# Russoul/cuda-mat

Hardware: AMD Instinct MI355X
Metric: BiCGSTAB iters/sec + SpMV effective HBM GB/s, 10M-row CSR at 1/2/4/8 GPUs (higher is better)
Workload: dtype f64

## Files before the change

### cuda_mat_amd/_lib.py

```python
import ctypes as C
import os
import subprocess

_HERE = os.path.dirname(os.path.abspath(__file__))
LIB_PATH = os.path.join(_HERE, "libcudamat_hip.so")

OK = 0
PRECOND_NONE, PRECOND_ILU0, PRECOND_BLOCK_ILU0 = 0, 1, 2
LOOP_PBICGSTAB, LOOP_PBICGSTAB2, LOOP_PIPELINED = 0, 1, 2
FLAG_DEBUG, FLAG_PROFILE, FLAG_NO_EXIT, FLAG_X0_ONES = 1, 2, 4, 8


class CudamatError(RuntimeError):
    def __init__(self, code, msg):
        super().__init__("cudamat error %d: %s" % (code, msg))
        self.code = code


class Stats(C.Structure):
    _fields_ = [("iters", C.c_int), ("half_exit", C.c_int), ("converged", C.c_int),
                ("breakdown", C.c_int), ("nrm0", C.c_double), ("nrm", C.c_double),
                ("t_analysis", C.c_double), ("t_factor", C.c_double), ("t_solve", C.c_double),
                ("t_total", C.c_double), ("ms_spmv", C.c_double), ("n_spmv", C.c_int),
                ("ms_trsv", C.c_double), ("n_trsv", C.c_int), ("n_levels_l", C.c_int),
                ("n_levels_u", C.c_int), ("trsv_form", C.c_int), ("trsv_fallbacks", C.c_int),
                ("n_gather", C.c_int), ("n_allreduce", C.c_int), ("ms_gather", C.c_double),
                ("ms_gather_exposed", C.c_double), ("ms_allreduce", C.c_double), ("overlapped", C.c_int),
                ("loop_form", C.c_int), ("gather_fraction", C.c_double), ("ms_spmv_alone", C.c_double),
                ("loop_fallbacks", C.c_int), ("restarts", C.c_int), ("t_upload", C.c_double), ("t_setup", C.c_double),
                ("t_tune", C.c_double), ("spmv_mode", C.c_int), ("plan_reused", C.c_int),
                ("trsv_groups_l", C.c_int), ("trsv_groups_u", C.c_int)]

    def as_dict(self):
        return {k: getattr(self, k) for k, _ in self._fields_}


ALLGATHER_FN = C.CFUNCTYPE(C.c_int, C.c_void_p, C.c_void_p, C.c_void_p, C.c_int64)
ALLREDUCE_FN = C.CFUNCTYPE(C.c_int, C.c_void_p, C.c_void_p, C.c_int)


GATHER_PART_FN = C.CFUNCTYPE(C.c_int, C.c_void_p, C.c_void_p, C.c_void_p, C.c_int64, C.c_int64, C.c_int64)
_I64P = C.POINTER(C.c_int64)
GATHER_WINDOW_FN = C.CFUNCTYPE(C.c_int, C.c_void_p, C.c_void_p, C.c_void_p, C.c_int64, _I64P, _I64P, _I64P, _I64P)


class Comm(C.Structure):
    _fields_ = [("rank", C.c_int), ("world", C.c_int), ("user", C.c_void_p),
                ("allgather", ALLGATHER_FN), ("allreduce", ALLREDUCE_FN),
                ("gather_part", GATHER_PART_FN), ("comm_stream", C.c_void_p),
                ("allreduce_side", ALLREDUCE_FN), ("reduce_stream", C.c_void_p),
                ("gather_window", GATHER_WINDOW_FN)]


def build(force=False):
    if force:
        subprocess.run(["make", "-C", _HERE, "clean"], check=True, capture_output=True)
    r = subprocess.run(["make", "-C", _HERE, "-j", "6"], capture_output=True, text=True)
    if r.returncode != 0:
        raise RuntimeError("building libcudamat_hip.so failed:\n" + r.stdout + r.stderr)


_P = C.c_void_p
_SIGS = {
    "cudamat_version": (C.c_int, []),
    "cudamat_last_error": (C.c_char_p, []),
    "cudamat_device_count": (C.c_int, [C.POINTER(C.c_int)]),
    "cudamat_ctx_create": (C.c_int, [C.c_int, _P, C.POINTER(_P)]),
    "cudamat_ctx_destroy": (C.c_int, [_P]),
    "cudamat_ctx_set_option": (C.c_int, [_P, C.c_char_p, C.c_char_p]),
    "cudamat_ctx_reset_options": (C.c_int, [_P]),
    "cudamat_options_help": (C.c_char_p, []),
    "cudamat_option_check": (C.c_int, [C.c_char_p, C.c_char_p]),
    "cudamat_ctx_sync": (C.c_int, [_P]),
    "cudamat_ctx_stream": (C.c_int, [_P, C.POINTER(_P)]),
    "cudamat_malloc": (C.c_int, [_P, C.c_size_t, C.POINTER(_P)]),
    "cudamat_free": (C.c_int, [_P, _P]),
    "cudamat_h2d": (C.c_int, [_P, _P, _P, C.c_size_t]),
    "cudamat_d2h": (C.c_int, [_P, _P, _P, C.c_size_t]),
    "cudamat_d2d": (C.c_int, [_P, _P, _P, C.c_size_t]),
    "cudamat_memset": (C.c_int, [_P, _P, C.c_int, C.c_size_t]),
    "cudamat_timer_create": (C.c_int, [_P, C.POINTER(_P)]),
    "cudamat_timer_start": (C.c_int, [_P, _P]),
    "cudamat_timer_stop": (C.c_int, [_P, _P]),
    "cudamat_timer_elapsed_ms": (C.c_int, [_P, _P, C.POINTER(C.c_double)]),
    "cudamat_timer_destroy": (C.c_int, [_P, _P]),
    "cudamat_spmv": (C.c_int, [_P, C.c_int, _P, _P, _P, C.c_int, C.c_double, _P, _P, C.c_double, _P]),
    "cudamat_dot": (C.c_int, [_P, C.c_int64, _P, _P, _P]),
    "cudamat_nrm2": (C.c_int, [_P, C.c_int64, _P, _P]),
    "cudamat_axpy": (C.c_int, [_P, C.c_int64, C.c_double, _P, _P]),
    "cudamat_scal": (C.c_int, [_P, C.c_int64, C.c_double, _P]),
    "cudamat_solver_create": (C.c_int, [_P, C.c_int, C.c_int64, C.c_int64, _P, _P, _P, C.c_int, C.POINTER(_P)]),
    "cudamat_solver_create_host": (C.c_int, [_P, C.c_int, C.c_int64, C.c_int64, _P, _P, _P, C.c_int, C.POINTER(_P)]),
    "cudamat_solver_destroy": (C.c_int, [_P]),
    "cudamat_solver_set_shift": (C.c_int, [_P, _P]),
    "cudamat_solver_ilu0": (C.c_int, [_P]),
    "cudamat_solver_block_ilu0": (C.c_int, [_P]),
    "cudamat_solver_ilu0_values": (C.c_int, [_P, _P]),
    "cudamat_solver_ilu0_nnz": (C.c_int, [_P, C.POINTER(C.c_int64)]),
    "cudamat_solver_trsv_form": (C.c_int, [_P, C.POINTER(C.c_int)]),
    "cudamat_solver_precond_apply": (C.c_int, [_P, _P, _P]),
    "cudamat_solver_set_comm": (C.c_int, [_P, C.POINTER(Comm)]),
    "cudamat_solve_sharded": (C.c_int, [C.c_int, C.c_int, C.c_int, _P, _P, _P, _P, _P, _P, C.c_int, C.c_int, C.c_int,
                                        C.c_double, C.c_int, _P, C.POINTER(Stats)]),
    "cudamat_comm_dry_create": (C.c_int, [_P, C.c_int, C.c_int, C.POINTER(Comm)]),
    "cudamat_comm_dry_destroy": (C.c_int, [C.POINTER(Comm)]),
    "cudamat_rccl_available": (C.c_int, []),
    "cudamat_rccl_unique_id": (C.c_int, [_P]),
    "cudamat_rccl_comm_create": (C.c_int, [_P, _P, C.c_int, C.c_int, C.POINTER(Comm)]),
    "cudamat_rccl_comm_destroy": (C.c_int, [C.POINTER(Comm)]),
    "cudamat_rccl_comm_abort": (C.c_int, [C.POINTER(Comm)]),
    "cudamat_solver_spmv_mode": (C.c_int, [_P, C.POINTER(C.c_int)]),
    "cudamat_solver_spmv_kernel": (C.c_int, [_P, C.c_char_p, C.c_int]),
    "cudamat_solver_value_dict": (C.c_int, [_P, C.POINTER(C.c_int)]),
    "cudamat_solver_placement": (C.c_int, [_P, C.POINTER(C.c_int), C.POINTER(C.c_int), C.POINTER(C.c_double), C.c_char_p, C.c_int]),
    "cudamat_solver_spmv": (C.c_int, [_P, _P, _P]),
    "cudamat_solver_solve": (C.c_int, [_P, _P, _P, C.c_int, C.c_int, C.c_int, C.c_double, C.c_int,
                                       C.POINTER(Stats)]),
    "cudamat_solver_history": (C.c_int, [_P, _P, C.c_int, C.POINTER(C.c_int)]),
    "cudamat_solver_spmm": (C.c_int, [_P, C.c_int, _P, C.c_int, _P, C.c_int]),
    "cudamat_solver_solve_many": (C.c_int, [_P, C.c_int, _P, C.c_int, _P, C.c_int, C.c_int, C.c_int, C.c_int, C.c_double,
                                            C.c_int, _P, C.POINTER(C.c_int)]),
    "cudamat_solver_precond_apply_many": (C.c_int, [_P, C.c_int, _P, C.c_int, _P, C.c_int]),
    "cudamat_solver_trsm_kernel": (C.c_int, [_P, C.c_int, C.c_char_p, C.c_int]),
    "cudamat_solver_history_col": (C.c_int, [_P, C.c_int, _P, C.c_int, C.POINTER(C.c_int)]),
    "cudamat_solve_many": (C.c_int, [C.c_int, C.c_int, _P, _P, _P, _P, C.c_int, _P, C.c_int, _P, _P, C.c_int, C.c_int,
                                     C.c_int, C.c_int, C.c_double, _P, C.POINTER(C.c_int)]),
    "cudamat_solver_spmm_shifts": (C.c_int, [_P, C.c_int, _P, C.c_int, _P, C.c_int, _P, C.c_int]),
    "cudamat_solver_solve_shifts": (C.c_int, [_P, C.c_int, _P, C.c_int, _P, C.c_int, _P, C.c_int, C.c_int, C.c_int, C.c_int,
                                              C.c_double, C.c_int, _P, C.POINTER(C.c_int)]),
    "cudamat_solve_shifts": (C.c_int, [C.c_int, C.c_int, _P, _P, _P, C.c_int, _P, C.c_int, _P, C.c_int, _P, _P, C.c_int,
                                       C.c_int, C.c_int, C.c_double, _P, C.POINTER(C.c_int)]),
    "cudamat_solve": (C.c_int, [C.c_int, C.c_int, _P, _P, _P, _P, _P, _P, C.c_int, C.c_int, C.c_int,
                                C.c_double, C.c_int, _P, C.POINTER(Stats)]),
    "cudamat_plan_cache_clear": (C.c_int, []),
    "cudamat_pool_trim": (C.c_int, []),
    "cudamat_mem_info": (C.c_int, [C.c_int, C.POINTER(C.c_size_t), C.POINTER(C.c_size_t), C.POINTER(C.c_size_t)]),
    "cudamat_poisson5_nnz": (C.c_int64, [C.c_int, C.c_int]),
    "cudamat_gen_poisson5": (C.c_int, [_P, C.c_int, C.c_int, C.c_int64, C.c_int64, C.c_int, _P, _P, _P]),
    "cudamat_rand_row_nnz": (C.c_int, [C.c_int64, C.c_int]),
    "cudamat_gen_rand_rows": (C.c_int, [_P, C.c_int64, C.c_int, C.c_uint64, C.c_int64, C.c_int64,
                                        C.c_int, _P, _P, _P]),
    "cudamat_gen_xstar": (C.c_int, [_P, C.c_int64, C.c_int64, C.c_uint64, _P]),
    "cudamat_load_mtx": (C.c_int, [C.c_char_p, C.c_int, C.POINTER(C.c_int), C.POINTER(C.c_int),
                                   C.POINTER(C.c_int), C.POINTER(C.POINTER(C.c_double)),
                                   C.POINTER(C.POINTER(C.c_int)), C.POINTER(C.POINTER(C.c_int))]),
    "cudamat_host_free": (None, [_P]),
    "cudamat_to_dense_vector": (None, [C.c_int, C.c_int, _P, _P, _P]),
}

_lib = None


def lib():
    global _lib
    if _lib is None:
        if not os.path.exists(LIB_PATH):
            build()
        L = C.CDLL(LIB_PATH)
        for name, (res, args) in _SIGS.items():
            fn = getattr(L, name)
            fn.restype = res
            fn.argtypes = args
        _lib = L
    return _lib


def check(rc):
    if rc != OK:
        raise CudamatError(rc, lib().cudamat_last_error().decode(errors="replace"))


def device_count():
    n = C.c_int(0)
    rc = lib().cudamat_device_count(C.byref(n))
    return n.value if rc == OK else 0
```

### cuda_mat_amd/api.py

```python
import ctypes as C

import numpy as np

from . import _lib
from ._lib import (FLAG_DEBUG, FLAG_NO_EXIT, FLAG_PROFILE, FLAG_X0_ONES, LOOP_PBICGSTAB,
                   LOOP_PBICGSTAB2, LOOP_PIPELINED, PRECOND_BLOCK_ILU0, PRECOND_ILU0, PRECOND_NONE, Comm, CudamatError, Stats, check)


def _np(a, dtype):
    return np.ascontiguousarray(a, dtype=dtype)


def _vp(a):
    return None if a is None else a.ctypes.data_as(C.c_void_p)


_GPUS = 1


def use_gpus(ngpu):
    global _GPUS
    _GPUS = max(1, int(ngpu))


def _solve(n, nnz, A, iA, jA, d, x0, b, precond, loop, maxit, tol, debug):
    A, iA, jA, b = _np(A, np.float64), _np(iA, np.int32), _np(jA, np.int32), _np(b, np.float64)
    d = None if d is None else _np(d, np.float64)
    x0 = None if x0 is None else _np(x0, np.float64)
    if len(iA) != n + 1 or len(A) < nnz or len(jA) < nnz or len(b) != n:
        raise ValueError("array sizes do not match n / nnz")
    x = np.zeros(n)
    st = Stats()
    if _GPUS > 1:
        if precond == PRECOND_ILU0:
            precond = PRECOND_BLOCK_ILU0
        check(_lib.lib().cudamat_solve_sharded(_GPUS, n, nnz, _vp(A), _vp(iA), _vp(jA), _vp(d), _vp(x0), _vp(b), precond,
                                               loop, maxit, tol, int(bool(debug)), _vp(x), C.byref(st)))
    else:
        check(_lib.lib().cudamat_solve(n, nnz, _vp(A), _vp(iA), _vp(jA), _vp(d), _vp(x0), _vp(b), precond,
                                       loop, maxit, tol, int(bool(debug)), _vp(x), C.byref(st)))
    return x, st


def bicgstab(n, nnz, A, iA, jA, b, maxit, tol, debug=False):
    x, st = _solve(n, nnz, A, iA, jA, None, None, b, PRECOND_NONE, LOOP_PBICGSTAB2, maxit, tol, debug)
    return bool(st.converged), x, st.t_solve, st


def bicgstab_d(n, nnz, A0, iA0, jA0, d, x0, b, maxit, tol, debug=False):
    x, st = _solve(n, nnz, A0, iA0, jA0, d, x0, b, PRECOND_NONE, LOOP_PBICGSTAB2, maxit, tol, debug)
    return bool(st.converged), x, st.t_solve, st


def bicgstab_lu_precond(n, nnz, A, iA, jA, b, maxit, tol, debug=False):
    x, st = _solve(n, nnz, A, iA, jA, None, None, b, PRECOND_ILU0, LOOP_PBICGSTAB, maxit, tol, debug)
    return True, x, st.t_solve, st


def bicgstab_many(n, nnz, A, iA, jA, B, maxit, tol, d=None, x0=None):
    A, iA, jA = _np(A, np.float64), _np(iA, np.int32), _np(jA, np.int32)
    B = np.asarray(B, dtype=np.float64)
    if B.ndim == 1:
        B = B[:, None]
    if len(iA) != n + 1 or len(A) < nnz or len(jA) < nnz or B.shape[0] != n:
        raise ValueError("array sizes do not match n / nnz")
    k = B.shape[1]
    Bf = np.asfortranarray(B)
    d = None if d is None else _np(d, np.float64)
    x0f = None
    if x0 is not None:
        x0f = np.asfortranarray(np.asarray(x0, dtype=np.float64).reshape(n, k))
    X = np.zeros((n, k), order="F")
    st = (Stats * max(k, 1))()
    form = C.c_int(0)
    check(_lib.lib().cudamat_solve_many(n, nnz, _vp(A), _vp(iA), _vp(jA), _vp(d), k, _vp(Bf), n, _vp(x0f), _vp(X), n,
                                        PRECOND_NONE, LOOP_PBICGSTAB2, maxit, tol, st, C.byref(form)))
    stats = [st[j] for j in range(k)]
    return [bool(s.converged) for s in stats], np.ascontiguousarray(X), (stats[0].t_solve if k else 0.0), stats, form.value


def bicgstab_d_many(n, nnz, A0, iA0, jA0, D, x0, B, maxit, tol):
    A0, iA0, jA0 = _np(A0, np.float64), _np(iA0, np.int32), _np(jA0, np.int32)
    B = np.asarray(B, dtype=np.float64)
    if B.ndim == 1:
        B = B[:, None]
    if len(iA0) != n + 1 or len(A0) < nnz or len(jA0) < nnz or B.ndim != 2 or B.shape[0] != n:
        raise ValueError("array sizes do not match n / nnz")
    k = B.shape[1]
    D = np.asarray(D, dtype=np.float64)
    if D.ndim == 1 and D.shape[0] == k:
        D = np.broadcast_to(D[None, :], (n, k))
    if D.shape != (n, k):
        raise ValueError("D must have shape (n, k) = (%d, %d), or hold k scalars; got %s" % (n, k, D.shape))
    Df, Bf = np.asfortranarray(D), np.asfortranarray(B)
    x0f = None
    if x0 is not None:
        x0f = np.asarray(x0, dtype=np.float64)
        if x0f.size != n * k:
            raise ValueError("x0 must have shape (n, k)")
        x0f = np.asfortranarray(x0f.reshape(n, k))
    X = np.zeros((n, k), order="F")
    st = (Stats * max(k, 1))()
    form = C.c_int(0)
    check(_lib.lib().cudamat_solve_shifts(n, nnz, _vp(A0), _vp(iA0), _vp(jA0), k, _vp(Df), n, _vp(Bf), n, _vp(x0f), _vp(X), n,
                                          LOOP_PBICGSTAB2, maxit, tol, st, C.byref(form)))
    stats = [st[j] for j in range(k)]
    return [bool(s.converged) for s in stats], np.ascontiguousarray(X), (stats[0].t_solve if k else 0.0), stats, form.value


def bicgstab_lu_precond_many(n, nnz, A, iA, jA, B, maxit, tol):
    A, iA, jA = _np(A, np.float64), _np(iA, np.int32), _np(jA, np.int32)
    B = np.asarray(B, dtype=np.float64)
    if B.ndim == 1:
        B = B[:, None]
    if len(iA) != n + 1 or len(A) < nnz or len(jA) < nnz or B.ndim != 2 or B.shape[0] != n:
        raise ValueError("array sizes do not match n / nnz")
    k = B.shape[1]
    Bf = np.asfortranarray(B)
    X = np.zeros((n, k), order="F")
    st = (Stats * max(k, 1))()
    form = C.c_int(0)
    check(_lib.lib().cudamat_solve_many(n, nnz, _vp(A), _vp(iA), _vp(jA), None, k, _vp(Bf), n, None, _vp(X), n,
                                        PRECOND_ILU0, LOOP_PBICGSTAB, maxit, tol, st, C.byref(form)))
    stats = [st[j] for j in range(k)]
    return [True] * k, np.ascontiguousarray(X), (stats[0].t_solve if k else 0.0), stats, form.value


def loadMMSparseMatrix(filename, elem_type="d", csrFormat=True):
    if elem_type != "d":
        raise ValueError("only elem_type 'd' is supported on this path")
    m, n, nnz = C.c_int(), C.c_int(), C.c_int()
    v, r, c = C.POINTER(C.c_double)(), C.POINTER(C.c_int)(), C.POINTER(C.c_int)()
    L = _lib.lib()
    err = L.cudamat_load_mtx(str(filename).encode(), int(bool(csrFormat)), C.byref(m), C.byref(n),
                             C.byref(nnz), C.byref(v), C.byref(r), C.byref(c))
    if err:
        return 1, 0, 0, 0, None, None, None
    nr = m.value + 1 if csrFormat else nnz.value
    nc = nnz.value if csrFormat else n.value + 1
    row = np.ctypeslib.as_array(r, shape=(nr,)).astype(np.int32, copy=True)
    col = np.ctypeslib.as_array(c, shape=(nc,)).astype(np.int32, copy=True) if nc else np.zeros(0, np.int32)
    val = (np.ctypeslib.as_array(v, shape=(nnz.value,)).astype(np.float64, copy=True)
           if nnz.value else np.zeros(0))
    for p in (v, r, c):
        L.cudamat_host_free(p)
    return 0, m.value, n.value, nnz.value, val, row, col


def toDenseVector(n, nnz, A, IA):
    A, IA = _np(A, np.float64), _np(IA, np.int32)
    out = np.empty(n)
    _lib.lib().cudamat_to_dense_vector(n, nnz, _vp(A), _vp(IA), _vp(out))
    return out


class DeviceArray:

    def __init__(self, ctx, n, dtype):
        self.ctx, self.n, self.dtype = ctx, int(n), np.dtype(dtype)
        p = C.c_void_p()
        check(_lib.lib().cudamat_malloc(ctx.h, self.n * self.dtype.itemsize, C.byref(p)))
        self.ptr = p.value

    @property
    def nbytes(self):
        return self.n * self.dtype.itemsize

    def upload(self, a):
        a = _np(a, self.dtype)
        assert a.size == self.n
        check(_lib.lib().cudamat_h2d(self.ctx.h, self.ptr, _vp(a), self.nbytes))
        return self

    def download(self):
        out = np.empty(self.n, self.dtype)
        check(_lib.lib().cudamat_d2h(self.ctx.h, _vp(out), self.ptr, self.nbytes))
        return out

    def zero(self):
        check(_lib.lib().cudamat_memset(self.ctx.h, self.ptr, 0, self.nbytes))
        return self

    def free(self):
        if self.ptr:
            _lib.lib().cudamat_free(self.ctx.h, self.ptr)
            self.ptr = None


def _ptr(a):
    if a is None:
        return None
    if isinstance(a, DeviceArray):
        return a.ptr
    if hasattr(a, "data_ptr"):
        return a.data_ptr()
    return int(a)


class Context:

    def __init__(self, device=0, stream=None):
        h = C.c_void_p()
        check(_lib.lib().cudamat_ctx_create(device, stream, C.byref(h)))
        self.h = h
        self.device = device

    def close(self):
        if self.h:
            _lib.lib().cudamat_ctx_destroy(self.h)
            self.h = None

    def sync(self):
        check(_lib.lib().cudamat_ctx_sync(self.h))

    def set_option(self, name, value):
        check(_lib.lib().cudamat_ctx_set_option(self.h, str(name).encode(), str(value).encode()))
        return self

    def reset_options(self):
        check(_lib.lib().cudamat_ctx_reset_options(self.h))
        return self

    def empty(self, n, dtype=np.float64):
        return DeviceArray(self, n, dtype)

    def array(self, a, dtype=None):
        a = np.asarray(a)
        dtype = a.dtype if dtype is None else dtype
        return DeviceArray(self, a.size, dtype).upload(a)

    def spmv(self, n, rowptr, colidx, val, base, x, y, alpha=1.0, beta=0.0, d=None):
        check(_lib.lib().cudamat_spmv(self.h, n, _ptr(rowptr), _ptr(colidx), _ptr(val), base, alpha,
                                      _ptr(x), _ptr(d), beta, _ptr(y)))

    def dot(self, n, x, y):
        out = self.empty(1)
        check(_lib.lib().cudamat_dot(self.h, n, _ptr(x), _ptr(y), out.ptr))
        v = out.download()[0]
        out.free()
        return v

    def nrm2(self, n, x):
        out = self.empty(1)
        check(_lib.lib().cudamat_nrm2(self.h, n, _ptr(x), out.ptr))
        v = out.download()[0]
        out.free()
        return v

    def axpy(self, n, alpha, x, y):
        check(_lib.lib().cudamat_axpy(self.h, n, alpha, _ptr(x), _ptr(y)))

    def scal(self, n, alpha, x):
        check(_lib.lib().cudamat_scal(self.h, n, alpha, _ptr(x)))

    def gen_rand_rows(self, n, per_row, seed, row0, row1, base, rowptr, colidx, val):
        check(_lib.lib().cudamat_gen_rand_rows(self.h, n, per_row, seed, row0, row1, base, _ptr(rowptr),
                                               _ptr(colidx), _ptr(val)))

    def gen_poisson5(self, nx, ny, row0, row1, base, rowptr, colidx, val):
        check(_lib.lib().cudamat_gen_poisson5(self.h, nx, ny, row0, row1, base, _ptr(rowptr),
                                              _ptr(colidx), _ptr(val)))

    def gen_xstar(self, i0, i1, seed, x):
        check(_lib.lib().cudamat_gen_xstar(self.h, i0, i1, seed, _ptr(x)))

    def timer(self):
        return Timer(self)


class Timer:

    def __init__(self, ctx):
        self.ctx = ctx
        h = C.c_void_p()
        check(_lib.lib().cudamat_timer_create(ctx.h, C.byref(h)))
        self.h = h

    def start(self):
        check(_lib.lib().cudamat_timer_start(self.ctx.h, self.h))

    def stop(self):
        check(_lib.lib().cudamat_timer_stop(self.ctx.h, self.h))

    def elapsed_ms(self):
        ms = C.c_double()
        check(_lib.lib().cudamat_timer_elapsed_ms(self.ctx.h, self.h, C.byref(ms)))
        return ms.value

    def close(self):
        if self.h:
            _lib.lib().cudamat_timer_destroy(self.ctx.h, self.h)
            self.h = None


class Solver:

    def __init__(self, ctx, n_local, n_cols, nnz, rowptr, colidx, val, base):
        self.ctx = ctx
        self.n, self.n_cols, self.nnz = int(n_local), int(n_cols), int(nnz)
        h = C.c_void_p()
        check(_lib.lib().cudamat_solver_create(ctx.h, self.n, self.n_cols, self.nnz, _ptr(rowptr),
                                               _ptr(colidx), _ptr(val), base, C.byref(h)))
        self.h = h
        self._keep = []

    @classmethod
    def from_host_csr(cls, ctx, rowptr, colidx, val, n_cols=None):
        rowptr, colidx, val = _np(rowptr, np.int32), _np(colidx, np.int32), _np(val, np.float64)
        n = len(rowptr) - 1
        base = int(rowptr[0])
        nnz = int(rowptr[-1]) - base
        if nnz == 0:
            colidx, val = np.zeros(1, np.int32), np.zeros(1)
        s = cls.__new__(cls)
        s.ctx = ctx
        s.n, s.n_cols, s.nnz = n, int(n if n_cols is None else n_cols), nnz
        h = C.c_void_p()
        check(_lib.lib().cudamat_solver_create_host(ctx.h, s.n, s.n_cols, s.nnz, _vp(rowptr), _vp(colidx), _vp(val), base, C.byref(h)))
        s.h = h
        s._keep = []
        return s

    def close(self):
        if self.h:
            _lib.lib().cudamat_solver_destroy(self.h)
            self.h = None

    def set_shift(self, d):
        self._keep.append(d)
        check(_lib.lib().cudamat_solver_set_shift(self.h, _ptr(d)))

    def set_comm(self, comm):
        self._keep.append(comm)
        check(_lib.lib().cudamat_solver_set_comm(self.h, None if comm is None else C.byref(comm)))

    def ilu0(self):
        check(_lib.lib().cudamat_solver_ilu0(self.h))

    def trsv_form(self):
        f = C.c_int()
        check(_lib.lib().cudamat_solver_trsv_form(self.h, C.byref(f)))
        return f.value

    def block_ilu0(self):
        check(_lib.lib().cudamat_solver_block_ilu0(self.h))

    def ilu0_values(self):
        cnt = C.c_int64()
        check(_lib.lib().cudamat_solver_ilu0_nnz(self.h, C.byref(cnt)))
        out = self.ctx.empty(max(cnt.value, 1))
        check(_lib.lib().cudamat_solver_ilu0_values(self.h, out.ptr))
        v = out.download()[:cnt.value]
        out.free()
        return v

    def precond_apply(self, vin, vout):
        check(_lib.lib().cudamat_solver_precond_apply(self.h, _ptr(vin), _ptr(vout)))

    def precond_apply_many(self, nrhs, In, ldin, Out, ldout):
        check(_lib.lib().cudamat_solver_precond_apply_many(self.h, int(nrhs), _ptr(In), int(ldin), _ptr(Out), int(ldout)))

    def trsm_kernel(self, nrhs):
        buf = C.create_string_buffer(160)
        check(_lib.lib().cudamat_solver_trsm_kernel(self.h, int(nrhs), buf, 160))
        return buf.value.decode()

    def spmv(self, x, y):
        check(_lib.lib().cudamat_solver_spmv(self.h, _ptr(x), _ptr(y)))

    def spmv_mode(self):
        m = C.c_int()
        check(_lib.lib().cudamat_solver_spmv_mode(self.h, C.byref(m)))
        return m.value

    def spmv_kernel(self):
        buf = C.create_string_buffer(96)
        check(_lib.lib().cudamat_solver_spmv_kernel(self.h, buf, 96))
        return buf.value.decode()

    def placement(self):
        placed, slabs, sec = C.c_int(), C.c_int(), C.c_double()
        buf = C.create_string_buffer(256)
        check(_lib.lib().cudamat_solver_placement(self.h, C.byref(placed), C.byref(slabs), C.byref(sec), buf, 256))
        return {"placed": placed.value, "slabs": slabs.value, "seconds": sec.value, "blocks_by_class": buf.value.decode().strip()}

    def value_dict(self):
        m = C.c_int()
        check(_lib.lib().cudamat_solver_value_dict(self.h, C.byref(m)))
        return m.value

    def solve(self, b, x, precond=PRECOND_NONE, loop=LOOP_PBICGSTAB, maxit=2000, tol=1e-8, flags=0):
        st = Stats()
        check(_lib.lib().cudamat_solver_solve(self.h, _ptr(b), _ptr(x), precond, loop, maxit, tol, flags,
                                              C.byref(st)))
        return st

    def history(self, cap=1 << 16, col=None):
        if col is not None:
            return self.history_col(col, cap)
        buf = np.empty(cap)
        cnt = C.c_int()
        check(_lib.lib().cudamat_solver_history(self.h, _vp(buf), cap, C.byref(cnt)))
        return buf[:cnt.value].copy()

    def history_col(self, col, cap=1 << 16):
        buf = np.empty(cap)
        cnt = C.c_int()
        check(_lib.lib().cudamat_solver_history_col(self.h, int(col), _vp(buf), cap, C.byref(cnt)))
        return buf[:cnt.value].copy()

    def spmm(self, nrhs, X, ldx, Y, ldy):
        check(_lib.lib().cudamat_solver_spmm(self.h, int(nrhs), _ptr(X), int(ldx), _ptr(Y), int(ldy)))

    def solve_many(self, nrhs, B, ldb, X, ldx, precond=PRECOND_NONE, loop=LOOP_PBICGSTAB, maxit=2000, tol=1e-8, flags=0):
        st = (Stats * max(int(nrhs), 1))()
        form = C.c_int(0)
        check(_lib.lib().cudamat_solver_solve_many(self.h, int(nrhs), _ptr(B), int(ldb), _ptr(X), int(ldx), precond, loop,
                                                   maxit, tol, flags, st, C.byref(form)))
        return [st[j] for j in range(int(nrhs))], form.value

    def spmm_shifts(self, nrhs, X, ldx, D, ldd, Y, ldy):
        check(_lib.lib().cudamat_solver_spmm_shifts(self.h, int(nrhs), _ptr(X), int(ldx), _ptr(D), int(ldd), _ptr(Y), int(ldy)))

    def solve_shifts(self, nrhs, D, ldd, B, ldb, X, ldx, precond=PRECOND_NONE, loop=LOOP_PBICGSTAB, maxit=2000, tol=1e-8,
                     flags=0):
        st = (Stats * max(int(nrhs), 1))()
        form = C.c_int(0)
        check(_lib.lib().cudamat_solver_solve_shifts(self.h, int(nrhs), _ptr(D), int(ldd), _ptr(B), int(ldb), _ptr(X), int(ldx),
                                                     precond, loop, maxit, tol, flags, st, C.byref(form)))
        return [st[j] for j in range(int(nrhs))], form.value
```

### cuda_mat_amd/csrc/config.cpp

```cpp
#include "config.h"

#include <stdio.h>
#include <stdlib.h>
#include <string.h>

#include <unistd.h>

#include <mutex>
#include <set>
#include <string>

extern char **environ;

#include "common.h"

namespace cm {

namespace {

enum Kind { K_FLAG, K_INT, K_LLONG, K_ENUM, K_FAIL };

struct Option {
    const char *name;
    Kind kind;
    int Config::*field;
    long long Config::*wide;
    long long lo, hi;
    const char *words;
    const char *help;
};

#define OPT_FLAG(NAME, FIELD, HELP) {NAME, K_FLAG, &Config::FIELD, nullptr, 0, 1, nullptr, HELP}
#define OPT_INT(NAME, FIELD, LO, HI, HELP) {NAME, K_INT, &Config::FIELD, nullptr, LO, HI, nullptr, HELP}
#define OPT_ENUM(NAME, FIELD, WORDS, HELP) {NAME, K_ENUM, &Config::FIELD, nullptr, 0, 0, WORDS, HELP}

const Option kOptions[] = {
    OPT_INT("VERBOSE", verbose, 0, 2, "1: set-up breakdowns and auto-tune timings on stderr; 2: also the memory classes of a large blocked copy's arrays (timed probe, diagnosis)"),
    OPT_FLAG("ROCTX", roctx, "roctx ranges around solver creation, SpMV-form choice, ILU(0) set-up, the loop, SpMVs and all-reduces"),
    OPT_ENUM("SPMV_MODE", spmv_mode, "csr=0,pb=1,sell=2,pat=3", "force the CSR forms / the blocked two-phase form / SELL-C-sigma / the row-pattern dictionary"),
    OPT_FLAG("SPMV_SELL", spmv_sell, "0: keep SELL-C-sigma out of the candidates"),
    OPT_ENUM("SPMV_FORM", spmv_form, "lanes=1,tiles=2", "inside the CSR forms: lanes per row / nnz-balanced tiles"),
    OPT_INT("SPMV_LANES", spmv_lanes, 2, 64, "lanes per row, a power of two (and no stream tiles)"),
    OPT_FLAG("SPMV_COMPRESS", spmv_compress, "0: stream kernel on the plain 32-bit indices"),
    OPT_FLAG("SPMV_ALIGN", spmv_align, "0: compressed stream kernel without line-aligned copies of its value / offset streams"),
    OPT_ENUM("SPMV_TUNE", spmv_tune_full, "full=1", "time every SpMV candidate even when the column span already decides"),
    OPT_FLAG("VALUE_DICT", value_dict, "0: keep fp64 values even when the matrix has <= 256 distinct ones"),
    OPT_INT("PB_MIN_WAVES", pb_min_waves, 256, 1 << 20, "blocked form: fewest phase-2 waves"),
    OPT_INT("PB_DEPTH", pb_depth, 4, 16, "blocked form: segment loads in flight per phase-2 wave (4, 8 or 16)"),
    OPT_FLAG("POOL", pool, "0: device memory straight from hipMalloc / hipFree instead of the library's recycling pool (read once per process)"),
    OPT_FLAG("SKIP_ORIG_COPY", skip_orig_copy, "0: cudamat_solve with ILU(0) builds the blocked copy in the original index space even when its loop will run in the level-major spaces"),
    OPT_FLAG("EARLY_ANALYSIS", early_analysis, "0: cudamat_solve analyses the ILU(0) levels after the upload of the values instead of beside it"),
    OPT_INT("PB_FILL_OCC", pb_fill_occ, 0, 64, "resident waves per CU of the two-pass fill's first pass (0: 8; probing)"),
    OPT_FLAG("PB_FILL2", pb_fill2, "0: fill the blocked copy with the single-pass scatter kernel (rounds 1-4) instead of the two-pass partition"),
    OPT_INT("PB_PLACE", pb_place, 0, 2, "blocked copy of a large matrix: 1 (default): a resident solver's product stream is placed in a memory class of its own, values and indices in another (timed probe of the device's memory classes, 10-35 ms per copy: spmv_pb.hip); 2: the drop-in calls place theirs as well; 0: arrays wherever the allocator puts them"),
    OPT_INT("PB_PLACE_MAX_MS", pb_place_max_ms, 0, 60000, "PB_PLACE: what the search for an arrangement may take before the arrays are allocated as ever (ms; the slabs it allocates included -- 0.3 ms per 16 GB on most boxes, 2 s on some)"),
    OPT_FLAG("PB_PROBE_FAIL", pb_probe_fail, "1 (tests): treat the run-time LDS-order probe as failed, i.e. select the architected-order phase 2"),
    OPT_FLAG("PB_STRICT", pb_strict, "1: phase 2 adds a row's products of one wave instruction rank by rank (architected order, +10 %)"),
    {"FUSED", K_LLONG, nullptr, &Config::fused, 0, 1LL << 40, nullptr,
     "0: never fold the vector updates into the SpMVs (three launches per iteration); N: do it for every supported plan up to N rows"},
    OPT_FLAG("RESIDENT", resident, "0: never run the whole loop of a very small system in one launch"),
    OPT_INT("RESIDENT_SPIN_LIMIT", resident_spin_limit, 0, 1 << 30, "polls a grid-barrier wait of the single-launch loop may take"),
    OPT_INT("PIPE_RR", pipe_rr, 0, 1 << 20, "residual replacement period of the pipelined loop (0: never)"),
    OPT_FLAG("TRSV_SYNCFREE", trsv_syncfree, "0: one launch per level; 1: dependency-driven launches also for narrow levels"),
    OPT_FLAG("TRSV_LDS", trsv_lds, "0: no single-workgroup LDS-resident triangular solve for small systems"),
    OPT_FLAG("TRSV_HYBRID", trsv_hybrid, "0 | 1: never / always split big factors into far (blocked SpMV) and near (dependency-driven) parts"),
    OPT_INT("TRSV_GROUPS", trsv_groups, 2, 128, "groups of levels of a hybrid factor"),
    OPT_INT("TRSV_LANES", trsv_lanes, 2, 64, "lanes per row of the triangular-solve kernels, a power of two"),
    OPT_INT("TRSV_SPIN_LIMIT", trsv_spin_limit, 1, 1 << 30, "polls of one dependency before a row gives up"),
    OPT_FLAG("TRSV_PERM", trsv_perm, "0: permute around every M^-1 application instead of running the loop in the level-major spaces"),
    OPT_FLAG("LEVELS_SWEEP", levels_sweep, "1: level analysis by relaxation sweeps"),
    OPT_FLAG("ILU0_SIMPLE", ilu0_simple, "1: numeric ILU(0) without LDS staging / prefetch"),
    OPT_FLAG("FORCE_SHARDED", force_sharded, "1: keep the collective path at world size 1"),
    OPT_FLAG("OVERLAP", overlap, "0: plain all-gather instead of pieces behind phase 1 of the blocked SpMV"),
    OPT_INT("OVERLAP_CHUNKS", overlap_chunks, 1, 16, "pieces per slice of an overlapped gather"),
    OPT_FLAG("WINDOWED", windowed, "0: never exchange windows (halo) only"),
    OPT_FLAG("SHARDED_ONE_DEVICE", sharded_one_device,
             "1: cudamat_solve_sharded with every rank on device 0 and host-synchronised copies in place of RCCL (debugging aid)"),
    OPT_FLAG("PLAN_CACHE", plan_cache, "0: cudamat_solve does not keep the solver of its last call"),
    OPT_ENUM("MANY_FORM", many_form, "auto=0,batched=1,columns=2",
             "several right-hand sides: batched (one SpMM per step for up to 8 columns) / columns (one solve per column); auto: the faster as timed at the first solve"),
    OPT_ENUM("MANY_PRECOND", many_precond, "columns=0,auto=1,batched=2",
             "several right-hand sides with ILU(0): columns (one preconditioned solve per column, default) / batched (multi-column triangular solves and one SpMM per step for up to 8 columns, where the factors are covered) / auto: the faster as timed at the first such solve; MANY_FORM = columns overrides"),
    {"TEST_COMM_FAIL", K_FAIL, nullptr, nullptr, 0, 0, nullptr, "rank:k -- fault injection: that rank's k-th all-reduce reports an error (tests)"},
};

bool power_of_two(long long v) { return v > 0 && (v & (v - 1)) == 0; }

bool apply(Config &cfg, const Option &o, const char *value)
{
    switch (o.kind) {
    case K_FLAG:
        if (!strcmp(value, "0") || !strcmp(value, "1")) { cfg.*(o.field) = value[0] - '0'; return true; }
        return false;
    case K_INT: {
        char *end = nullptr;
        const long long v = strtoll(value, &end, 10);
        if (end == value || *end || v < o.lo || v > o.hi) return false;
        if ((!strcmp(o.name, "SPMV_LANES") || !strcmp(o.name, "TRSV_LANES")) && !power_of_two(v)) return false;
        if (!strcmp(o.name, "PB_DEPTH") && v != 4 && v != 8 && v != 16) return false;
        cfg.*(o.field) = (int)v;
        return true;
    }
    case K_LLONG: {
        char *end = nullptr;
        const long long v = strtoll(value, &end, 10);
        if (end == value || *end || v < o.lo || v > o.hi) return false;
        cfg.*(o.wide) = v;
        return true;
    }
    case K_ENUM: {
        const size_t len = strlen(value);
        for (const char *w = o.words; w && *w;) {
            const char *eq = strchr(w, '=');
            if ((size_t)(eq - w) == len && !strncmp(w, value, len)) { cfg.*(o.field) = atoi(eq + 1); return true; }
            const char *comma = strchr(eq, ',');
            w = comma ? comma + 1 : nullptr;
        }
        return false;
    }
    case K_FAIL: {
        int r = -1, k = -1;
        if (sscanf(value, "%d:%d", &r, &k) != 2 || r < 0 || k < 1) return false;
        cfg.fail_rank = r;
        cfg.fail_call = k;
        return true;
    }
    }
    return false;
}

}

bool Config::operator==(const Config &o) const
{
    for (const Option &q : kOptions) {
        if (q.field && this->*(q.field) != o.*(q.field)) return false;
        if (q.wide && this->*(q.wide) != o.*(q.wide)) return false;
    }
    return fail_rank == o.fail_rank && fail_call == o.fail_call;
}

bool config_set(Config &cfg, const char *name, const char *value)
{
    if (!name || !value) { set_error("option name / value is NULL"); return false; }
    if (!strncmp(name, "CUDAMAT_", 8)) name += 8;
    for (const Option &o : kOptions) {
        if (strcmp(o.name, name)) continue;
        if (apply(cfg, o, value)) return true;
        set_error("option %s: value \"%s\" is not accepted (%s)", name, value, o.help);
        return false;
    }
    set_error("unknown option \"%s\" (cudamat_options_help lists them)", name);
    return false;
}

static void warn_once(const std::string &text)
{
    static std::mutex mu;
    static std::set<std::string> seen;
    std::lock_guard<std::mutex> lock(mu);
    if (seen.insert(text).second) fprintf(stderr, "cudamat: %s\n", text.c_str());
}

Config config_from_env()
{
    Config cfg;
    for (const Option &o : kOptions) {
        const std::string var = std::string("CUDAMAT_") + o.name;
        const char *v = getenv(var.c_str());
        if (!v || !*v) continue;
        if (!apply(cfg, o, v))
            warn_once(var + "=\"" + v + "\" is not an accepted value and was IGNORED (" + o.help + ")");
    }
    for (char **e = environ; e && *e; e++) {
        if (strncmp(*e, "CUDAMAT_", 8) || !strncmp(*e, "CUDAMAT_BENCH_", 14)) continue;
        const char *eq = strchr(*e, '=');
        if (!eq || !eq[1]) continue;
        const std::string name(*e + 8, (size_t)(eq - (*e + 8)));
        bool known = false;
        for (const Option &o : kOptions) known = known || name == o.name;
        if (!known) warn_once("CUDAMAT_" + name + " names no switch of this library and was IGNORED (cudamat_options_help lists them)");
    }
    return cfg;
}

const char *config_help()
{
    static const std::string text = [] {
        std::string t;
        for (const Option &o : kOptions) {
            t += "CUDAMAT_";
            t += o.name;
            t += o.kind == K_FLAG ? " = 0 | 1" : o.kind == K_ENUM ? " = " : o.kind == K_FAIL ? " = rank:k" : " = N";
            if (o.kind == K_ENUM) {
                for (const char *w = o.words; w && *w;) {
                    const char *eq = strchr(w, '=');
                    if (w != o.words) t += " | ";
                    t.append(w, (size_t)(eq - w));
                    const char *comma = strchr(eq, ',');
                    w = comma ? comma + 1 : nullptr;
                }
            }
            if (o.kind == K_INT || o.kind == K_LLONG) t += " in [" + std::to_string(o.lo) + ", " + std::to_string(o.hi) + "]";
            t += "   ";
            t += o.help;
            t += "\n";
        }
        return t;
    }();
    return text.c_str();
}

}
```

### cuda_mat_amd/csrc/config.h

```cpp
#pragma once

namespace cm {

struct Config {
    int verbose = 0;
    int roctx = 0;
    int spmv_mode = -1;
    int spmv_sell = 1;
    int spmv_form = 0;
    int spmv_lanes = 0;
    int spmv_compress = 1;
    int spmv_align = 1;
    int spmv_tune_full = 0;
    int value_dict = 1;
    int pb_min_waves = 0;
    int pb_depth = 0;
    int pool = 1;
    int skip_orig_copy = 1;
    int early_analysis = 1;
    int pb_fill_occ = 0;
    int pb_fill2 = 1;
    int pb_place = 1;
    int pb_place_max_ms = 300;
    int pb_probe_fail = 0;
    int pb_strict = 0;
    long long fused = -1;
    int resident = 1;
    int resident_spin_limit = -1;
    int pipe_rr = -1;
    int trsv_syncfree = -1;
    int trsv_lds = 1;
    int trsv_hybrid = -1;
    int trsv_groups = 0;
    int trsv_lanes = 0;
    int trsv_spin_limit = 0;
    int trsv_perm = 1;
    int levels_sweep = 0;
    int ilu0_simple = 0;
    int force_sharded = 0;
    int overlap = 1;
    int overlap_chunks = 0;
    int windowed = 1;
    int sharded_one_device = 0;
    int plan_cache = 1;
    int many_form = 0;
    int many_precond = 0;
    int fail_rank = -1, fail_call = -1;

    bool operator==(const Config &o) const;
    bool operator!=(const Config &o) const { return !(*this == o); }
};

Config config_from_env();
bool config_set(Config &cfg, const char *name, const char *value);
const char *config_help();

}
```

### cuda_mat_amd/csrc/solver.hip

```cpp
#include <mutex>
#include <utility>
#include <math.h>
#include <stdlib.h>
#include <string.h>

#include "solver.h"

using namespace cm;

namespace cm {

int dev_alloc(void **p, size_t bytes)
{
    *p = nullptr;
    hipError_t e = hipMalloc(p, bytes ? bytes : 16);
    if (e != hipSuccess) {
        set_error("hipMalloc(%zu bytes) failed: %s", bytes, hipGetErrorString(e));
        return e == hipErrorOutOfMemory ? CUDAMAT_ERR_NOMEM : CUDAMAT_ERR_HIP;
    }
    return CUDAMAT_OK;
}

static void free_work(cudamat_solver *s)
{
    double **vs[] = {&s->r, &s->rw, &s->p, &s->pw, &s->s, &s->t, &s->v, &s->gather, &s->x0_save, &s->v2,
                     &s->pz, &s->pww, &s->pq, &s->py, &s->pxh, &s->pipeA, &s->pipeB, &s->red_pipe,
                     &s->prh, &s->pwh, &s->psh, &s->pzh, &s->pqh, &s->ptmp};
    for (double **q : vs) {
        if (*q) CM_DROP(hipFree(*q));
        *q = nullptr;
    }
}

int ensure_work(cudamat_solver *s)
{
    if (s->r) return CUDAMAT_OK;
    hipStream_t st = s->ctx->stream;
    const size_t nb = sizeof(double) * (size_t)(s->n_pad > 0 ? s->n_pad : 1);
    double **vs[] = {&s->r, &s->rw, &s->p, &s->pw, &s->s, &s->t, &s->v};
    for (double **q : vs) {
        CM_TRY(dev_alloc((void **)q, nb));
        CM_HIP(hipMemsetAsync(*q, 0, nb, st));
    }
    if (s->ctx->cfg.verbose)
        fprintf(stderr, "[cudamat] work vectors: r %p rw %p p %p pw %p s %p t %p v %p (%zu bytes each)\n", (void *)s->r, (void *)s->rw, (void *)s->p,
                (void *)s->pw, (void *)s->s, (void *)s->t, (void *)s->v, nb);
    if (s->sharded) {
        CM_TRY(dev_alloc((void **)&s->gather, nb * (size_t)s->comm.world));
        CM_HIP(hipMemsetAsync(s->gather, 0, nb * (size_t)s->comm.world, st));
    }
    return CUDAMAT_OK;
}

}

__global__ __launch_bounds__(kBlock) void k_check_rowptr(int n, long long nnz, const int *rp, int *flags)
{
    const long long i = (long long)blockIdx.x * kBlock + threadIdx.x;
    if (i > n) return;
    bool bad = false;
    if (i == 0 && rp[0] != 0) bad = true;
    if (i == n && rp[n] != nnz) bad = true;
    if (i < n && rp[i] > rp[i + 1]) bad = true;
    if (rp[i] < 0 || rp[i] > nnz) bad = true;
    if (bad) flags[0] = 1;
}

__global__ __launch_bounds__(kBlock) void k_check_columns(int n, long long n_cols, const int *rp, const int *ci, int *flags)
{
    constexpr int L = 8;
    const long long row = ((long long)blockIdx.x * kBlock + threadIdx.x) / L;
    if (row >= n) return;
    const int lane = threadIdx.x & (L - 1);
    const int s = rp[row], e = rp[row + 1];
    bool range = false, order = false;
    for (int k = s + lane; k < e; k += L) {
        const int c = ci[k];
        if (c < 0 || c >= n_cols) range = true;
        if (k > s && ci[k - 1] >= c) order = true;
    }
    if (range) flags[1] = 1;
    if (order) flags[2] = 1;
}

static int validate_csr(cudamat_solver *s)
{
    hipStream_t st = s->ctx->stream;
    int *d = (int *)s->ctx->scratch, h[3] = {0, 0, 0};
    hipError_t e = hipMemsetAsync(d, 0, sizeof(h), st);
    hipLaunchKernelGGL(k_check_rowptr, dim3((unsigned)(((long long)s->n + 1 + kBlock - 1) / kBlock)), dim3(kBlock), 0, st, s->n,
                       (long long)s->nnz, s->rp, d);
    if (e == hipSuccess) e = hipGetLastError();
    if (e == hipSuccess) e = hipMemcpyAsync(h, d, sizeof(h), hipMemcpyDeviceToHost, st);
    if (e == hipSuccess) e = hipStreamSynchronize(st);
    if (e == hipSuccess && !h[0] && s->n > 0 && s->nnz > 0) {
        hipLaunchKernelGGL(k_check_columns, dim3((unsigned)(((long long)s->n * 8 + kBlock - 1) / kBlock)), dim3(kBlock), 0, st,
                           s->n, (long long)s->n_cols, s->rp, s->ci, d);
        e = hipGetLastError();
        if (e == hipSuccess) e = hipMemcpyAsync(h, d, sizeof(h), hipMemcpyDeviceToHost, st);
        if (e == hipSuccess) e = hipStreamSynchronize(st);
    }
    if (e != hipSuccess) return fail_hip(e, "CSR validation", __FILE__, __LINE__);
    if (h[0]) { set_error("row pointers must start at the index base, never decrease and end at nnz"); return CUDAMAT_ERR_ARG; }
    if (h[1]) { set_error("a column index lies outside [base, base + n_cols)"); return CUDAMAT_ERR_ARG; }
    s->cols_sorted = h[2] == 0;
    return CUDAMAT_OK;
}

namespace cm {

int solver_alloc(cudamat_ctx *ctx, int n_local, int64_t n_cols, int64_t nnz, cudamat_solver **out)
{
    *out = nullptr;
    CM_ARG(n_local >= 0 && n_cols >= n_local && nnz >= 0, "sizes");
    CM_ARG(nnz < (1LL << 31) && n_cols < (1LL << 31), "local nnz and dimension must fit int32");
    CM_HIP(hipSetDevice(ctx->device));
    cudamat_solver *s = new cudamat_solver();
    s->ctx = ctx;
    s->n = n_local;
    s->n_pad = n_local;
    s->n_cols = n_cols;
    s->nnz = nnz;
    s->t_create0 = now_s();
    hipStream_t st = ctx->stream;
    int rc = CUDAMAT_OK;
    do {
        if ((rc = dev_alloc((void **)&s->rp, sizeof(int) * ((size_t)n_local + 1)))) break;
        if ((rc = dev_alloc((void **)&s->ci, sizeof(int) * (size_t)nnz))) break;
        if ((rc = dev_alloc((void **)&s->val, sizeof(double) * (size_t)nnz))) break;
        if ((rc = dev_alloc((void **)&s->parts_full, sizeof(double) * 2 * kMaxParts))) break;
        if ((rc = dev_alloc((void **)&s->parts_rv, sizeof(double) * 2 * kMaxParts))) break;
        if ((rc = dev_alloc((void **)&s->parts_half, sizeof(double) * 2 * kMaxParts))) break;
        if ((rc = dev_alloc((void **)&s->parts_tt, sizeof(double) * 2 * kMaxParts))) break;
        if ((rc = dev_alloc((void **)&s->red, sizeof(double) * 16))) break;
        if ((rc = dev_alloc((void **)&s->st, sizeof(LoopState)))) break;
        if (hipHostMalloc((void **)&s->st_ring, sizeof(LoopState) * kRing, hipHostMallocDefault) != hipSuccess) {
            rc = CUDAMAT_ERR_HIP; set_error("hipHostMalloc failed"); break;
        }
        if (hipHostMalloc((void **)&s->snap_host, sizeof(unsigned long long) * kRing, hipHostMallocDefault) != hipSuccess ||
            hipHostGetDevicePointer((void **)&s->snap_dev, s->snap_host, 0) != hipSuccess) {
            rc = CUDAMAT_ERR_HIP; set_error("pinned progress words unavailable"); break;
        }
        if (hipMemsetAsync(s->st, 0, sizeof(LoopState), st) != hipSuccess) { rc = CUDAMAT_ERR_HIP; break; }
    } while (0);
    if (rc) {
        cudamat_solver_destroy(s);
        return rc;
    }
    *out = s;
    return CUDAMAT_OK;
}

int solver_setup_pattern(cudamat_solver *s)
{
    cudamat_ctx *ctx = s->ctx;
    hipStream_t st = ctx->stream;
    const bool verbose = ctx->cfg.verbose != 0;
    double t_mark = now_s();
    auto stamp = [&](const char *what) {
        if (!verbose) return;
        const double t = now_s();
        fprintf(stderr, "[cudamat] create %-34s %8.3f ms\n", what, (t - t_mark) * 1e3);
        t_mark = t;
    };
    if (verbose) fprintf(stderr, "[cudamat] create %-34s %8.3f ms\n", "allocations + copies", (t_mark - s->t_create0) * 1e3);
    CM_TRY(validate_csr(s));
    stamp("validation");
    s->plan = plan_spmv(ctx->cfg, s->n, s->nnz);
    CM_TRY(plan_spmv_refine(st, ctx->cfg, s->n, s->nnz, s->rp, 0, &s->plan, ctx->scratch));
    stamp("CSR launch plan (refine)");
    CM_TRY(plan_spmv_compress(st, ctx->cfg, s->n, s->nnz, s->rp, s->ci, &s->plan));
    stamp("compressed-index attempt");
    return CUDAMAT_OK;
}

int solver_setup_values(cudamat_solver *s)
{
    cudamat_ctx *ctx = s->ctx;
    hipStream_t st = ctx->stream;
    if (s->plan.c_off16) {
        CM_TRY(ensure_valdict(s));
        if (s->vd.n > 0) CM_TRY(plan_spmv_dict(st, s->n, s->nnz, s->rp, s->vd.idx, s->vd.dict, &s->plan));
        if (!s->plan.d_pbase)
            CM_TRY(plan_spmv_align(st, ctx->cfg, s->n, s->nnz, s->rp, s->val, &s->plan));
    }
    s->t_create = now_s() - s->t_create0;
    return CUDAMAT_OK;
}

}

extern "C" int cudamat_solver_create(cudamat_ctx *ctx, int n_local, int64_t n_cols, int64_t nnz,
                                     const int *rowptr, const int *colidx, const double *val,
                                     int base, cudamat_solver **out)
{
    CM_ARG(ctx && out, "null pointer");
    *out = nullptr;
    CM_ARG(base == 0 || base == 1, "base in {0,1}");
    CM_ARG(rowptr && (nnz == 0 || (colidx && val)), "null CSR array");
    Range range_create("cudamat: solver create (copies, validation, CSR plan)");
    cudamat_solver *s = nullptr;
    CM_TRY(solver_alloc(ctx, n_local, n_cols, nnz, &s));
    hipStream_t st = ctx->stream;
    int rc = launch_rebase(st, (int64_t)n_local + 1, rowptr, -base, s->rp);
    if (!rc && nnz) {
        rc = launch_rebase(st, nnz, colidx, -base, s->ci);
        if (!rc && hipMemcpyAsync(s->val, val, sizeof(double) * (size_t)nnz, hipMemcpyDeviceToDevice, st) != hipSuccess) {
            rc = CUDAMAT_ERR_HIP; set_error("val copy failed");
        }
    }
    if (!rc && hipStreamSynchronize(st) != hipSuccess) { rc = CUDAMAT_ERR_HIP; set_error("sync after upload failed"); }
    if (!rc) rc = solver_setup_pattern(s);
    if (!rc) rc = solver_setup_values(s);
    if (rc) {
        cudamat_solver_destroy(s);
        return rc;
    }
    *out = s;
    return CUDAMAT_OK;
}

extern "C" int cudamat_solver_destroy(cudamat_solver *s)
{
    if (!s) return CUDAMAT_OK;
    CM_DROP(hipSetDevice(s->ctx->device));
    CM_DROP(hipStreamSynchronize(s->ctx->stream));
    ilu0_release(s);
    pb_free(&s->pb);
    sell_free(&s->sell);
    pat_free(&s->pat);
    free_work(s);
    many_release(s);
    plan_spmv_free(&s->plan);
    void *ptrs[] = {s->rp, s->ci, s->val, s->parts_full, s->parts_rv, s->parts_half, s->parts_tt,
                    s->red, s->st, s->hist};
    for (void *p : ptrs)
        if (p) CM_DROP(hipFree(p));
    if (s->st_ring) CM_DROP(hipHostFree(s->st_ring));
    if (s->snap_host) CM_DROP(hipHostFree(s->snap_host));
    for (int i = 0; i < kRing; i++)
        if (s->ev[i]) CM_DROP(hipEventDestroy(s->ev[i]));
    for (hipEvent_t e : s->prof_ev) CM_DROP(hipEventDestroy(e));
    for (hipEvent_t e : s->comm_ev) CM_DROP(hipEventDestroy(e));
    if (s->need_dev) CM_DROP(hipFree(s->need_dev));
    if (s->bar) CM_DROP(hipFree(s->bar));
    valdict_free(&s->vd);
    for (int e = 0; e < 2; e++) {
        if (s->ev_red[e]) CM_DROP(hipEventDestroy(s->ev_red[e]));
        if (s->ev_red_done[e]) CM_DROP(hipEventDestroy(s->ev_red_done[e]));
    }
    if (s->ev_x) CM_DROP(hipEventDestroy(s->ev_x));
    for (hipEvent_t e : s->ev_part)
        if (e) CM_DROP(hipEventDestroy(e));
    for (hipEvent_t e : s->ev_p1)
        if (e) CM_DROP(hipEventDestroy(e));
    for (hipStream_t q : s->part_stream)
        if (q) { CM_DROP(hipStreamSynchronize(q)); CM_DROP(hipStreamDestroy(q)); }
    delete s;
    return CUDAMAT_OK;
}

extern "C" int cudamat_solver_set_shift(cudamat_solver *s, const double *d)
{
    CM_ARG(s, "solver is NULL");
    s->d = d;
    return CUDAMAT_OK;
}

extern "C" int cudamat_solver_set_comm(cudamat_solver *s, const cudamat_comm *comm)
{
    CM_ARG(s, "solver is NULL");
    CM_HIP(hipStreamSynchronize(s->ctx->stream));
    free_work(s);
    pb_free(&s->pb);
    sell_free(&s->sell);
    pat_free(&s->pat);
    ilu0_release(s);
    s->spmv_mode = -1;
    s->overlap = false;
    s->agreed = false;
    s->windowed = false;
    s->windows_known = false;
    if (s->need_dev) { CM_DROP(hipFree(s->need_dev)); s->need_dev = nullptr; }
    const bool forced = comm && comm->world == 1 && s->ctx->cfg.force_sharded;
    if (!comm || (comm->world <= 1 && !forced)) {
        s->sharded = false;
        s->n_pad = s->n;
        return CUDAMAT_OK;
    }
    CM_ARG(comm->allgather && comm->allreduce, "collectives missing");
    CM_ARG(comm->rank >= 0 && comm->rank < comm->world, "rank");
    const int64_t per = (s->n_cols + comm->world - 1) / comm->world;
    int64_t mine = s->n_cols - per * comm->rank;
    if (mine > per) mine = per;
    if (mine < 0) mine = 0;
    if (mine != s->n) {
        set_error("row block mismatch: rank %d of %d must own %lld rows of %lld (uniform blocks of %lld), has %d",
                  comm->rank, comm->world, (long long)mine, (long long)s->n_cols, (long long)per, s->n);
        return CUDAMAT_ERR_ARG;
    }
    s->comm = *comm;
    s->sharded = true;
    s->n_pad = (int)per;
    if (comm->gather_window && comm->world > 1 && comm->world <= 4096)
        CM_TRY(dev_alloc((void **)&s->need_dev, sizeof(double) * ((size_t)2 * comm->world + (size_t)2 * comm->world * comm->world)));
    if (comm->gather_part && comm->comm_stream && !s->ev_x) {
        CM_HIP(hipEventCreateWithFlags(&s->ev_x, hipEventDisableTiming));
        for (int c = 0; c < kPbMaxChunks; c++) {
            CM_HIP(hipEventCreateWithFlags(&s->ev_part[c], hipEventDisableTiming));
            CM_HIP(hipEventCreateWithFlags(&s->ev_p1[c], hipEventDisableTiming));
            CM_HIP(hipStreamCreateWithFlags(&s->part_stream[c], hipStreamNonBlocking));
        }
    }
    if (s->ctx->cfg.overlap_chunks >= 1 && s->ctx->cfg.overlap_chunks <= kPbMaxChunks) s->overlap_chunks = s->ctx->cfg.overlap_chunks;
    return CUDAMAT_OK;
}

namespace cm {

static hipEvent_t comm_event(cudamat_solver *s)
{
    if (s->comm_used == s->comm_ev.size()) {
        hipEvent_t e = nullptr;
        if (hipEventCreate(&e) != hipSuccess) s->prof_failed = true;
        s->comm_ev.push_back(e);
    }
    return s->comm_ev[s->comm_used++];
}
void comm_mark_begin(cudamat_solver *s, int kind, hipStream_t st)
{
    if (!s->profiling) return;
    s->comm_kind.push_back(kind);
    if (hipEventRecord(comm_event(s), st) != hipSuccess) s->prof_failed = true;
}
void comm_mark_end(cudamat_solver *s, hipStream_t st)
{
    if (s->profiling && hipEventRecord(comm_event(s), st) != hipSuccess) s->prof_failed = true;
}

int spmv_local(cudamat_solver *s, const double *x_local, double *y, int dot, const double *w,
               double *parts, LoopArgs la, int check, ScalarSrc half)
{
    Range range_spmv(s->sharded ? "cudamat: SpMV + exchange of its input" : "cudamat: SpMV");
    const double *xfull = x_local;
    const bool windowed = s->sharded && s->windowed;
    const bool overlapped = s->sharded && !windowed && s->overlap && s->spmv_mode == 1;
    if (windowed) {
        hipStream_t st = s->ctx->stream;
        CM_HIP(hipMemcpyAsync(s->gather + (size_t)s->comm.rank * (size_t)s->n_pad, x_local, sizeof(double) * (size_t)s->n_pad,
                              hipMemcpyDeviceToDevice, st));
        comm_mark_begin(s, 2, st);
        if (s->comm.gather_window(s->comm.user, x_local, s->gather, (int64_t)s->n_pad, s->w_send_off.data(), s->w_send_cnt.data(),
                                  s->w_recv_off.data(), s->w_recv_cnt.data()) != 0) {
            set_error("gather_window callback failed");
            return CUDAMAT_ERR_COMM;
        }
        comm_mark_end(s, st);
    } else if (s->sharded && !overlapped) {
        comm_mark_begin(s, 2, s->ctx->stream);
        if (s->comm.allgather(s->comm.user, x_local, s->gather, (int64_t)s->n_pad) != 0) {
            set_error("allgather callback failed");
            return CUDAMAT_ERR_COMM;
        }
        comm_mark_end(s, s->ctx->stream);
    }
    if (s->sharded) xfull = s->gather;
    SpmvArgs a{};
    a.n = s->n;
    a.rp = s->rp;
    a.ci = s->ci;
    a.val = s->val;
    a.x = xfull;
    a.d = s->d;
    a.xd = x_local;
    a.alpha = 1.0;
    a.beta = 0.0;
    a.y = y;
    a.dot = dot;
    a.w = w;
    a.parts = parts;
    a.loop = la;
    a.check = check;
    a.half = half;
    a.pb_strict = 0;
    if (s->spmv_mode == 1 || s->perm_active) CM_TRY(pb_strict_for(s->ctx, &a.pb_strict));
    if (overlapped) {
        hipStream_t st = s->ctx->stream, cst = (hipStream_t)s->comm.comm_stream;
        const PbPlan &p = s->pb;
        CM_HIP(hipEventRecord(s->ev_x, st));
        CM_HIP(hipStreamWaitEvent(cst, s->ev_x, 0));
        comm_mark_begin(s, 0, cst);
        for (int c = 0; c < p.chunks; c++) {
            const int64_t off = (int64_t)c * p.chunk_len;
            int64_t cnt = (int64_t)s->n_pad - off;
            if (cnt > p.chunk_len) cnt = p.chunk_len;
            if (cnt > 0 && s->comm.gather_part(s->comm.user, x_local, s->gather, (int64_t)s->n_pad, off, cnt) != 0) {
                set_error("gather_part callback failed");
                return CUDAMAT_ERR_COMM;
            }
            CM_HIP(hipEventRecord(s->ev_part[c], cst));
        }
        comm_mark_end(s, cst);
        CM_HIP(hipMemcpyAsync(s->gather + (size_t)s->comm.rank * (size_t)s->n_pad, x_local, sizeof(double) * (size_t)s->n_pad,
                              hipMemcpyDeviceToDevice, st));
        CM_TRY(launch_pb_check(st, a));
        CM_TRY(launch_pb_phase1(st, p, a, 0));
        for (int c = 0; c < p.chunks; c++) {
            hipStream_t ps = s->part_stream[c];
            CM_HIP(hipStreamWaitEvent(ps, s->ev_x, 0));
            CM_HIP(hipStreamWaitEvent(ps, s->ev_part[c], 0));
            CM_TRY(launch_pb_phase1(ps, p, a, 1 + c));
            CM_HIP(hipEventRecord(s->ev_p1[c], ps));
        }
        for (int c = 0; c < p.chunks; c++) CM_HIP(hipStreamWaitEvent(st, s->ev_p1[c], 0));
        return launch_pb_phase2(st, p, a);
    }
    if (s->perm_active) return launch_spmv_pb(s->ctx->stream, s->pb_perm, a);
    if (s->spmv_mode == 1) return launch_spmv_pb(s->ctx->stream, s->pb, a);
    if (s->spmv_mode == 2) return launch_spmv_sell(s->ctx->stream, s->sell, a);
    if (s->spmv_mode == 3) return launch_spmv_pat(s->ctx->stream, s->pat, a);
    return launch_spmv(s->ctx->stream, s->plan, a);
}

int ensure_valdict(cudamat_solver *s)
{
    if (s->vd_tried) return CUDAMAT_OK;
    s->vd_tried = true;
    if (s->nnz < (1 << 20)) return CUDAMAT_OK;
    return valdict_build(s->ctx->stream, s->ctx->cfg, s->nnz, s->val, &s->vd);
}

int spmv_parts(const cudamat_solver *s)
{
    if (s->perm_active) return s->pb_perm.NRB;
    return s->spmv_mode == 1 ? s->pb.NRB : s->spmv_mode == 2 ? s->sell.grid : s->spmv_mode == 3 ? s->pat.grid : plan_spmv_parts(s->plan);
}

__global__ __launch_bounds__(kBlock) void k_col_span(int n, const int *rp, const int *ci, int samples, unsigned long long *sum, int *cnt)
{
    const int q = blockIdx.x * kBlock + threadIdx.x;
    if (q >= samples) return;
    const int row = (int)((long long)q * n / samples);
    const int s = rp[row], e = rp[row + 1];
    if (e - s < 2) return;
    atomicAdd(sum, (unsigned long long)(ci[e - 1] - ci[s]));
    atomicAdd(cnt, 1);
}

static int col_span_bytes(cudamat_solver *s, double *out)
{
    *out = 0.0;
    hipStream_t st = s->ctx->stream;
    unsigned long long *d = (unsigned long long *)s->ctx->scratch, h[2] = {0ULL, 0ULL};
    CM_HIP(hipMemsetAsync(d, 0, sizeof(h), st));
    const int samples = s->n < 4096 ? s->n : 4096;
    hipLaunchKernelGGL(k_col_span, dim3((samples + kBlock - 1) / kBlock), dim3(kBlock), 0, st, s->n, s->rp, s->ci, samples, d, (int *)(d + 1));
    hipError_t e = hipMemcpyAsync(h, d, sizeof(h), hipMemcpyDeviceToHost, st);
    if (e == hipSuccess) e = hipStreamSynchronize(st);
    CM_HIP(e);
    const int cnt = (int)(h[1] & 0xffffffffULL);
    *out = cnt > 0 ? 8.0 * (double)h[0] / cnt : 0.0;
    return CUDAMAT_OK;
}

static int ensure_spmv_mode_inner(cudamat_solver *s);

int spmv_mode_is_blocked_early(cudamat_solver *s, bool *blocked)
{
    *blocked = false;
    const Config &cfg = s->ctx->cfg;
    if (s->sharded || s->n == 0 || s->nnz == 0 || !s->cols_sorted) return CUDAMAT_OK;
    if (cfg.spmv_mode == 0 || cfg.spmv_mode == 2) return CUDAMAT_OK;
    if (cfg.spmv_mode == 1) { *blocked = true; return CUDAMAT_OK; }
    if (!pb_candidate(s->ctx->stream, s->n, s->n_cols, s->nnz, s->rp, s->ci)) return CUDAMAT_OK;
    if (cfg.spmv_tune_full || s->nnz < 8 * (int64_t)s->n) return CUDAMAT_OK;
    if (s->col_span_bytes < 0.0) CM_TRY(col_span_bytes(s, &s->col_span_bytes));
    *blocked = s->col_span_bytes >= 16.0 * 1024 * 1024;
    return CUDAMAT_OK;
}

void spmv_mode_adopt_blocked(cudamat_solver *s, const PbPlan &pb, double seconds)
{
    s->pb = pb;
    s->spmv_mode = 1;
    s->t_spmv_setup = seconds;
    if (s->ctx->cfg.verbose)
        fprintf(stderr, "[cudamat] SpMV form 1 (blocked) built beside the upload in %.3f ms (a row's columns span %.1f MB of x)\n",
                seconds * 1e3, s->col_span_bytes / 1048576.0);
}

int ensure_spmv_mode(cudamat_solver *s)
{
    if (s->spmv_mode >= 0) return CUDAMAT_OK;
    Range range_mode("cudamat: SpMV form (matrix copies, tuning)");
    const double t0 = now_s();
    int rc = ensure_spmv_mode_inner(s);
    const int rc_sync = CM_RC(hipStreamSynchronize(s->ctx->stream));
    if (!rc) rc = rc_sync;
    s->t_spmv_setup = now_s() - t0;
    if (s->ctx->cfg.verbose)
        fprintf(stderr, "[cudamat] SpMV form %d chosen in %.3f ms (blocked copy %.3f ms, timing %.3f ms)\n", s->spmv_mode,
                s->t_spmv_setup * 1e3, s->pb.build_seconds * 1e3, s->t_spmv_timing * 1e3);
    return rc;
}

static int ensure_spmv_mode_inner(cudamat_solver *s)
{
    hipStream_t st = s->ctx->stream;
    const Config &cfg = s->ctx->cfg;
    const bool force_csr = cfg.spmv_mode == 0;
    const bool force_pb = cfg.spmv_mode == 1;
    const bool force_sell = cfg.spmv_mode == 2;
    const bool force_pat = cfg.spmv_mode == 3;
    s->spmv_mode = 0;
    if (force_csr || s->n == 0 || s->nnz == 0) return CUDAMAT_OK;
    bool have[4] = {true, false, false, false};
    if (!force_sell && !force_pat) {
        if (!s->cols_sorted) {
            if (force_pb) { set_error("the blocked SpMV needs rows with increasing column indices"); return CUDAMAT_ERR_ARG; }
        } else if (force_pb || pb_candidate(st, s->n, s->n_cols, s->nnz, s->rp, s->ci)) {
            PbCols cols;
            const bool can_overlap = s->sharded && s->comm.world > 1 && s->comm.gather_part && s->comm.comm_stream;
            if (s->sharded && s->comm.world > 1) {
                cols.per = s->n_pad;
                cols.rank = s->comm.rank;
                cols.chunks = can_overlap ? s->overlap_chunks : 1;
            }
            CM_TRY(ensure_valdict(s));
            const int rc = pb_build(st, cfg, s->n, s->n_cols, s->nnz, s->rp, s->ci, s->val, &s->pb, &cols, &s->vd);
            if (rc != CUDAMAT_OK && force_pb) return rc;
            have[1] = rc == CUDAMAT_OK;
        }
        if (force_pb && !s->sharded) { s->spmv_mode = 1; return CUDAMAT_OK; }
        if (force_pb) { have[0] = false; }
    }
    bool scattered = false;
    {
        if (have[1] && !force_pb && !force_sell && !force_pat && !cfg.spmv_tune_full && s->nnz >= 8 * (int64_t)s->n) {
            if (s->col_span_bytes < 0.0) CM_TRY(col_span_bytes(s, &s->col_span_bytes));
            scattered = s->col_span_bytes >= 16.0 * 1024 * 1024;
        }
        if (scattered) {
            have[0] = false;
            if (!s->sharded) {
                s->spmv_mode = 1;
                if (cfg.verbose)
                    fprintf(stderr, "cudamat: SpMV: a row's columns span %.1f MB of x on average -> blocked, nothing timed\n", s->col_span_bytes / 1048576.0);
                return CUDAMAT_OK;
            }
        }
    }
    const bool sell_off = !cfg.spmv_sell;
    if (force_sell || (!force_pb && !force_pat && !scattered && !sell_off && s->n >= 4096 && s->nnz >= (1 << 16) && s->plan.stream_rows == 0 && s->nnz >= 8 * (int64_t)s->n)) {
        const int rc = sell_build(st, s->n, s->nnz, s->rp, s->ci, s->val, &s->sell, force_sell ? 0.0 : 1.5);
        if (rc != CUDAMAT_OK && force_sell) return rc;
        have[2] = rc == CUDAMAT_OK;
        if (force_sell) { s->spmv_mode = 2; return CUDAMAT_OK; }
    }
    if (force_pat || (!force_pb && !scattered && s->plan.stream_rows > 0 && s->n > 300000 && s->nnz >= (1 << 20))) {
        CM_TRY(ensure_valdict(s));
        const int rc = pat_build(st, s->n, s->nnz, s->rp, s->ci, s->val, &s->pat, force_pat ? 0.0 : 1.25, &s->vd);
        if (rc != CUDAMAT_OK && (force_pat || rc != CUDAMAT_ERR_ARG) && rc != CUDAMAT_ERR_NOMEM) return rc;
        if (rc != CUDAMAT_OK && force_pat) return rc;
        have[3] = rc == CUDAMAT_OK;
        if (force_pat) { s->spmv_mode = 3; return CUDAMAT_OK; }
    }
    if (!have[1] && !have[2] && !have[3]) return CUDAMAT_OK;
    if (force_pb && !have[1]) { set_error("the blocked copy could not be built"); return CUDAMAT_ERR_NOMEM; }
    if (force_pb) have[2] = have[3] = false;
    const LoopArgs la_none{nullptr, nullptr, 0, 0, 0};
    const ScalarSrc nosrc{nullptr, 0, 1};
    const double *xin = s->sharded ? s->gather : s->p;
    hipEvent_t e0 = nullptr, e1 = nullptr;
    CM_HIP(hipEventCreate(&e0));
    if (hipEventCreate(&e1) != hipSuccess) { CM_DROP(hipEventDestroy(e0)); return fail_hip(hipGetLastError(), "hipEventCreate", __FILE__, __LINE__); }
    float ms[4] = {0.f, 0.f, 0.f, 0.f};
    int rc = CUDAMAT_OK;
    const double t_timing0 = now_s();
    for (int mode = 0; mode < 4 && rc == CUDAMAT_OK; mode++) {
        if (!have[mode]) continue;
        SpmvArgs a{};
        a.n = s->n; a.rp = s->rp; a.ci = s->ci; a.val = s->val; a.x = xin; a.d = nullptr; a.xd = s->p;
        a.alpha = 1.0; a.beta = 0.0; a.y = s->v; a.dot = 0; a.loop = la_none; a.check = CHECK_NONE; a.half = nosrc;
        a.pb_strict = 0;
        if (mode == 1) CM_TRY(pb_strict_for(s->ctx, &a.pb_strict));
        for (int rep = 0; rep < 3 && rc == CUDAMAT_OK; rep++) {
            if (rep == 1) rc = CM_RC(hipEventRecord(e0, st));
            if (rc) break;
            rc = mode == 1 ? launch_spmv_pb(st, s->pb, a) : mode == 2 ? launch_spmv_sell(st, s->sell, a) :
                 mode == 3 ? launch_spmv_pat(st, s->pat, a) : launch_spmv(st, s->plan, a);
        }
        if (!rc) rc = CM_RC(hipEventRecord(e1, st));
        if (!rc) rc = CM_RC(hipEventSynchronize(e1));
        if (!rc) rc = CM_RC(hipEventElapsedTime(&ms[mode], e0, e1));
    }
    CM_DROP(hipEventDestroy(e0));
    CM_DROP(hipEventDestroy(e1));
    CM_TRY(rc);
    s->t_spmv_timing = now_s() - t_timing0;
    CM_HIP(hipMemsetAsync(s->v, 0, sizeof(double) * (size_t)(s->n_pad > 0 ? s->n_pad : 1), st));
    s->ms_csr = ms[0] / 2;
    s->ms_pb = ms[1] / 2;
    s->ms_sell = ms[2] / 2;
    s->ms_pat = ms[3] / 2;
    int best = have[0] ? 0 : 1;
    if (rc == CUDAMAT_OK)
        for (int mode = 1; mode < 4; mode++)
            if (have[mode] && (!have[best] || ms[mode] < ms[best])) best = mode;
    s->spmv_mode = best;
    s->ms_spmv_alone = ms[best] / 2;
    const double sell_fill = s->sell.fill;
    if (best != 1) pb_free(&s->pb);
    if (best != 2) sell_free(&s->sell);
    const int npat = s->pat.npat;
    if (best != 3) pat_free(&s->pat);
    if (cfg.verbose)
        fprintf(stderr, "cudamat: SpMV auto-tune csr %.3f ms, blocked %s%.3f ms, sell %s%.3f ms (fill %.2f), row patterns %s%.3f ms (%d patterns) -> %s\n",
                s->ms_csr, have[1] ? "" : "(n/a) ", s->ms_pb, have[2] ? "" : "(n/a) ", s->ms_sell, sell_fill, have[3] ? "" : "(n/a) ", s->ms_pat,
                npat, best == 1 ? "blocked" : best == 2 ? "sell" : best == 3 ? "row patterns" : "csr");
    return CUDAMAT_OK;
}

int allreduce(cudamat_solver *s, double *buf, int count)
{
    Range range_ar("cudamat: all-reduce");
    if (s->ctx->cfg.fail_rank >= 0 && s->ctx->cfg.fail_rank == s->comm.rank && ++s->test_allreduces == s->ctx->cfg.fail_call) {
        set_error("injected all-reduce failure (TEST_COMM_FAIL=%d:%d)", s->ctx->cfg.fail_rank, s->ctx->cfg.fail_call);
        return CUDAMAT_ERR_COMM;
    }
    comm_mark_begin(s, 3, s->ctx->stream);
    if (s->comm.allreduce(s->comm.user, buf, count) != 0) {
        set_error("allreduce callback failed");
        return CUDAMAT_ERR_COMM;
    }
    comm_mark_end(s, s->ctx->stream);
    return CUDAMAT_OK;
}

__global__ __launch_bounds__(kBlock) void k_col_windows(long long nnz, const int *ci, int per, int world, int *lo, int *hi)
{
    extern __shared__ int tab[];
    int *lo_s = tab, *hi_s = tab + world;
    for (int q = threadIdx.x; q < world; q += kBlock) { lo_s[q] = per; hi_s[q] = 0; }
    __syncthreads();
    const long long per_thread = (nnz + (long long)gridDim.x * kBlock - 1) / ((long long)gridDim.x * kBlock);
    const long long k0 = ((long long)blockIdx.x * kBlock + threadIdx.x) * per_thread;
    const long long k1 = k0 + per_thread < nnz ? k0 + per_thread : nnz;
    int cq = -1, clo = 0, chi = 0;
    for (long long k = k0; k < k1; k++) {
        const int c = ci[k], q = c / per, w = c - q * per;
        if (q == cq && w >= clo && w < chi) continue;
        if (q != cq) { cq = q; clo = w; chi = w + 1; }
        else { clo = w < clo ? w : clo; chi = w + 1 > chi ? w + 1 : chi; }
        atomicMin(&lo_s[q], w);
        atomicMax(&hi_s[q], w + 1);
    }
    __syncthreads();
    for (int q = threadIdx.x; q < world; q += kBlock) {
        if (hi_s[q] > 0) { atomicMin(&lo[q], lo_s[q]); atomicMax(&hi[q], hi_s[q]); }
    }
}

static int compute_windows(cudamat_solver *s)
{
    s->windows_known = true;
    s->windowed = false;
    s->gather_fraction = 1.0;
    const int W = s->comm.world, me = s->comm.rank;
    if (!s->comm.gather_window || W <= 1 || W > 4096) return CUDAMAT_OK;
    hipStream_t st = s->ctx->stream;
    const int per = s->n_pad;
    std::vector<int> h((size_t)2 * W);
    std::vector<double> mine((size_t)2 * W, 0.0), all((size_t)2 * W * W, 0.0);
    char saved[512] = "";
    auto local = [&]() -> int {
        int *d_lohi = nullptr;
        CM_HIP(hipMalloc((void **)&d_lohi, sizeof(int) * 2 * (size_t)W));
        for (int q = 0; q < W; q++) { h[(size_t)q] = per; h[(size_t)W + q] = 0; }
        hipError_t e = hipMemcpyAsync(d_lohi, h.data(), sizeof(int) * h.size(), hipMemcpyHostToDevice, st);
        if (e == hipSuccess && s->nnz > 0) {
            hipLaunchKernelGGL(k_col_windows, dim3(row_grid(s->nnz, 4096LL * kBlock)), dim3(kBlock), sizeof(int) * 2 * (size_t)W, st, (long long)s->nnz, s->ci, per, W,
                               d_lohi, d_lohi + W);
        }
        if (e == hipSuccess) e = hipMemcpyAsync(h.data(), d_lohi, sizeof(int) * h.size(), hipMemcpyDeviceToHost, st);
        if (e == hipSuccess) e = hipStreamSynchronize(st);
        CM_DROP(hipFree(d_lohi));
        CM_HIP(e);
        for (int q = 0; q < W; q++)
            if (q != me && h[(size_t)W + q] > h[(size_t)q]) { mine[(size_t)2 * q] = h[(size_t)q]; mine[(size_t)2 * q + 1] = h[(size_t)W + q]; }
        return CUDAMAT_OK;
    };
    const int rc_local = local();
    if (rc_local != CUDAMAT_OK) {
        snprintf(saved, sizeof(saved), "%s", cudamat_last_error());
        mine.assign((size_t)2 * W, -1.0);
    }
    CM_HIP(hipMemcpyAsync(s->need_dev, mine.data(), sizeof(double) * mine.size(), hipMemcpyHostToDevice, st));
    CM_HIP(hipStreamSynchronize(st));
    if (s->comm.allgather(s->comm.user, s->need_dev, s->need_dev + 2 * W, (int64_t)2 * W) != 0) {
        set_error("allgather callback failed");
        return CUDAMAT_ERR_COMM;
    }
    CM_HIP(hipMemcpyAsync(all.data(), s->need_dev + 2 * W, sizeof(double) * all.size(), hipMemcpyDeviceToHost, st));
    CM_HIP(hipStreamSynchronize(st));
    if (rc_local != CUDAMAT_OK) { set_error("%s", saved); return rc_local; }
    for (double v : all)
        if (v < 0.0) { set_error("another rank failed while it looked for its column windows"); return CUDAMAT_ERR_COMM; }
    s->w_send_off.assign((size_t)W, 0); s->w_send_cnt.assign((size_t)W, 0);
    s->w_recv_off.assign((size_t)W, 0); s->w_recv_cnt.assign((size_t)W, 0);
    double worst = 0.0;
    for (int p = 0; p < W; p++) {
        double tot = 0.0;
        for (int q = 0; q < W; q++) {
            const double lo = all[((size_t)p * W + q) * 2], hi = all[((size_t)p * W + q) * 2 + 1];
            if (q == p || hi <= lo) continue;
            tot += hi - lo;
            if (p == me) { s->w_recv_off[(size_t)q] = (int64_t)lo; s->w_recv_cnt[(size_t)q] = (int64_t)(hi - lo); }
            if (q == me) { s->w_send_off[(size_t)p] = (int64_t)lo; s->w_send_cnt[(size_t)p] = (int64_t)(hi - lo); }
        }
        const double frac = tot / ((double)(W - 1) * (double)per);
        if (p == me) s->gather_fraction = frac;
        worst = frac > worst ? frac : worst;
    }
    s->windowed = worst <= 0.5 && s->ctx->cfg.windowed;
    if (!s->windowed) s->gather_fraction = 1.0;
    if (s->ctx->cfg.verbose)
        fprintf(stderr, "cudamat: rank %d references %.4f of the other slices (worst rank %.4f) -> %s\n", me,
                s->windowed ? s->gather_fraction : worst, worst, s->windowed ? "windowed gather" : "whole gather");
    return CUDAMAT_OK;
}

int setup_agree(cudamat_solver *s, int rc_local)
{
    if (!s->sharded) return rc_local;
    char saved[512];
    snprintf(saved, sizeof(saved), "%s", cudamat_last_error());
    hipStream_t st = s->ctx->stream;
    double h[2] = {rc_local != CUDAMAT_OK ? 1.0 : 0.0, s->spmv_mode == 1 ? 1.0 : 0.0};
    CM_HIP(hipMemcpyAsync(s->red + 10, h, sizeof(h), hipMemcpyHostToDevice, st));
    CM_HIP(hipStreamSynchronize(st));
    CM_TRY(allreduce(s, s->red + 10, 2));
    CM_HIP(hipMemcpyAsync(h, s->red + 10, sizeof(h), hipMemcpyDeviceToHost, st));
    CM_HIP(hipStreamSynchronize(st));
    s->overlap = s->comm.world > 1 && s->comm.gather_part && s->comm.comm_stream && s->ev_x && s->pb.chunks >= 1 &&
                 h[1] == (double)s->comm.world && s->ctx->cfg.overlap;
    s->agreed = true;
    if (h[0] == 0.0 && !s->windows_known) CM_TRY(compute_windows(s));
    if (h[0] != 0.0) {
        if (rc_local != CUDAMAT_OK) { set_error("%s", saved); return rc_local; }
        set_error("%d rank(s) of the sharded solver failed during setup", (int)h[0]);
        return CUDAMAT_ERR_COMM;
    }
    return CUDAMAT_OK;
}

}

extern "C" int cudamat_solver_spmv_mode(cudamat_solver *s, int *mode)
{
    CM_ARG(s && mode, "null pointer");
    CM_HIP(hipSetDevice(s->ctx->device));
    CM_TRY(ensure_work(s));
    CM_TRY(ensure_spmv_mode(s));
    *mode = s->spmv_mode;
    return CUDAMAT_OK;
}

extern "C" int cudamat_solver_value_dict(cudamat_solver *s, int *distinct)
{
    CM_ARG(s && distinct, "null pointer");
    CM_HIP(hipSetDevice(s->ctx->device));
    CM_TRY(ensure_work(s));
    CM_TRY(ensure_spmv_mode(s));
    *distinct = 0;
    if (s->spmv_mode == 1 && s->pb.pvi) *distinct = s->pb.ndict;
    else if (s->spmv_mode == 0 && s->plan.d_pbase) *distinct = s->vd.n;
    else if (s->spmv_mode == 3 && s->pat.vidx) *distinct = s->pat.ndict;
    return CUDAMAT_OK;
}

extern "C" int cudamat_solver_placement(cudamat_solver *s, int *placed, int *slabs, double *seconds, char *classes, int cap)
{
    CM_ARG(s, "null pointer");
    CM_HIP(hipSetDevice(s->ctx->device));
    CM_TRY(ensure_work(s));
    CM_TRY(ensure_spmv_mode(s));
    const PbPlan *q = s->pb_perm.P ? &s->pb_perm : s->spmv_mode == 1 && s->pb.P ? &s->pb : nullptr;
    if (placed) *placed = q ? q->placed : -1;
    if (slabs) *slabs = q ? q->place_slabs : 0;
    if (seconds) *seconds = q ? q->place_seconds : 0.0;
    if (classes && cap > 0) snprintf(classes, (size_t)cap, "%s", q ? q->place_classes : "");
    return CUDAMAT_OK;
}

extern "C" int cudamat_solver_spmv_kernel(cudamat_solver *s, char *name, int cap)
{
    CM_ARG(s && name && cap > 0, "null pointer");
    CM_HIP(hipSetDevice(s->ctx->device));
    CM_TRY(ensure_work(s));
    CM_TRY(ensure_spmv_mode(s));
    const SpmvPlan &p = s->plan;
    if (s->spmv_mode == 1) {
        int strict = 0;
        CM_TRY(pb_strict_for(s->ctx, &strict));
        snprintf(name, (size_t)cap, "%s + k_pb_phase2%s", s->pb.pvi ? "k_pb_phase1_dict" : "k_pb_phase1", strict ? " (architected order)" : "");
    }
    else if (s->spmv_mode == 2) snprintf(name, (size_t)cap, "k_spmv_sell");
    else if (s->spmv_mode == 3 && s->pat.vidx) snprintf(name, (size_t)cap, "k_spmv_pat_d<%d>", s->pat.vword / 8);
    else if (s->spmv_mode == 3) snprintf(name, (size_t)cap, "k_spmv_pat<%d>", s->pat.W <= 8 ? 8 : 16);
    else if (p.tiles > 0) snprintf(name, (size_t)cap, "k_spmv_tiles");
    else if (p.stream_rows && p.c_off16) snprintf(name, (size_t)cap, "%s<%d>", p.d_pbase ? "k_spmv_stream_d" : "k_spmv_stream_c", p.stream_rows);
    else if (p.stream_rows) snprintf(name, (size_t)cap, "k_spmv_stream<%d>", p.stream_rows);
    else snprintf(name, (size_t)cap, "k_spmv<%d>", p.lanes);
    return CUDAMAT_OK;
}

extern "C" int cudamat_solver_spmv(cudamat_solver *s, const double *x_local, double *y_local)
{
    CM_ARG(s && x_local && y_local, "null pointer");
    CM_HIP(hipSetDevice(s->ctx->device));
    {
        int rc_setup = ensure_work(s);
        if (rc_setup == CUDAMAT_OK) rc_setup = ensure_spmv_mode(s);
        if (s->sharded && !s->agreed) rc_setup = setup_agree(s, rc_setup);
        CM_TRY(rc_setup);
    }
    const double *xin = x_local;
    if (s->sharded) {
        CM_HIP(hipMemcpyAsync(s->pw, x_local, sizeof(double) * (size_t)s->n, hipMemcpyDeviceToDevice,
                              s->ctx->stream));
        xin = s->pw;
    }
    return spmv_local(s, xin, y_local, 0, nullptr, nullptr, LoopArgs{nullptr, nullptr, 0, 0, 0},
                      CHECK_NONE, ScalarSrc{nullptr, 0, 1});
}

namespace cm {

hipEvent_t prof_event(cudamat_solver *s, size_t i)
{
    while (s->prof_ev.size() <= i) {
        hipEvent_t e = nullptr;
        if (hipEventCreate(&e) != hipSuccess) s->prof_failed = true;
        s->prof_ev.push_back(e);
    }
    return s->prof_ev[i];
}

int precond_apply(cudamat_solver *s, const double *in, double *tmp, double *out, bool native)
{
    if (s->L.lm && !native) return precond_apply_original(s, in, tmp, out);
    CM_TRY(trsv_apply(s, s->L, false, in, tmp));
    CM_TRY(trsv_apply(s, s->U, true, tmp, out));
    return CUDAMAT_OK;
}

}

extern "C" int cudamat_solver_precond_apply(cudamat_solver *s, const double *in, double *out)
{
    CM_ARG(s && in && out, "null pointer");
    CM_ARG(s->has_ilu, "call cudamat_solver_ilu0 / cudamat_solver_block_ilu0 first");
    CM_HIP(hipSetDevice(s->ctx->device));
    CM_TRY(ensure_work(s));
    return precond_apply(s, in, s->t, out);
}
```

### cuda_mat_amd/csrc/spmv_pb.h

```cpp
#pragma once
#include "kernels.h"
#include "valdict.h"

namespace cm {

constexpr int kPbMaxChunks = 16;

struct PbCols {
    int64_t per = 0;
    int chunks = 1;
    int rank = 0;
};

struct PbPlan {
    int n = 0;
    int64_t n_cols = 0;
    int64_t nnz = 0;
    int CB = 0, NCB = 0;
    int64_t per = 0;
    int chunks = 1;
    int64_t chunk_len = 0;
    int bpc = 0;
    int RB = 0, NRB = 0;
    int NW = 0;
    int SR = 0;
    int LPS = 64;
    int depth = 4;
    int NSUB = 0;
    double *pv = nullptr;
    unsigned char *pvi = nullptr;
    const double *dict = nullptr;
    int ndict = 0;
    unsigned short *pc = nullptr;
    unsigned short *pr = nullptr;
    double *P = nullptr;
    int *cstart = nullptr;
    int *col0 = nullptr;
    int *sstart = nullptr;
    int *slen = nullptr;
    int *order = nullptr;
    int part_off[kPbMaxChunks + 2] = {0};
    int placed = -1;
    int place_slabs = 0;
    double place_seconds = 0.0;
    float place_check_ms = 0.f, place_fast_ms = 0.f, place_slow_ms = 0.f;
    char place_classes[192] = {0};
    bool pc_zeroed = false;
    double build_seconds = 0.0;
};

struct PbCut {
    int per, chunks, chunk_len, bpc, CB;
};
struct PbBuild {
    PbPlan p;
    int *bins = nullptr;
    PbCut cut{};
    size_t cap = 0;
    double t0 = 0.0;
    bool verbose = false;
    bool two_pass = false;
    int place = 0;
    bool report_classes = false;
    double place_max_seconds = 0.3;
    int fill_occ = 0;
    int GB = 1, NG = 1;
    unsigned long long *smeta = nullptr;
    int *gstart = nullptr;
};
int pb_build_begin(hipStream_t st, const Config &cfg, int n, int64_t n_cols, int64_t nnz, const int *rp, const int *ci,
                   const PbCols *cols, PbBuild *b);
int pb_build_alloc(hipStream_t st, const Config &cfg, int n, int64_t n_cols, int64_t nnz, const PbCols *cols, PbBuild *b);
int pb_build_count(hipStream_t st, const Config &cfg, const int *rp, const int *ci, PbBuild *b);
int pb_build_values(hipStream_t st, PbBuild *b, const ValDict *vd);
int pb_build_fill(hipStream_t st, PbBuild *b, const int *rp, const int *ci, const double *val, const ValDict *vd, int sub0, int sub1);
int pb_build_end(hipStream_t st, PbBuild *b, PbPlan *out);
void pb_build_abort(PbBuild *b);

bool pb_candidate(hipStream_t st, int n, int64_t n_cols, int64_t nnz, const int *rp, const int *ci);
int pb_build(hipStream_t st, const Config &cfg, int n, int64_t n_cols, int64_t nnz, const int *rp, const int *ci,
             const double *val, PbPlan *out, const PbCols *cols = nullptr, const ValDict *vd = nullptr);
void pb_free(PbPlan *p);
int pb_strict_for(cudamat_ctx *ctx, int *strict);
int launch_spmv_pb(hipStream_t st, const PbPlan &plan, const SpmvArgs &a);
int launch_pb_check(hipStream_t st, const SpmvArgs &a);
int launch_pb_phase1(hipStream_t st, const PbPlan &plan, const SpmvArgs &a, int part);
int launch_pb_phase2(hipStream_t st, const PbPlan &plan, const SpmvArgs &a);

}
```

### cuda_mat_amd/csrc/spmv_pb.hip

```cpp
#include <algorithm>
#include <map>
#include <mutex>
#include <string>
#include <vector>

#include "spmv_pb.h"

namespace cm {

typedef unsigned short u16;
constexpr int kPbBuildWaves = 4;
constexpr int kP1Threads = 1024;
constexpr int kP1Unroll = 8;
constexpr int kTileMax = 13312;
constexpr int kPbAlign = 64;

template <typename T>
static int dalloc(T **p, size_t count)
{
    *p = nullptr;
    hipError_t e = hipMalloc((void **)p, sizeof(T) * (count ? count : 1));
    if (e != hipSuccess) {
        set_error("hipMalloc(%zu bytes) failed: %s", sizeof(T) * count, hipGetErrorString(e));
        return e == hipErrorOutOfMemory ? CUDAMAT_ERR_NOMEM : CUDAMAT_ERR_HIP;
    }
    return CUDAMAT_OK;
}

void pb_free(PbPlan *p)
{
    void *ptrs[] = {p->pv, p->pvi, p->pc, p->pr, p->P, p->cstart, p->col0, p->sstart, p->slen, p->order};
    for (void *q : ptrs)
        if (q) CM_DROP(hipFree(q));
    *p = PbPlan();
}

bool pb_candidate(hipStream_t st, int n, int64_t n_cols, int64_t nnz, const int *rp, const int *ci)
{
    (void)st; (void)rp; (void)ci;
    if (n < 65536 || nnz < (1 << 20) || n_cols * 8 < (1 << 20)) return false;
    if ((double)nnz / n < 4.0) return false;
    if ((int64_t)n > (int64_t)kMaxParts * kTileMax) return false;
    return true;
}

__device__ __forceinline__ int col_to_cb(const PbCut &c, int col)
{
    const int q = col / c.per, w = col - q * c.per;
    const int ch = w / c.chunk_len, off = w - ch * c.chunk_len;
    return (q * c.chunks + ch) * c.bpc + off / c.CB;
}

__device__ __forceinline__ int col_to_cb_fast(const PbCut &c, double inv_cb, int col)
{
    if (c.chunks == 1 && col < c.per) {
        int cb = (int)((double)col * inv_cb);
        cb -= (long long)cb * c.CB > (long long)col ? 1 : 0;
        cb += (long long)(cb + 1) * c.CB <= (long long)col ? 1 : 0;
        return cb;
    }
    return col_to_cb(c, col);
}

__device__ __forceinline__ int wave_match_rank(unsigned long long *tab, int key, bool active, int lane, int nkeys, int *count_of_key_lane)
{
    if (lane < nkeys) tab[lane] = 0ULL;
    __builtin_amdgcn_fence(__ATOMIC_RELEASE, "wavefront");
    __builtin_amdgcn_wave_barrier();
    if (active) atomicOr(&tab[key], 1ULL << lane);
    __builtin_amdgcn_fence(__ATOMIC_RELEASE, "wavefront");
    __builtin_amdgcn_wave_barrier();
    const unsigned long long mine = active ? tab[key] : 0ULL;
    *count_of_key_lane = lane < nkeys ? __popcll(tab[lane]) : 0;
    __builtin_amdgcn_fence(__ATOMIC_RELEASE, "wavefront");
    __builtin_amdgcn_wave_barrier();
    return __popcll(mine & ((1ULL << lane) - 1ULL));
}

template <bool FILL>
__global__ __launch_bounds__(64 * kPbBuildWaves) void k_pb_rows(int n, const int *rp, const int *ci,
                                                               const double *val, PbCut cut, const int *col0, int NCB,
                                                               int SR, int NSUB, int *bins, double *pv, u16 *pc, u16 *pr,
                                                               const unsigned char *vidx, unsigned char *pvi, int sub0, int sub1)
{
    extern __shared__ int lds_i[];
    const int wave = threadIdx.x >> 6, lane = threadIdx.x & 63;
    const int sub = sub0 + blockIdx.x * kPbBuildWaves + wave;
    if (sub >= sub1) return;
    int *cur = lds_i + (size_t)wave * NCB;
    for (int c = lane; c < NCB; c += 64) cur[c] = FILL ? bins[(size_t)c * NSUB + sub] : 0;
    __builtin_amdgcn_fence(__ATOMIC_RELEASE, "wavefront");
    __builtin_amdgcn_wave_barrier();
    const long long row0 = (long long)sub * SR;
    const int row1 = (int)(row0 + SR < n ? row0 + SR : n);
    for (int row = (int)row0; row < row1; row++) {
        const int rs = rp[row], re = rp[row + 1];
        for (int k0 = rs; k0 < re; k0 += 64) {
            const int k = k0 + lane;
            const bool active = k < re;
            const int col = active ? ci[k] : -1;
            const int cb = active ? col_to_cb(cut, col) : -1;
            const int prev = __shfl_up(cb, 1, 64);
            const bool head = lane == 0 || cb != prev;
            int hs = head ? lane : 0;
#pragma unroll
            for (int o = 1; o < 64; o <<= 1) {
                const int t = __shfl_up(hs, o, 64);
                if (lane >= o) hs = t > hs ? t : hs;
            }
            const int next = __shfl_down(cb, 1, 64);
            const bool tail = lane == 63 || next != cb;
            if (active) {
                const int base = cur[cb];
                const int rank = lane - hs;
                if (FILL) {
                    const int dest = base + rank;
                    if (pvi) pvi[dest] = vidx[k];
                    else pv[dest] = val[k];
                    pc[dest] = (u16)(col - col0[cb]);
                    pr[dest] = (u16)(row - (int)row0);
                }
                if (tail) cur[cb] = base + rank + 1;
            }
            __builtin_amdgcn_fence(__ATOMIC_RELEASE, "wavefront");
            __builtin_amdgcn_wave_barrier();
        }
    }
    if (!FILL)
        for (int c = lane; c < NCB; c += 64) bins[(size_t)c * NSUB + sub] = cur[c];
}

constexpr int kPbGroups = 32;
static_assert(kPbGroups <= 64, "one lane per group");
constexpr int kPbRpMax = 2047;
constexpr int kPbBucketMax = 2048;

__device__ __forceinline__ unsigned long long pb_pack(int cb, int pc, int pr)
{
    return ((unsigned long long)(unsigned)cb << 32) | ((unsigned long long)(unsigned)(pc & 0xffff) << 16) | (unsigned long long)(unsigned)(pr & 0xffff);
}

__global__ __launch_bounds__(64 * kPbBuildWaves) void k_pb_count(int n, const int *rp, const int *ci, PbCut cut, int NCB, int SR, int NSUB,
                                                                int *bins, int sub0, int sub1)
{
    extern __shared__ int lds_i[];
    const int wave = threadIdx.x >> 6, lane = threadIdx.x & 63;
    const int sub = sub0 + blockIdx.x * kPbBuildWaves + wave;
    if (sub >= sub1) return;
    int *cur = lds_i + (size_t)wave * NCB;
    for (int c = lane; c < NCB; c += 64) cur[c] = 0;
    __builtin_amdgcn_fence(__ATOMIC_RELEASE, "wavefront");
    __builtin_amdgcn_wave_barrier();
    const long long row0 = (long long)sub * SR;
    const int row1 = (int)(row0 + SR < n ? row0 + SR : n);
    const int e0 = row0 < n ? rp[row0] : rp[n], e1 = rp[row1];
    const double inv_cb = 1.0 / (double)cut.CB;
    for (int k0 = e0; k0 < e1; k0 += 256) {
        int col[4];
#pragma unroll
        for (int u = 0; u < 4; u++) col[u] = k0 + 64 * u + lane < e1 ? ci[k0 + 64 * u + lane] : -1;
#pragma unroll
        for (int u = 0; u < 4; u++)
            if (col[u] >= 0) atomicAdd(&cur[col_to_cb_fast(cut, inv_cb, col[u])], 1);
    }
    __builtin_amdgcn_fence(__ATOMIC_RELEASE, "wavefront");
    __builtin_amdgcn_wave_barrier();
    for (int c = lane; c < NCB; c += 64) bins[(size_t)c * NSUB + sub] = cur[c];
}

__global__ __launch_bounds__(64 * kPbBuildWaves) void k_pb_group(int n, const int *rp, const int *ci, const double *val,
                                                                const unsigned char *vidx, PbCut cut, const int *col0, int NCB,
                                                                int SR, const int *slen, int GB, int NG, int *gstart,
                                                                double *sval, unsigned char *sval8, unsigned long long *smeta,
                                                                int sub0, int sub1)
{
    __shared__ unsigned long long tab_all[kPbBuildWaves][kPbGroups];
    __shared__ int lrp_all[kPbBuildWaves][kPbRpMax + 1];
    const int wave = threadIdx.x >> 6, lane = threadIdx.x & 63;
    const int sub = sub0 + blockIdx.x * kPbBuildWaves + wave;
    if (sub >= sub1) return;
    unsigned long long *tab = tab_all[wave];
    int *lrp = lrp_all[wave];
    const int gshift = 31 - __builtin_clz(GB);
    const double inv_cb = 1.0 / (double)cut.CB;
    const long long row0 = (long long)sub * SR;
    const int row1 = (int)(row0 + SR < n ? row0 + SR : n);
    int cnt = 0;
    if (lane < NG) {
        const int *sl = slen + (size_t)sub * NCB;
        for (int c = lane * GB; c < (lane + 1) * GB && c < NCB; c++) cnt += sl[c];
    }
    int inc = cnt;
#pragma unroll
    for (int o = 1; o < 64; o <<= 1) {
        const int t = __shfl_up(inc, o, 64);
        if (lane >= o) inc += t;
    }
    const int e0 = row0 < n ? rp[row0] : rp[n], e1 = rp[row1];
    const int base = e0 - rp[0];
    const int total = __builtin_amdgcn_readlane(inc, 63);
    int run = base + inc - cnt;
    if (lane < NG) gstart[(size_t)sub * (NG + 1) + lane] = run;
    if (lane == 0) gstart[(size_t)sub * (NG + 1) + NG] = base + total;
    const int nrows = row1 - (int)row0;
    const bool rp_lds = nrows <= kPbRpMax;
    if (rp_lds)
        for (int i = lane; i <= nrows; i += 64) lrp[i] = rp[row0 + i];
    __builtin_amdgcn_fence(__ATOMIC_RELEASE, "wavefront");
    __builtin_amdgcn_wave_barrier();
    const bool one_piece = cut.chunks == 1 && cut.bpc >= NCB;
    int rbase = 0;
    int col_n = e0 + lane < e1 ? ci[e0 + lane] : -1;
    double val_n = 0.0;
    unsigned char vidx_n = 0;
    if (e0 + lane < e1) { if (sval8) vidx_n = vidx[e0 + lane]; else val_n = val[e0 + lane]; }
    for (int k0 = e0; k0 < e1; k0 += 64) {
        const int k = k0 + lane;
        const bool active = k < e1;
        const int col = col_n;
        const double v = val_n;
        const unsigned char vi = vidx_n;
        col_n = k + 64 < e1 ? ci[k + 64] : -1;
        if (k + 64 < e1) { if (sval8) vidx_n = vidx[k + 64]; else val_n = val[k + 64]; }
        int r = rbase;
        if (active) {
            if (rp_lds) { while (k >= lrp[r + 1]) r++; }
            else { while (k >= rp[row0 + r + 1]) r++; }
        }
        const int cb = active ? col_to_cb_fast(cut, inv_cb, col) : 0;
        const int g = cb >> gshift;
        int added;
        const int rank = wave_match_rank(tab, g, active, lane, NG, &added);
        const int dest = __shfl(run, g, 64) + rank;
        run += added;
        if (active) {
            if (sval8) sval8[dest] = vi;
            else sval[dest] = v;
            smeta[dest] = pb_pack(cb, col - (one_piece ? cb * cut.CB : col0[cb]), r);
        }
        const unsigned long long am = __ballot(active);
        rbase = __builtin_amdgcn_readlane(r, 63 - __builtin_clzll(am));
    }
}

constexpr int kPbScatterWaves = 4;
__global__ __launch_bounds__(64 * kPbScatterWaves) void k_pb_scatter(int NCB, int NSUB, const int *slen, const int *bins, int GB, int NG,
                                                                    const int *gstart, const double *sval, const unsigned char *sval8,
                                                                    const unsigned long long *smeta, double *pv, unsigned char *pvi,
                                                                    u16 *pc, u16 *pr, int sub0, int sub1)
{
    __shared__ unsigned raw_all[kPbScatterWaves][kPbBucketMax];
    __shared__ unsigned char cbl_all[kPbScatterWaves][kPbBucketMax];
    __shared__ u16 inv_all[kPbScatterWaves][kPbBucketMax];
    __shared__ unsigned long long tab_all[kPbScatterWaves][64];
    const int wave = threadIdx.x >> 6, lane = threadIdx.x & 63;
    const long long bucket = (long long)blockIdx.x * kPbScatterWaves + wave;
    const int sub = sub0 + (int)(bucket / NG), g = (int)(bucket % NG);
    if (sub >= sub1) return;
    u16 *inv = inv_all[wave];
    unsigned *raw = raw_all[wave];
    unsigned char *cbs = cbl_all[wave];
    const int start = gstart[(size_t)sub * (NG + 1) + g], len = gstart[(size_t)sub * (NG + 1) + g + 1] - start;
    if (len <= 0) return;
    const int cbid = g * GB + lane;
    const bool owner = lane < GB && cbid < NCB;
    const int cnt = owner ? slen[(size_t)sub * NCB + cbid] : 0;
    int inc = cnt;
#pragma unroll
    for (int o = 1; o < 64; o <<= 1) {
        const int t = __shfl_up(inc, o, 64);
        if (lane >= o) inc += t;
    }
    const int lbase = inc - cnt;
    const int gdst = owner ? bins[(size_t)cbid * NSUB + sub] : 0;
    const bool staged = len <= kPbBucketMax;
    int run = staged ? lbase : gdst;
    unsigned long long m_next = lane < len ? smeta[start + lane] : 0ULL;
    for (int k0 = 0; k0 < len; k0 += 64) {
        const int k = k0 + lane;
        const bool active = k < len;
        const unsigned long long m = m_next;
        m_next = k + 64 < len ? smeta[start + k + 64] : 0ULL;
        const int cbl = active ? (int)(m >> 32) - g * GB : 0;
        int added;
        const int rank = wave_match_rank(tab_all[wave], cbl, active, lane, GB, &added);
        const int r = __shfl(run, cbl, 64) + rank;
        run += added;
        if (active) {
            if (staged) { inv[r] = (u16)k; raw[k] = (unsigned)(m & 0xffffffffULL); cbs[k] = (unsigned char)cbl; }
            else {
                if (pvi) pvi[r] = sval8[start + k];
                else pv[r] = sval[start + k];
                pc[r] = (u16)((m >> 16) & 0xffff);
                pr[r] = (u16)(m & 0xffff);
            }
        }
    }
    if (!staged) return;
    __builtin_amdgcn_fence(__ATOMIC_RELEASE, "wavefront");
    __builtin_amdgcn_wave_barrier();
    for (int t0 = 0; t0 < len; t0 += 256) {
        unsigned m[4];
        double v[4];
        unsigned char vi[4];
        int dest[4];
#pragma unroll
        for (int u = 0; u < 4; u++) {
            const int t = t0 + 64 * u + lane;
            const bool active = t < len;
            const int loc = active ? (int)inv[t] : 0;
            m[u] = raw[loc];
            v[u] = 0.0;
            vi[u] = 0;
            if (active) { if (pvi) vi[u] = sval8[start + loc]; else v[u] = sval[start + loc]; }
            const int cbl = active ? (int)cbs[loc] : 0;
            dest[u] = __shfl(gdst, cbl, 64) + (t - __shfl(lbase, cbl, 64));
        }
#pragma unroll
        for (int u = 0; u < 4; u++) {
            if (t0 + 64 * u + lane < len) {
                if (pvi) pvi[dest[u]] = vi[u];
                else pv[dest[u]] = v[u];
                pc[dest[u]] = (u16)((m[u] >> 16) & 0xffff);
                pr[dest[u]] = (u16)(m[u] & 0xffff);
            }
        }
    }
}

__global__ __launch_bounds__(kBlock) void k_pb_colsum(int NSUB, const int *bins, int *colsum)
{
    __shared__ int red[kBlock / 64];
    const int *b = bins + (size_t)blockIdx.x * NSUB;
    int acc = 0;
    for (int i = threadIdx.x; i < NSUB; i += kBlock) acc += b[i];
#pragma unroll
    for (int o = 32; o > 0; o >>= 1) acc += __shfl_xor(acc, o, 64);
    if ((threadIdx.x & 63) == 0) red[threadIdx.x >> 6] = acc;
    __syncthreads();
    if (threadIdx.x == 0) {
        int t = 0;
        for (int w = 0; w < kBlock / 64; w++) t += red[w];
        colsum[blockIdx.x] = t;
    }
}

__device__ __forceinline__ int block_exclusive_scan(int v, int *lds_waves, int *total)
{
    const int lane = threadIdx.x & 63, wave = threadIdx.x >> 6;
    int inc = v;
#pragma unroll
    for (int o = 1; o < 64; o <<= 1) {
        const int t = __shfl_up(inc, o, 64);
        if (lane >= o) inc += t;
    }
    __syncthreads();
    if (lane == 63) lds_waves[wave] = inc;
    __syncthreads();
    int before = 0, all = 0;
    for (int w = 0; w < kBlock / 64; w++) {
        const int t = lds_waves[w];
        if (w < wave) before += t;
        all += t;
    }
    *total = all;
    return before + inc - v;
}

__global__ __launch_bounds__(kBlock) void k_pb_colscan(int NCB, const int *colsum, int *cstart, int align)
{
    __shared__ int lds_waves[kBlock / 64];
    int run = 0;
    for (int c0 = 0; c0 < NCB; c0 += kBlock) {
        const int c = c0 + threadIdx.x;
        const int v = c < NCB ? (colsum[c] + align - 1) / align * align : 0;
        int total;
        const int ex = block_exclusive_scan(v, lds_waves, &total);
        if (c < NCB) cstart[c] = run + ex;
        run += total;
    }
    if (threadIdx.x == 0) cstart[NCB] = run;
}

__global__ __launch_bounds__(kBlock) void k_pb_segscan(int NCB, int NSUB, const int *cstart, int *bins, int *sstart,
                                                       int *slen)
{
    __shared__ int lds_waves[kBlock / 64];
    const int c = blockIdx.x;
    int *b = bins + (size_t)c * NSUB;
    int run = cstart[c];
    for (int s0 = 0; s0 < NSUB; s0 += kBlock) {
        const int sidx = s0 + threadIdx.x;
        const int cnt = sidx < NSUB ? b[sidx] : 0;
        int total;
        const int ex = block_exclusive_scan(cnt, lds_waves, &total);
        if (sidx < NSUB) {
            const int start = run + ex;
            b[sidx] = start;
            sstart[(size_t)sidx * NCB + c] = start;
            slen[(size_t)sidx * NCB + c] = cnt;
        }
        run += total;
    }
}

static int round_blocks(int64_t n, int tile_max)
{
    int64_t m = (n + (int64_t)256 * tile_max - 1) / ((int64_t)256 * tile_max);
    if (m < 1) m = 1;
    return (int)(256 * m);
}

static void pb_scratch_free(PbBuild *b)
{
    if (b->smeta) CM_DROP(hipFree(b->smeta));
    if (b->gstart) CM_DROP(hipFree(b->gstart));
    b->smeta = nullptr;
    b->gstart = nullptr;
}

void pb_build_abort(PbBuild *b)
{
    pb_scratch_free(b);
    if (b->bins) CM_DROP(hipFree(b->bins));
    b->bins = nullptr;
    pb_free(&b->p);
}

int pb_build_begin(hipStream_t st, const Config &cfg, int n, int64_t n_cols, int64_t nnz, const int *rp, const int *ci,
                   const PbCols *cols, PbBuild *b)
{
    CM_TRY(pb_build_alloc(st, cfg, n, n_cols, nnz, cols, b));
    return pb_build_count(st, cfg, rp, ci, b);
}

int pb_build_alloc(hipStream_t st, const Config &cfg, int n, int64_t n_cols, int64_t nnz, const PbCols *cols, PbBuild *b)
{
    b->t0 = now_s();
    PbPlan &p = b->p;
    p = PbPlan();
    p.n = n;
    p.n_cols = n_cols;
    p.nnz = nnz;
    int local_slice = 0;
    if (cols && cols->per > 0 && cols->per < n_cols) {
        p.per = cols->per;
        p.chunks = cols->chunks < 1 ? 1 : cols->chunks > kPbMaxChunks ? kPbMaxChunks : cols->chunks;
        p.chunk_len = (p.per + p.chunks - 1) / p.chunks;
        p.bpc = (int)((p.chunk_len + kTileMax - 1) / kTileMax);
        p.CB = (int)((p.chunk_len + p.bpc - 1) / p.bpc);
        const int64_t slices = (n_cols + p.per - 1) / p.per;
        p.NCB = (int)(slices * p.chunks * p.bpc);
        local_slice = cols->rank;
    } else {
        p.per = n_cols;
        p.chunks = 1;
        p.chunk_len = n_cols;
        p.NCB = round_blocks(n_cols, kTileMax);
        p.CB = (int)((n_cols + p.NCB - 1) / p.NCB);
        p.NCB = (int)((n_cols + p.CB - 1) / p.CB);
        p.bpc = p.NCB;
    }
    const double seg_target = 48.0;
    double nsub_t = (double)nnz / ((double)p.NCB * seg_target);
    const bool few = nsub_t < 2560.0 && (double)n / 2048.0 * 8.0 * 8.0 <= 144.0 * 1024.0;
    double min_waves = few ? 2048.0 : 4096.0;
    if (cfg.pb_min_waves) min_waves = (double)cfg.pb_min_waves;
    if (nsub_t < min_waves) nsub_t = min_waves;
    if (nsub_t > (double)n / 16.0) nsub_t = (double)n / 16.0;
    if (nsub_t < 4.0) nsub_t = 4.0;
    p.NW = nsub_t >= 4096.0 ? 16 : nsub_t >= 2048.0 ? 8 : 4;
    int nrb = (int)(nsub_t / p.NW / 256.0 + 0.5) * 256;
    if (nrb < 256) nrb = 256;
    const int nrb_min = (int)(((int64_t)n + kTileMax - 1) / kTileMax);
    while (nrb < nrb_min) nrb += 256;
    if (nrb > kMaxParts) nrb = kMaxParts;
    p.NRB = nrb;
    p.RB = (int)(((int64_t)n + p.NRB - 1) / p.NRB);
    p.SR = (p.RB + p.NW - 1) / p.NW;
    if (p.SR < 1) p.SR = 1;
    p.RB = p.SR * p.NW;
    p.NRB = (int)(((int64_t)n + p.RB - 1) / p.RB);
    p.NSUB = p.NRB * p.NW;
    const double seg = (double)nnz / ((double)p.NCB * p.NSUB);
    p.LPS = seg <= 6.0 ? 16 : seg <= 22.0 ? 32 : 64;
    p.depth = few ? 16 : 4;
    if (cfg.pb_depth) p.depth = cfg.pb_depth;
    if (p.NRB > kMaxParts || p.CB > 65536 || p.SR > 65536 || (size_t)p.RB * 8 > 150 * 1024 ||
        sizeof(int) * (size_t)kPbBuildWaves * p.NCB > 150 * 1024) {
        set_error("pb_build: matrix shape outside the blocked kernel's limits");
        return CUDAMAT_ERR_ARG;
    }
    const size_t nbins = (size_t)p.NCB * p.NSUB;
    int *&bins = b->bins;
    bins = nullptr;
    int rc = CUDAMAT_OK;
    do {
        if ((rc = dalloc(&bins, nbins))) break;
        constexpr int align = kPbAlign;
        const size_t cap = (size_t)nnz + (size_t)(align - 1) * (size_t)p.NCB + 16;
        b->cap = cap;
        if ((rc = dalloc(&p.cstart, (size_t)p.NCB + 1))) break;
        if ((rc = dalloc(&p.col0, (size_t)p.NCB + 1))) break;
        if ((rc = dalloc(&p.order, (size_t)p.NCB))) break;
        {
            std::vector<int> h0((size_t)p.NCB + 1), ord;
            const int per_slice = p.chunks * p.bpc;
            for (int cb = 0; cb <= p.NCB; cb++) {
                const int64_t q = cb / per_slice, ch = (cb % per_slice) / p.bpc, k = cb % p.bpc;
                int64_t in_piece = k * (int64_t)p.CB;
                if (in_piece > p.chunk_len) in_piece = p.chunk_len;
                int64_t in_slice = ch * p.chunk_len + in_piece;
                if (in_slice > p.per) in_slice = p.per;
                int64_t c0 = q * p.per + in_slice;
                if (c0 > n_cols) c0 = n_cols;
                h0[(size_t)cb] = (int)c0;
            }
            ord.reserve((size_t)p.NCB);
            const int slices = p.NCB / per_slice;
            if (slices > 1) {
                for (int k = 0; k < per_slice; k++) ord.push_back(local_slice * per_slice + k);
                p.part_off[0] = 0;
                p.part_off[1] = (int)ord.size();
                for (int ch = 0; ch < p.chunks; ch++) {
                    for (int q = 0; q < slices; q++)
                        if (q != local_slice)
                            for (int k = 0; k < p.bpc; k++) ord.push_back((q * p.chunks + ch) * p.bpc + k);
                    p.part_off[ch + 2] = (int)ord.size();
                }
            } else {
                for (int cb = 0; cb < p.NCB; cb++) ord.push_back(cb);
                p.part_off[0] = 0;
                for (int ch = 0; ch <= p.chunks; ch++) p.part_off[ch + 1] = p.NCB;
            }
            if (hipMemcpyAsync(p.col0, h0.data(), sizeof(int) * h0.size(), hipMemcpyHostToDevice, st) != hipSuccess ||
                hipMemcpyAsync(p.order, ord.data(), sizeof(int) * ord.size(), hipMemcpyHostToDevice, st) != hipSuccess ||
                hipStreamSynchronize(st) != hipSuccess) { rc = CUDAMAT_ERR_HIP; set_error("pb column cut upload failed"); break; }
        }
        b->cut = PbCut{(int)p.per, p.chunks, (int)p.chunk_len, p.bpc, p.CB};
        if ((rc = dalloc(&p.sstart, nbins))) break;
        if ((rc = dalloc(&p.slen, nbins))) break;
        if ((rc = set_max_lds((const void *)k_pb_count))) break;
        if ((rc = set_max_lds((const void *)k_pb_rows<true>))) break;
        b->GB = 1;
        while (b->GB * kPbGroups < p.NCB) b->GB *= 2;
        b->NG = (p.NCB + b->GB - 1) / b->GB;
        b->fill_occ = cfg.pb_fill_occ;
        b->place = cfg.pb_place;
        b->place_max_seconds = 1e-3 * cfg.pb_place_max_ms;
        b->verbose = cfg.verbose != 0;
        b->report_classes = cfg.verbose >= 2;
        b->two_pass = cfg.pb_fill2 != 0 && nnz > 0 && nnz < 0x7fffffffLL && p.SR <= 65536 && b->GB <= 64;
        if (b->two_pass) {
            if (dalloc(&b->smeta, (size_t)nnz) != CUDAMAT_OK || dalloc(&b->gstart, (size_t)p.NSUB * (size_t)(b->NG + 1)) != CUDAMAT_OK) {
                if (b->smeta) CM_DROP(hipFree(b->smeta));
                b->smeta = nullptr;
                b->two_pass = false;
            }
        }
    } while (0);
    if (rc) pb_build_abort(b);
    return rc;
}

int pb_build_count(hipStream_t st, const Config &cfg, const int *rp, const int *ci, PbBuild *b)
{
    PbPlan &p = b->p;
    const int n = p.n;
    const int64_t nnz = p.nnz;
    int *bins = b->bins;
    constexpr int align = kPbAlign;
    int rc = CUDAMAT_OK;
    do {
        const PbCut cut = b->cut;
        const unsigned grid = (unsigned)((p.NSUB + kPbBuildWaves - 1) / kPbBuildWaves);
        const size_t lds = sizeof(int) * (size_t)kPbBuildWaves * p.NCB;
        hipLaunchKernelGGL(k_pb_count, dim3(grid), dim3(64 * kPbBuildWaves), lds, st, n, rp, ci, cut, p.NCB, p.SR, p.NSUB, bins, 0, p.NSUB);
        if (hipGetLastError() != hipSuccess) { rc = CUDAMAT_ERR_HIP; set_error("pb count launch failed"); break; }
        hipLaunchKernelGGL(k_pb_colsum, dim3(p.NCB), dim3(kBlock), 0, st, p.NSUB, bins, p.cstart);
        hipLaunchKernelGGL(k_pb_colscan, dim3(1), dim3(kBlock), 0, st, p.NCB, p.cstart, p.cstart, align);
        hipLaunchKernelGGL(k_pb_segscan, dim3(p.NCB), dim3(kBlock), 0, st, p.NCB, p.NSUB, p.cstart, bins, p.sstart, p.slen);
        int counted = -1;
        if (hipGetLastError() != hipSuccess ||
            hipMemcpyAsync(&counted, p.cstart + p.NCB, sizeof(int), hipMemcpyDeviceToHost, st) != hipSuccess ||
            hipStreamSynchronize(st) != hipSuccess) { rc = CUDAMAT_ERR_HIP; set_error("pb scan failed"); break; }
        if ((int64_t)counted < nnz || (int64_t)counted > nnz + (int64_t)(align - 1) * p.NCB) {
            rc = CUDAMAT_ERR_ARG; set_error("pb_build: counted %d entries, expected %lld", counted, (long long)nnz); break;
        }
        b->verbose = cfg.verbose != 0;
        b->report_classes = cfg.verbose >= 2;
    } while (0);
    if (rc) pb_build_abort(b);
    return rc;
}

__global__ __launch_bounds__(1024) void k_place_probe(const double2 *rd, double2 *wr, long n2)
{
    const long per = (n2 + gridDim.x - 1) / gridDim.x;
    const long lo = blockIdx.x * per, hi = lo + per < n2 ? lo + per : n2;
    for (long i = lo + threadIdx.x; i < hi; i += 1024) {
        const double2 v = rd[i];
        double2 o;
        o.x = v.x * 1.5;
        o.y = v.y + 1.0;
        wr[i] = o;
    }
}

struct PlaceTimer {
    hipStream_t st;
    hipEvent_t e0 = nullptr, e1 = nullptr;
    bool ok = false;
    int launches = 0;
    explicit PlaceTimer(hipStream_t s) : st(s) { ok = hipEventCreate(&e0) == hipSuccess && hipEventCreate(&e1) == hipSuccess; }
    ~PlaceTimer()
    {
        if (e0) CM_DROP(hipEventDestroy(e0));
        if (e1) CM_DROP(hipEventDestroy(e1));
    }
    float ms(const void *rd, void *wr, size_t bytes)
    {
        float t[12];
        int n = 0;
        while (ok && n < 12) {
            if (hipEventRecord(e0, st) != hipSuccess) { ok = false; break; }
            hipLaunchKernelGGL(k_place_probe, dim3(256), dim3(1024), 0, st, (const double2 *)rd, (double2 *)wr, (long)(bytes / 16));
            float x = 0.f;
            if (hipGetLastError() != hipSuccess || hipEventRecord(e1, st) != hipSuccess || hipEventSynchronize(e1) != hipSuccess ||
                hipEventElapsedTime(&x, e0, e1) != hipSuccess) { ok = false; break; }
            launches++;
            t[n++] = x;
            if (n >= 3) {
                const float lo = fminf(t[n - 1], fminf(t[n - 2], t[n - 3])), hi = fmaxf(t[n - 1], fmaxf(t[n - 2], t[n - 3]));
                if (hi <= 1.015f * lo) return lo;
            }
        }
        if (!ok || n < 3) return -1.f;
        return fminf(t[n - 1], fminf(t[n - 2], t[n - 3]));
    }
};

constexpr size_t kPlaceBlock = (size_t)2 << 30;
constexpr size_t kPlaceSample = (size_t)896 << 20;
constexpr size_t kPlaceSlab = (size_t)16 << 30;
constexpr size_t kPlaceMinBytes = (size_t)2 << 30;
constexpr size_t kPlaceMaxHeld = (size_t)96 << 30;
constexpr float kPlaceGap = 1.035f;

struct PlaceMemo {
    unsigned gen = ~0u;
    std::map<char *, int> cls;
    std::vector<char *> ref;
    float t_own = 0.f;
    float t_lo = 0.f, t_hi = 0.f;
    std::vector<std::pair<char *, float>> provisional;
    bool relabel = false;
    void reset() { cls.clear(); ref.clear(); provisional.clear(); t_own = t_lo = t_hi = 0.f; relabel = false; }
};
static std::mutex g_place_mu;
static std::map<int, PlaceMemo> g_place;

struct PlaceRun { size_t slab; size_t first, count; int cls; };

struct PlaceSlab {
    char *base = nullptr;
    size_t bytes = 0;
    char *b0 = nullptr;
    std::vector<int> cls;
    std::vector<char> taken;
};

static int place_class_of(PlaceTimer &tm, PlaceMemo &m, char *blk)
{
    auto it = m.cls.find(blk);
    if (it != m.cls.end()) return it->second;
    if (m.ref.empty()) {
        m.t_own = tm.ms(blk, blk + kPlaceBlock - kPlaceSample, kPlaceSample);
        if (m.t_own <= 0.f) return -1;
        m.ref.push_back(blk);
        m.cls[blk] = 0;
        return 0;
    }
    float t[3] = {0.f, 0.f, 0.f};
    const bool was_separated = m.t_hi >= kPlaceGap * m.t_lo && m.t_lo > 0.f;
    for (size_t k = 0; k < m.ref.size() && k < 3; k++) {
        t[k] = tm.ms(m.ref[k], blk + kPlaceBlock - kPlaceSample, kPlaceSample);
        if (t[k] <= 0.f) return -1;
        if (m.t_lo <= 0.f || t[k] < m.t_lo) m.t_lo = t[k];
        if (t[k] > m.t_hi) m.t_hi = t[k];
    }
    const bool separated = m.t_hi >= kPlaceGap * m.t_lo;
    int c = 0;
    if (separated) {
        const float mid = sqrtf(m.t_lo * m.t_hi);
        if (!was_separated) {
            for (auto p = m.provisional.begin(); p != m.provisional.end(); ++p)
                if (p->second <= mid) { m.cls.erase(p->first); m.relabel = true; }
            m.provisional.clear();
        }
        int slow = 0, arg = 0;
        for (size_t k = 0; k < m.ref.size() && k < 3; k++) {
            if (t[k] > mid) slow++;
            if (t[k] > t[arg]) arg = (int)k;
        }
        if (slow == 0 && m.ref.size() < 3) {
            c = (int)m.ref.size();
            m.ref.push_back(blk);
        } else {
            c = arg;
        }
    } else {
        m.provisional.push_back({blk, t[0]});
    }
    m.cls[blk] = c;
    return c;
}

static bool place_find(std::vector<PlaceSlab> &slabs, size_t need, int want, int avoid, PlaceRun *out)
{
    for (size_t si = 0; si < slabs.size(); si++) {
        PlaceSlab &sl = slabs[si];
        for (size_t i = 0; i + need <= sl.cls.size(); i++) {
            const int c = sl.cls[i];
            if (c < 0 || (want >= 0 && c != want) || c == avoid) continue;
            bool ok = true;
            for (size_t j = i; j < i + need && ok; j++) ok = !sl.taken[j] && sl.cls[j] == c;
            if (!ok) continue;
            for (size_t j = i; j < i + need; j++) sl.taken[j] = 1;
            *out = PlaceRun{si, i, need, c};
            return true;
        }
    }
    return false;
}

static int place_copy(hipStream_t st, bool verbose, double max_seconds, size_t b_vals, size_t b_idx, size_t b_prod, void **vals, void **pc, void **pr, void **prod, bool *placed,
                      PbPlan *report)
{
    *placed = false;
    if (!pool_enabled()) return CUDAMAT_OK;
    const double t0 = now_s();
    PlaceTimer tm(st);
    if (!tm.ok) return CUDAMAT_OK;
    int dev = 0;
    if (hipGetDevice(&dev) != hipSuccess) return CUDAMAT_OK;
    std::lock_guard<std::mutex> lock(g_place_mu);
    PlaceMemo &m = g_place[dev];
    if (m.gen != pool_generation()) {
        m.gen = pool_generation();
        m.reset();
    }
    const size_t gran = (size_t)2 << 20;
    auto up = [&](size_t x) { return (x + gran - 1) / gran * gran; };
    const size_t a_vals = up(b_vals), a_idx = up(b_idx), a_prod = up(b_prod);
    const size_t n_prod = (a_prod + kPlaceBlock - 1) / kPlaceBlock;
    const size_t n_vals = (a_vals + 2 * a_idx + kPlaceBlock - 1) / kPlaceBlock;
    const size_t slab_bytes = std::max(kPlaceSlab, (n_prod + n_vals + 1) * kPlaceBlock);
    std::vector<PlaceSlab> slabs;
    PlaceRun r_prod{}, r_vals{};
    float check_ms = 0.f;
    bool found = false, verified = false;
    size_t held = 0;
    while (!found) {
        if (held + slab_bytes > kPlaceMaxHeld || now_s() - t0 > max_seconds) break;
        PlaceSlab sl;
        if (hipMalloc(&sl.base, slab_bytes) != hipSuccess) { CM_DROP(hipGetLastError()); break; }
        sl.bytes = slab_bytes;
        held += slab_bytes;
        char *seg = nullptr;
        size_t blk_bytes = 0;
        if (!pool_segment_of(sl.base, &seg, &blk_bytes)) { slabs.push_back(sl); break; }
        sl.bytes = blk_bytes;
        sl.b0 = seg + ((size_t)(sl.base - seg) + kPlaceBlock - 1) / kPlaceBlock * kPlaceBlock;
        const size_t whole = sl.b0 + kPlaceBlock <= sl.base + sl.bytes ? (size_t)(sl.base + sl.bytes - sl.b0) / kPlaceBlock : 0;
        bool verdicts = true;
        for (size_t i = 0; i < whole && verdicts; i++) {
            const int c = place_class_of(tm, m, sl.b0 + i * kPlaceBlock);
            verdicts = c >= 0;
            sl.cls.push_back(c);
        }
        sl.taken.assign(sl.cls.size(), 0);
        slabs.push_back(sl);
        if (verdicts && m.relabel) {
            m.relabel = false;
            for (auto &q : slabs)
                for (size_t i = 0; i < q.cls.size() && verdicts; i++) {
                    q.cls[i] = place_class_of(tm, m, q.b0 + i * kPlaceBlock);
                    verdicts = q.cls[i] >= 0;
                }
        }
        if (!verdicts) break;
        for (size_t a = 0; a < m.ref.size() && !found; a++) {
            for (auto &q : slabs) std::fill(q.taken.begin(), q.taken.end(), 0);
            found = place_find(slabs, n_prod, (int)a, -1, &r_prod) && place_find(slabs, n_vals, -1, (int)a, &r_vals);
        }
    }
    if (found) {
        struct Keep { size_t slab; char *p; size_t bytes; void **out; };
        char *p_vals = slabs[r_vals.slab].b0 + r_vals.first * kPlaceBlock, *p_prod = slabs[r_prod.slab].b0 + r_prod.first * kPlaceBlock;
        char *p_idx = p_vals + a_vals;
        const size_t s_idx = r_vals.slab;
        const Keep keeps[4] = {{r_vals.slab, p_vals, a_vals, vals}, {s_idx, p_idx, a_idx, pc}, {s_idx, p_idx + a_idx, a_idx, pr}, {r_prod.slab, p_prod, a_prod, prod}};
        for (size_t si = 0; si < slabs.size(); si++) {
            PlaceSlab &sl = slabs[si];
            std::vector<std::pair<char *, bool>> marks, cuts;
            bool base_kept = false;
            for (const Keep &k : keeps) {
                if (k.slab != si) continue;
                marks.push_back({k.p, true});
                marks.push_back({k.p + k.bytes, false});
                base_kept = base_kept || k.p == sl.base;
            }
            std::sort(marks.begin(), marks.end());
            for (size_t k = 0; k < marks.size(); k++) {
                if (k + 1 < marks.size() && marks[k + 1].first == marks[k].first) { marks[k + 1].second = marks[k].second || marks[k + 1].second; continue; }
                if (marks[k].first > sl.base && marks[k].first < sl.base + sl.bytes) cuts.push_back(marks[k]);
            }
            bool ok = true;
            for (size_t k = cuts.size(); k-- > 0 && ok;) ok = pool_split(sl.base, (size_t)(cuts[k].first - sl.base));
            if (!ok) { found = false; break; }
            if (!base_kept) CM_DROP(hipFree(sl.base));
            for (auto &c : cuts)
                if (!c.second) CM_DROP(hipFree(c.first));
            sl.base = nullptr;
        }
        if (found) {
            for (const Keep &k : keeps) *k.out = k.p;
            const float t_check = tm.ms(p_vals, p_prod + kPlaceBlock - kPlaceSample, kPlaceSample);
            *placed = true;
            verified = t_check > 0.f && m.t_hi >= kPlaceGap * m.t_lo && t_check < sqrtf(m.t_lo * m.t_hi);
            check_ms = t_check;
        }
    }
    for (auto &sl : slabs)
        if (sl.base) CM_DROP(hipFree(sl.base));
    std::string seen;
    for (auto &sl : slabs) {
        for (int c : sl.cls) seen += c < 0 ? '?' : (char)('0' + c % 10);
        seen += ' ';
    }
    report->placed = *placed && verified ? 1 : 0;
    report->place_check_ms = check_ms;
    report->place_fast_ms = m.t_lo;
    report->place_slow_ms = m.t_hi;
    report->place_slabs = (int)slabs.size();
    report->place_seconds = now_s() - t0;
    snprintf(report->place_classes, sizeof(report->place_classes), "%s| check %.3f ms, groups %.3f / %.3f ms", seen.c_str(), check_ms, m.t_lo, m.t_hi);
    if (verbose) {
        fprintf(stderr, "[cudamat] pb placement: %s; %zu slab(s) of %.0f GB, blocks by class: %s, %d timed launches, %.1f ms (one block read + written: %.3f ms)\n",
                *placed && verified ? "product stream in a memory class of its own, values and indices in another" : *placed ? "an arrangement was cut, but its own check timed slow (classes misjudged?)" : "no arrangement found: arrays allocated one after the other",
                slabs.size(), (double)slab_bytes / (double)((size_t)1 << 30), seen.c_str(), tm.launches, (now_s() - t0) * 1e3, m.t_own);
    }
    return CUDAMAT_OK;
}

int pb_build_values(hipStream_t st, PbBuild *b, const ValDict *vd)
{
    PbPlan &p = b->p;
    const size_t cap = b->cap;
    const bool dict = vd && vd->n > 0;
    int rc = CUDAMAT_OK;
    do {
        if (!p.P && b->place > 0 && sizeof(double) * cap >= kPlaceMinBytes) {
            void *v = nullptr, *c = nullptr, *r = nullptr, *pp = nullptr;
            bool placed = false;
            if ((rc = place_copy(st, b->verbose, b->place_max_seconds, dict ? cap : sizeof(double) * cap, sizeof(u16) * cap, sizeof(double) * cap, &v, &c, &r, &pp, &placed, &p))) break;
            if (placed) {
                if (dict) p.pvi = (unsigned char *)v; else p.pv = (double *)v;
                p.pc = (u16 *)c;
                p.pr = (u16 *)r;
                p.P = (double *)pp;
            }
        }
        if (dict) {
            if (!p.pvi && (rc = dalloc(&p.pvi, cap))) break;
            if (hipMemsetAsync(p.pvi, 0, cap, st) != hipSuccess) { rc = CUDAMAT_ERR_HIP; break; }
            p.dict = vd->dict;
            p.ndict = vd->n;
        } else {
            if (!p.pv && (rc = dalloc(&p.pv, cap))) break;
            if (hipMemsetAsync(p.pv, 0, sizeof(double) * cap, st) != hipSuccess) { rc = CUDAMAT_ERR_HIP; break; }
        }
        if (p.P && p.pc && p.pr && p.pc_zeroed) break;
        if (!p.pc && (rc = dalloc(&p.pc, cap))) break;
        if (!p.pr && (rc = dalloc(&p.pr, cap))) break;
        if (!p.P && (rc = dalloc(&p.P, cap))) break;
        if (kPbAlign > 1 && hipMemsetAsync(p.pc, 0, sizeof(u16) * cap, st) != hipSuccess) { rc = CUDAMAT_ERR_HIP; break; }
        p.pc_zeroed = true;
    } while (0);
    if (rc) pb_build_abort(b);
    return rc;
}

int pb_build_fill(hipStream_t st, PbBuild *b, const int *rp, const int *ci, const double *val, const ValDict *vd, int sub0, int sub1)
{
    PbPlan &p = b->p;
    if (sub1 > p.NSUB) sub1 = p.NSUB;
    if (sub1 <= sub0) return CUDAMAT_OK;
    const unsigned grid = (unsigned)((sub1 - sub0 + kPbBuildWaves - 1) / kPbBuildWaves);
    const unsigned char *vidx = p.pvi ? vd->idx : (const unsigned char *)nullptr;
    const int cfg_fill_occ = b->fill_occ;
    if (b->two_pass) {
        size_t pad = 0;
        if (cfg_fill_occ > 0) {
            const size_t per_wg = (size_t)(160 * 1024) / (size_t)((cfg_fill_occ + kPbBuildWaves - 1) / kPbBuildWaves);
            pad = per_wg > 40 * 1024 ? per_wg - 40 * 1024 : 0;
            if (pad > 64 * 1024) pad = 64 * 1024;
        }
        hipLaunchKernelGGL(k_pb_group, dim3(grid), dim3(64 * kPbBuildWaves), pad, st, p.n, rp, ci, val, vidx, b->cut, p.col0, p.NCB, p.SR,
                           p.slen, b->GB, b->NG, b->gstart, p.P, p.pvi ? (unsigned char *)p.P : (unsigned char *)nullptr, b->smeta, sub0, sub1);
        const long long buckets = (long long)(sub1 - sub0) * b->NG;
        hipLaunchKernelGGL(k_pb_scatter, dim3((unsigned)((buckets + kPbScatterWaves - 1) / kPbScatterWaves)), dim3(64 * kPbScatterWaves), 0, st,
                           p.NCB, p.NSUB, p.slen, b->bins, b->GB, b->NG, b->gstart, p.P, p.pvi ? (const unsigned char *)p.P : (const unsigned char *)nullptr,
                           b->smeta, p.pv, p.pvi, p.pc, p.pr, sub0, sub1);
    } else {
        const size_t lds = sizeof(int) * (size_t)kPbBuildWaves * p.NCB;
        hipLaunchKernelGGL(k_pb_rows<true>, dim3(grid), dim3(64 * kPbBuildWaves), lds, st, p.n, rp, ci, val, b->cut, p.col0,
                           p.NCB, p.SR, p.NSUB, b->bins, p.pv, p.pc, p.pr, vidx, p.pvi, sub0, sub1);
    }
    if (hipGetLastError() != hipSuccess) { set_error("pb fill launch failed"); pb_build_abort(b); return CUDAMAT_ERR_HIP; }
    return CUDAMAT_OK;
}

static void pb_print_plan(const PbPlan &p)
{
    const size_t nbins = (size_t)p.NCB * p.NSUB;
    std::vector<int> hl(nbins);
    if (hipMemcpy(hl.data(), p.slen, sizeof(int) * nbins, hipMemcpyDeviceToHost) != hipSuccess) return;
    long long hist[7] = {0, 0, 0, 0, 0, 0, 0}, in_long = 0;
    for (int v : hl) {
        hist[v == 0 ? 0 : v <= 8 ? 1 : v <= 24 ? 2 : v <= 48 ? 3 : v <= 64 ? 4 : v <= 128 ? 5 : 6]++;
        if (v > 64) in_long += v;
    }
    fprintf(stderr, "[cudamat] pb arrays: pv %p pvi %p pc %p pr %p P %p sstart %p slen %p cstart %p\n", (void *)p.pv, (void *)p.pvi, (void *)p.pc,
            (void *)p.pr, (void *)p.P, (void *)p.sstart, (void *)p.slen, (void *)p.cstart);
    fprintf(stderr, "[cudamat] pb plan: %d x %lld, nnz %lld, NCB %d (CB %d), NSUB %d (NW %d, SR %d), LPS %d, depth %d; segments: "
                    "empty %lld, 1-8 %lld, 9-24 %lld, 25-48 %lld, 49-64 %lld, 65-128 %lld, >128 %lld; %.1f %% of the entries in "
                    "segments longer than a wave\n",
            p.n, (long long)p.n_cols, (long long)p.nnz, p.NCB, p.CB, p.NSUB, p.NW, p.SR, p.LPS, p.depth, hist[0], hist[1], hist[2], hist[3],
            hist[4], hist[5], hist[6], 100.0 * (double)in_long / (double)(p.nnz > 0 ? p.nnz : 1));
}

static void place_report_classes(hipStream_t st, const PbPlan &p, size_t cap)
{
    if (!pool_enabled()) return;
    PlaceTimer tm(st);
    if (!tm.ok) return;
    int dev = 0;
    if (hipGetDevice(&dev) != hipSuccess) return;
    std::lock_guard<std::mutex> lock(g_place_mu);
    PlaceMemo &m = g_place[dev];
    if (m.gen != pool_generation()) { m.gen = pool_generation(); m.reset(); }
    std::vector<char *> slabs;
    std::vector<char *> scratch(3, nullptr);
    for (int k = 0; k < 4 && !(scratch[0] && scratch[1] && scratch[2]); k++) {
        char *base = nullptr;
        if (hipMalloc(&base, kPlaceSlab) != hipSuccess) { CM_DROP(hipGetLastError()); break; }
        slabs.push_back(base);
        char *seg = nullptr;
        size_t bytes = 0;
        if (!pool_segment_of(base, &seg, &bytes)) break;
        char *b0 = seg + ((size_t)(base - seg) + kPlaceBlock - 1) / kPlaceBlock * kPlaceBlock;
        for (char *q = b0; q + kPlaceBlock <= base + bytes; q += kPlaceBlock) {
            const int c = place_class_of(tm, m, q);
            if (c >= 0 && c < 3 && !scratch[c]) scratch[c] = q;
        }
    }
    struct Arr { const char *name; const char *ptr; size_t bytes; };
    const Arr arrs[4] = {{"values", p.pv ? (const char *)p.pv : (const char *)p.pvi, p.pv ? sizeof(double) * cap : cap},
                         {"col idx", (const char *)p.pc, sizeof(u16) * cap}, {"row idx", (const char *)p.pr, sizeof(u16) * cap}, {"products", (const char *)p.P, sizeof(double) * cap}};
    for (const Arr &a : arrs) {
        std::string line;
        for (size_t off = 0; off + kPlaceSample <= a.bytes; off += kPlaceSample) {
            int cls = -1;
            float worst = 0.f;
            for (int k = 0; k < 3; k++) {
                if (!scratch[k]) continue;
                const float t = tm.ms(a.ptr + off, scratch[k] + kPlaceBlock - kPlaceSample, kPlaceSample);
                if (t > worst) { worst = t; cls = k; }
            }
            line += cls < 0 || !(m.t_hi >= kPlaceGap * m.t_lo) || worst <= sqrtf(m.t_lo * m.t_hi) ? '?' : (char)('0' + cls);
        }
        fprintf(stderr, "[cudamat] pb classes: %-8s at %p, per %zu MB: %s\n", a.name, (const void *)a.ptr, kPlaceSample >> 20, line.c_str());
    }
    for (char *q : slabs) CM_DROP(hipFree(q));
}

int pb_build_end(hipStream_t st, PbBuild *b, PbPlan *out)
{
    if (hipStreamSynchronize(st) != hipSuccess) { set_error("pb fill failed"); pb_build_abort(b); return CUDAMAT_ERR_HIP; }
    if (b->verbose) pb_print_plan(b->p);
    if (b->report_classes && sizeof(double) * b->cap >= kPlaceMinBytes) place_report_classes(st, b->p, b->cap);
    pb_scratch_free(b);
    CM_DROP(hipFree(b->bins));
    b->bins = nullptr;
    b->p.build_seconds = now_s() - b->t0;
    *out = b->p;
    b->p = PbPlan();
    return CUDAMAT_OK;
}

int pb_build(hipStream_t st, const Config &cfg, int n, int64_t n_cols, int64_t nnz, const int *rp, const int *ci,
             const double *val, PbPlan *out, const PbCols *cols, const ValDict *vd)
{
    PbBuild b;
    CM_TRY(pb_build_begin(st, cfg, n, n_cols, nnz, rp, ci, cols, &b));
    CM_TRY(pb_build_values(st, &b, vd));
    CM_TRY(pb_build_fill(st, &b, rp, ci, val, vd, 0, b.p.NSUB));
    return pb_build_end(st, &b, out);
}


__global__ __launch_bounds__(kP1Threads) void k_pb_phase1(const double *x, const int *col0, const int *list,
                                                          const int *cstart, const double *pv, const u16 *pc,
                                                          double *P, const LoopState *st, int cb0)
{
    extern __shared__ __attribute__((aligned(16))) double xs[];
    if (st && st->state != 0) return;
    const int cb = list ? list[blockIdx.x] : (int)blockIdx.x + cb0;
    const int s = cstart[cb], e = cstart[cb + 1];
    if (s >= e) return;
    const int c0 = col0[cb], cn = col0[cb + 1] - c0;
    for (int i = threadIdx.x; i < cn; i += kP1Threads) xs[i] = x[c0 + i];
    __syncthreads();
    constexpr int STEP = 2 * kP1Threads;
    const int k0 = (s & ~1) + 2 * (int)threadIdx.x;
    for (int k = k0; k < e; k += 4 * STEP) {
        double2 v[4];
        ushort2 c[4];
        bool full[4];
#pragma unroll
        for (int u = 0; u < 4; u++) {
            const int kk = k + u * STEP;
            full[u] = kk >= s && kk + 1 < e;
            if (full[u]) {
                v[u] = *(const double2 *)(pv + kk);
                c[u] = *(const ushort2 *)(pc + kk);
            }
        }
#pragma unroll
        for (int u = 0; u < 4; u++) {
            const int kk = k + u * STEP;
            if (full[u]) {
                double2 o;
                o.x = v[u].x * xs[c[u].x];
                o.y = v[u].y * xs[c[u].y];
                *(double2 *)(P + kk) = o;
            } else {
                if (kk >= s && kk < e) P[kk] = pv[kk] * xs[pc[kk]];
                if (kk + 1 >= s && kk + 1 < e) P[kk + 1] = pv[kk + 1] * xs[pc[kk + 1]];
            }
        }
    }
}

__global__ __launch_bounds__(kP1Threads) void k_pb_phase1_dict(const double *x, const int *col0, const int *list,
                                                               const int *cstart, const unsigned char *pvi, const u16 *pc,
                                                               const double *dict, int cb_doubles, double *P,
                                                               const LoopState *st, int cb0)
{
    extern __shared__ __attribute__((aligned(16))) double xs[];
    if (st && st->state != 0) return;
    const int cb = list ? list[blockIdx.x] : (int)blockIdx.x + cb0;
    const int s = cstart[cb], e = cstart[cb + 1];
    if (s == e) return;
    double *dv = xs + cb_doubles;
    const int c0 = col0[cb], cn = col0[cb + 1] - c0;
    for (int i = threadIdx.x; i < cn; i += kP1Threads) xs[i] = x[c0 + i];
    if (threadIdx.x < kDictMax) dv[threadIdx.x] = dict[threadIdx.x];
    __syncthreads();
    constexpr int U = kP1Unroll, STEP = 2 * kP1Threads, CH = U * STEP;
    const int a0 = (s + 1) & ~1;
    if (threadIdx.x == 0 && s < a0) P[s] = dv[pvi[s]] * xs[pc[s]];
    int kb = a0;
    const int t2 = 2 * (int)threadIdx.x;
    for (; kb + CH <= e; kb += CH) {
        const int k = kb + t2;
        u16 iv[U];
        unsigned cv[U];
#pragma unroll
        for (int u = 0; u < U; u++) {
            iv[u] = *(const u16 *)(pvi + k + u * STEP);
            cv[u] = *(const unsigned *)(pc + k + u * STEP);
        }
#pragma unroll
        for (int u = 0; u < U; u++) {
            double2 o;
            o.x = dv[iv[u] & 0xffu] * xs[cv[u] & 0xffffu];
            o.y = dv[iv[u] >> 8] * xs[cv[u] >> 16];
            *(double2 *)(P + k + u * STEP) = o;
        }
    }
    {
        const int m = e > kb ? (e - kb) / STEP : 0;
        const int k = kb + t2;
        u16 iv[U - 1];
        unsigned cv[U - 1];
#pragma unroll
        for (int u = 0; u < U - 1; u++) {
            if (u < m) {
                iv[u] = *(const u16 *)(pvi + k + u * STEP);
                cv[u] = *(const unsigned *)(pc + k + u * STEP);
            }
        }
#pragma unroll
        for (int u = 0; u < U - 1; u++) {
            if (u < m) {
                double2 o;
                o.x = dv[iv[u] & 0xffu] * xs[cv[u] & 0xffffu];
                o.y = dv[iv[u] >> 8] * xs[cv[u] >> 16];
                *(double2 *)(P + k + u * STEP) = o;
            }
        }
        const int kr = k + m * STEP;
        if (kr + 1 < e) {
            const u16 iw = *(const u16 *)(pvi + kr);
            const unsigned cw = *(const unsigned *)(pc + kr);
            double2 o;
            o.x = dv[iw & 0xffu] * xs[cw & 0xffffu];
            o.y = dv[iw >> 8] * xs[cw >> 16];
            *(double2 *)(P + kr) = o;
        } else if (kr < e) {
            P[kr] = dv[pvi[kr]] * xs[pc[kr]];
        }
    }
}

struct Pb2Args {
    int n, NCB, SR;
    const int *sstart, *slen;
    const double *P;
    const u16 *pr;
    const double *d, *xd;
    double alpha, beta;
    double *y;
    int dot;
    const double *w;
    double *parts;
    const LoopState *st;
    int strict;
};

__device__ __forceinline__ void pb_seg_add(double *my, int r, double p, bool on, int lane, int group_first, bool strict)
{
    if (!strict) {
        if (on) unsafeAtomicAdd(&my[r], p);
        return;
    }
    const int r_prev = __shfl_up(r, 1, 64);
    const int on_prev = __shfl_up((int)on, 1, 64);
    const bool d1 = on && lane > group_first && on_prev && r_prev == r;
    if (on && !d1) unsafeAtomicAdd(&my[r], p);
    if (__ballot(d1) == 0) return;
    const bool d2 = d1 && __shfl_up((int)d1, 1, 64) != 0;
    if (d1 && !d2) unsafeAtomicAdd(&my[r], p);
    if (__ballot(d2) == 0) return;
    int head = d1 ? 0 : lane;
#pragma unroll
    for (int o = 1; o < 64; o <<= 1) {
        const int t = __shfl_up(head, o, 64);
        if (lane >= o) head = t > head ? t : head;
    }
    const int rank = on ? lane - head : 0;
    for (int q = 2; __ballot(on && rank >= q); q++)
        if (on && rank == q) unsafeAtomicAdd(&my[r], p);
}

__global__ __launch_bounds__(64) void k_lds_order_probe(int *mismatch)
{
    __shared__ double acc[64], val[64], start[64];
    const int lane = threadIdx.x;
    unsigned long long z = 0x9E3779B97F4A7C15ULL * (unsigned long long)(lane + 1);
    int bad = 0;
    for (int pat = 0; pat < 4; pat++) {
        const int addr = pat == 0 ? 0 : pat == 1 ? lane >> 3 : pat == 2 ? (lane & 31) : (lane & 3);
        const int naddr = pat == 0 ? 1 : pat == 1 ? 8 : pat == 2 ? 32 : 4;
        for (int rep = 0; rep < 4; rep++) {
            z ^= z >> 30; z *= 0xBF58476D1CE4E5B9ULL; z ^= z >> 27; z *= 0x94D049BB133111EBULL; z ^= z >> 31;
            const double v = 0.5 + (double)(z >> 11) * 0x1.0p-53;
            const double c = 3.0 + (double)((z * 0x9E3779B97F4A7C15ULL) >> 11) * 0x1.0p-53;
            val[lane] = v;
            start[lane] = c;
            acc[lane] = c;
            __syncthreads();
            unsafeAtomicAdd(&acc[addr], v);
            __syncthreads();
            if (lane < naddr) {
#pragma clang fp contract(off)
                double e = start[lane];
                for (int l = 0; l < 64; l++) {
                    const int al = pat == 0 ? 0 : pat == 1 ? l >> 3 : pat == 2 ? (l & 31) : (l & 3);
                    if (al == lane) e = e + val[l];
                }
                if (__double_as_longlong(e) != __double_as_longlong(acc[lane])) bad = 1;
            }
            __syncthreads();
        }
    }
    if (bad) atomicOr(mismatch, 1);
}

int pb_strict_for(cudamat_ctx *ctx, int *strict)
{
    *strict = 1;
    if (ctx->cfg.pb_strict) return CUDAMAT_OK;
    if (ctx->lds_lane_order < 0) {
        int *flag = (int *)ctx->scratch, h = 1;
        CM_HIP(hipMemsetAsync(flag, 0, sizeof(int), ctx->stream));
        hipLaunchKernelGGL(k_lds_order_probe, dim3(1), dim3(64), 0, ctx->stream, flag);
        CM_HIP(hipGetLastError());
        CM_HIP(hipMemcpyAsync(&h, flag, sizeof(int), hipMemcpyDeviceToHost, ctx->stream));
        CM_HIP(hipStreamSynchronize(ctx->stream));
        if (ctx->cfg.pb_probe_fail) h = 1;
        ctx->lds_lane_order = h ? 0 : 1;
        if (h || ctx->cfg.verbose)
            fprintf(stderr, "[cudamat] LDS order probe: equal addresses of one ds_add_f64 are %s -> blocked SpMV phase 2 in its %s form\n",
                    h ? (ctx->cfg.pb_probe_fail ? "reported NOT in lane order (PB_PROBE_FAIL)" : "NOT served in lane order")
                      : "served in lane order", h ? "architected-order (PB_STRICT)" : "default");
    }
    *strict = ctx->lds_lane_order ? 0 : 1;
    return CUDAMAT_OK;
}

template <int NW, int LPS, int DEPTH>
__global__ __launch_bounds__(64 * NW) void k_pb_phase2(Pb2Args a)
{
    extern __shared__ __attribute__((aligned(16))) double yt[];
    if (a.st && a.st->state != 0) return;
    const int wave = threadIdx.x >> 6, lane = threadIdx.x & 63;
    const int sub = blockIdx.x * NW + wave;
    double *my = yt + (size_t)wave * a.SR;
    for (int i = lane; i < a.SR; i += 64) my[i] = 0.0;
    __builtin_amdgcn_fence(__ATOMIC_RELEASE, "wavefront");
    __builtin_amdgcn_wave_barrier();
    const int *ss = a.sstart + (size_t)sub * a.NCB;
    const int *sl = a.slen + (size_t)sub * a.NCB;
    for (int cb0 = 0; cb0 < a.NCB; cb0 += 64) {
        const int c = cb0 + lane;
        const int mys = c < a.NCB ? ss[c] : 0;
        const int myl = c < a.NCB ? sl[c] : 0;
        const int lim = a.NCB - cb0 < 64 ? a.NCB - cb0 : 64;
        const bool grouped = LPS < 64 && !__any(myl > LPS);
        if (!grouped) {
            for (int j = 0; j < lim; j += DEPTH) {
                int s[DEPTH], l[DEPTH];
                double pv4[DEPTH];
                int r4[DEPTH];
#pragma unroll
                for (int u = 0; u < DEPTH; u++) {
                    s[u] = __builtin_amdgcn_readlane(mys, (j + u) & 63);
                    l[u] = __builtin_amdgcn_readlane(myl, (j + u) & 63);
                }
#pragma unroll
                for (int u = 0; u < DEPTH; u++) {
                    const bool on = lane < l[u];
                    pv4[u] = on ? a.P[s[u] + lane] : 0.0;
                    r4[u] = on ? (int)a.pr[s[u] + lane] : 0;
                }
#pragma unroll
                for (int u = 0; u < DEPTH; u++) {
                    pb_seg_add(my, r4[u], pv4[u], lane < l[u], lane, 0, a.strict != 0);
                    for (int off0 = 64; off0 < l[u]; off0 += 64) {
                        const int off = off0 + lane;
                        const bool on = off < l[u];
                        pb_seg_add(my, on ? (int)a.pr[s[u] + off] : 0, on ? a.P[s[u] + off] : 0.0, on, lane, 0, a.strict != 0);
                    }
                }
            }
        } else {
            constexpr int G = 64 / LPS;
            const int g = lane / LPS, li = lane % LPS;
            for (int j = 0; j < lim; j += DEPTH * G) {
                int s[DEPTH], l[DEPTH];
                double pv4[DEPTH];
                int r4[DEPTH];
#pragma unroll
                for (int u = 0; u < DEPTH; u++) {
                    const int cbi = j + u * G + g;
                    s[u] = __shfl(mys, cbi & 63, 64);
                    l[u] = cbi < 64 ? __shfl(myl, cbi & 63, 64) : 0;
                }
#pragma unroll
                for (int u = 0; u < DEPTH; u++) {
                    const bool on = li < l[u];
                    pv4[u] = on ? a.P[s[u] + li] : 0.0;
                    r4[u] = on ? (int)a.pr[s[u] + li] : 0;
                }
#pragma unroll
                for (int u = 0; u < DEPTH; u++) {
                    if (!a.strict) {
                        if (li < l[u]) unsafeAtomicAdd(&my[r4[u]], pv4[u]);
                    } else {
#pragma unroll
                        for (int gg = 0; gg < G; gg++)
                            pb_seg_add(my, r4[u], pv4[u], g == gg && li < l[u], lane, gg * LPS, true);
                    }
                }
            }
        }
    }
    __builtin_amdgcn_fence(__ATOMIC_RELEASE, "wavefront");
    __builtin_amdgcn_wave_barrier();
    double acc0 = 0.0, acc1 = 0.0;
    const long long row0 = (long long)sub * a.SR;
    for (int i = lane; i < a.SR && row0 + i < a.n; i += 64) {
#pragma clang fp contract(off)
        const int row = (int)(row0 + i);
        double sum = my[i];
        if (a.d) {
            const double dx = a.d[row] * a.xd[row];
            sum = sum + dx;
        }
        double out = a.alpha * sum;
        if (a.beta != 0.0) {
            const double by = a.beta * a.y[row];
            out = out + by;
        }
        a.y[row] = out;
        if (a.dot) {
            acc0 += out * a.w[row];
            acc1 += out * out;
        }
    }
    if (a.dot) {
        double *red = yt + (size_t)NW * a.SR;
#pragma unroll
        for (int o = 32; o > 0; o >>= 1) {
            acc0 += __shfl_xor(acc0, o, 64);
            acc1 += __shfl_xor(acc1, o, 64);
        }
        if (lane == 0) {
            red[2 * wave] = acc0;
            red[2 * wave + 1] = acc1;
        }
        __syncthreads();
        if (threadIdx.x == 0) {
            double t0 = 0.0, t1 = 0.0;
            for (int q = 0; q < NW; q++) {
                t0 += red[2 * q];
                t1 += red[2 * q + 1];
            }
            a.parts[2 * blockIdx.x] = t0;
            a.parts[2 * blockIdx.x + 1] = t1;
        }
    }
}

int launch_pb_check(hipStream_t st, const SpmvArgs &a)
{
    if (a.loop.st && a.check == CHECK_HALF) CM_TRY(launch_check(st, a.loop, a.half, CHECK_HALF));
    return CUDAMAT_OK;
}

static int launch_pb_phase1_blocks(hipStream_t st, const PbPlan &p, const SpmvArgs &a, const int *list, int first, int last)
{
    if (last <= first) return CUDAMAT_OK;
    if (p.pvi) {
        CM_TRY(set_max_lds((const void *)k_pb_phase1_dict));
        const int cbd = (p.CB + 1) & ~1;
        hipLaunchKernelGGL(k_pb_phase1_dict, dim3(last - first), dim3(kP1Threads), sizeof(double) * (size_t)(cbd + kDictMax), st, a.x,
                           p.col0, list ? list + first : (const int *)nullptr, p.cstart, p.pvi, p.pc, p.dict, cbd, p.P, a.loop.st,
                           list ? 0 : first);
        CM_HIP(hipGetLastError());
        return CUDAMAT_OK;
    }
    CM_TRY(set_max_lds((const void *)k_pb_phase1));
    hipLaunchKernelGGL(k_pb_phase1, dim3(last - first), dim3(kP1Threads), sizeof(double) * (size_t)p.CB, st, a.x, p.col0,
                       list ? list + first : (const int *)nullptr, p.cstart, p.pv, p.pc, p.P, a.loop.st, list ? 0 : first);
    CM_HIP(hipGetLastError());
    return CUDAMAT_OK;
}

int launch_pb_phase1(hipStream_t st, const PbPlan &p, const SpmvArgs &a, int part)
{
    if (part < 0) return launch_pb_phase1_blocks(st, p, a, nullptr, 0, p.NCB);
    return launch_pb_phase1_blocks(st, p, a, p.order, p.part_off[part], p.part_off[part + 1]);
}

int launch_spmv_pb(hipStream_t st, const PbPlan &p, const SpmvArgs &a)
{
    CM_TRY(launch_pb_check(st, a));
    CM_TRY(launch_pb_phase1(st, p, a, -1));
    return launch_pb_phase2(st, p, a);
}

int launch_pb_phase2(hipStream_t st, const PbPlan &p, const SpmvArgs &a)
{
    Pb2Args b;
    b.n = p.n; b.NCB = p.NCB; b.SR = p.SR;
    b.sstart = p.sstart; b.slen = p.slen;
    b.P = p.P; b.pr = p.pr;
    b.d = a.d; b.xd = a.xd;
    b.alpha = a.alpha; b.beta = a.beta;
    b.y = a.y; b.dot = a.dot; b.w = a.w; b.parts = a.parts;
    b.st = a.loop.st;
    b.strict = a.pb_strict;
    const size_t lds = sizeof(double) * ((size_t)p.NW * p.SR + 2 * (size_t)p.NW);
#define CM_P2D(NWV, LPSV, DV)                                                                             \
    do {                                                                                                  \
        CM_TRY(set_max_lds((const void *)k_pb_phase2<NWV, LPSV, DV>));                                   \
        hipLaunchKernelGGL((k_pb_phase2<NWV, LPSV, DV>), dim3(p.NRB), dim3(64 * NWV), lds, st, b);       \
    } while (0)
#define CM_P2(NWV, LPSV)                                                                                  \
    do {                                                                                                  \
        if (p.depth >= 16) CM_P2D(NWV, LPSV, 16);                                                         \
        else if (p.depth >= 8) CM_P2D(NWV, LPSV, 8);                                                      \
        else CM_P2D(NWV, LPSV, 4);                                                                        \
    } while (0)
#define CM_P2_LPS(NWV)                                           \
    do {                                                         \
        if (p.LPS == 16) CM_P2(NWV, 16);                         \
        else if (p.LPS == 32) CM_P2(NWV, 32);                    \
        else CM_P2(NWV, 64);                                     \
    } while (0)
    switch (p.NW) {
    case 4:  CM_P2_LPS(4); break;
    case 8:  CM_P2_LPS(8); break;
    default: CM_P2_LPS(16); break;
    }
#undef CM_P2_LPS
#undef CM_P2
#undef CM_P2D
    CM_HIP(hipGetLastError());
    return CUDAMAT_OK;
}

}
```

### cuda_mat_amd/host/selftest.cpp

```cpp
#include <cstdio>
#include <cstdlib>
#include <cstring>
#include <string>
#include <vector>

#include "Matrix.h"
#include "cudamat.h"

static int failures = 0;
#define EXPECT(cond)                                                       \
    do {                                                                   \
        if (!(cond)) { std::fprintf(stderr, "FAILED %s:%d: %s\n", __FILE__, __LINE__, #cond); failures++; } \
    } while (0)

static std::string write_file(const std::string &dir, const char *name, const char *text)
{
    const std::string path = dir + "/" + name;
    FILE *f = std::fopen(path.c_str(), "w");
    if (f) { std::fputs(text, f); std::fclose(f); }
    return path;
}

static int load(const std::string &path, bool csr, int *m, int *n, int *nnz, double **v, int **r, int **c)
{
    return cudamat_load_mtx(path.c_str(), csr ? 1 : 0, m, n, nnz, v, r, c);
}

int main(int argc, char **argv)
{
    if (argc < 3) { std::fprintf(stderr, "usage: selftest <golden dir> <scratch dir>\n"); return 2; }
    const std::string gold = argv[1], tmp = argv[2];
    int m, n, nnz;
    double *v;
    int *r, *c;
    struct { const char *file; int n, nnz; } fixtures[] = {{"mat3.mtx", 3, 8}, {"mat900.mtx", 900, 7744}, {"mat10000.mtx", 10000, 49600}};
    for (auto &fx : fixtures) {
        for (int csr = 0; csr < 2; csr++) {
            v = nullptr; r = c = nullptr;
            EXPECT(load(gold + "/" + fx.file, csr, &m, &n, &nnz, &v, &r, &c) == CUDAMAT_OK);
            EXPECT(m == fx.n && n == fx.n && nnz == fx.nnz);
            if (v) {
                const int *ptr = csr ? r : c;
                EXPECT(ptr[0] == 1 && ptr[fx.n] == 1 + fx.nnz);
            }
            cudamat_host_free(v); cudamat_host_free(r); cudamat_host_free(c);
        }
    }
    v = nullptr; r = c = nullptr;
    EXPECT(load(gold + "/vec3_d.mtx", true, &m, &n, &nnz, &v, &r, &c) == CUDAMAT_OK);
    if (v) {
        double dense[3] = {-1, -1, -1};
        cudamat_to_dense_vector(m, nnz, v, r, dense);
        EXPECT(dense[0] == 1.0 && dense[1] == 0.0 && dense[2] == 1.0);
    }
    cudamat_host_free(v); cudamat_host_free(r); cudamat_host_free(c);
    const char *bad[][2] = {
        {"huge.mtx", "%%MatrixMarket matrix coordinate real general\n3 3 2147483647\n1 1 1\n"},
        {"hugesym.mtx", "%%MatrixMarket matrix coordinate real symmetric\n3 3 1500000000\n1 1 1\n"},
        {"widecol.mtx", "%%MatrixMarket matrix coordinate real general\n3 3 2\n1 1 1\n2 7 2\n"},
        {"widerow.mtx", "%%MatrixMarket matrix coordinate real general\n3 3 2\n1 1 1\n9 2 2\n"},
        {"dup.mtx", "%%MatrixMarket matrix coordinate real general\n3 3 3\n1 1 1\n1 1 2\n3 3 1\n"},
        {"short.mtx", "%%MatrixMarket matrix coordinate real general\n3 3 3\n1 1 1\n2 2 2\n"},
        {"both.mtx", "%%MatrixMarket matrix coordinate real general\n3 3 2\n0 1 1\n3 3 2\n"},
        {"empty.mtx", ""},
    };
    for (auto &b : bad) {
        v = nullptr; r = c = nullptr;
        EXPECT(load(write_file(tmp, b[0], b[1]), true, &m, &n, &nnz, &v, &r, &c) != CUDAMAT_OK);
    }
    EXPECT(load(tmp + "/does_not_exist.mtx", true, &m, &n, &nnz, &v, &r, &c) != CUDAMAT_OK);
    v = nullptr; r = c = nullptr;
    EXPECT(load(write_file(tmp, "skew.mtx", "%%MatrixMarket matrix coordinate real skew-symmetric\n3 3 2\n2 1 5\n3 3 7\n"), true,
                &m, &n, &nnz, &v, &r, &c) == CUDAMAT_OK);
    EXPECT(nnz == 3);
    if (v && nnz == 3) EXPECT(v[0] == -5.0 && v[1] == 5.0 && v[2] == 7.0);
    cudamat_host_free(v); cudamat_host_free(r); cudamat_host_free(c);

    Matrix<double> A(2, 3, {1, 2, 3, 4, 5, 6});
    Matrix<double> At = Matrix<double>::transpose(A);
    EXPECT(At.n == 3 && At.m == 2 && At.get(2, 0) == 3 && At.get(0, 1) == 4);
    Matrix<double> G = mul(A, At);
    EXPECT(G.get(0, 0) == 14 && G.get(0, 1) == 32 && G.get(1, 1) == 77);
    EXPECT(mul(Matrix<double>::identity(2), A).get(1, 2) == 6);
    EXPECT(Matrix<double>::without_column(A, 1).get(1, 1) == 6 && A.column(2).get(1, 0) == 6 && A.row(1).get(0, 0) == 4);
    EXPECT(Matrix<double>::is_zero(Matrix<double>(2, 2, 0.0), 1e-12) && !Matrix<double>::is_zero(A, 1e-12));
    std::vector<double> val;
    std::vector<int> rp, ci;
    EXPECT(Matrix<double>(2, 2, {4, 0, -1, 4}).to_csr(1, &val, &rp, &ci) == 3 && rp[2] == 4 && ci[1] == 1);
    bool threw = false;
    try { A.get(2, 0); } catch (const std::out_of_range &) { threw = true; }
    EXPECT(threw);
    if (failures == 0) std::printf("SELFTEST_OK\n");
    return failures ? 1 : 0;
}
```

### include/cudamat.h

```cpp
#ifndef CUDAMAT_H
#define CUDAMAT_H

#include <stdint.h>

#ifdef __cplusplus
extern "C" {
#endif

#define CUDAMAT_VERSION 1

#define CUDAMAT_OK              0
#define CUDAMAT_ERR_HIP         1
#define CUDAMAT_ERR_ARG         2
#define CUDAMAT_ERR_ZERO_PIVOT  3
#define CUDAMAT_ERR_NOMEM       4
#define CUDAMAT_ERR_IO          5
#define CUDAMAT_ERR_COMM        6

#define CUDAMAT_PRECOND_NONE    0
#define CUDAMAT_PRECOND_ILU0    1
#define CUDAMAT_PRECOND_BLOCK_ILU0 2

#define CUDAMAT_LOOP_PBICGSTAB  0
#define CUDAMAT_LOOP_PBICGSTAB2 1
#define CUDAMAT_LOOP_PIPELINED  2

#define CUDAMAT_FLAG_DEBUG      1
#define CUDAMAT_FLAG_PROFILE    2
#define CUDAMAT_FLAG_NO_EXIT    4
#define CUDAMAT_FLAG_X0_ONES    8

typedef struct cudamat_ctx cudamat_ctx;
typedef struct cudamat_solver cudamat_solver;

typedef struct cudamat_stats {
    int iters;
    int half_exit;
    int converged;
    int breakdown;
    double nrm0;
    double nrm;
    double t_analysis;
    double t_factor;
    double t_solve;
    double t_total;
    double ms_spmv;     int n_spmv;
    double ms_trsv;     int n_trsv;
    int n_levels_l;     int n_levels_u;
    int trsv_form;
    int trsv_fallbacks;
    int n_gather;       int n_allreduce;
    double ms_gather;   double ms_gather_exposed;   double ms_allreduce;
    int overlapped;
    int loop_form;
    double gather_fraction;
    double ms_spmv_alone;
    int loop_fallbacks;
    int restarts;
    double t_upload;
    double t_setup;
    double t_tune;
    int spmv_mode;
    int plan_reused;
    int trsv_groups_l;     int trsv_groups_u;
} cudamat_stats;

typedef int (*cudamat_allgather_fn)(void *user, const double *send, double *recv, int64_t count);
typedef int (*cudamat_allreduce_fn)(void *user, double *buf, int count);
typedef int (*cudamat_gather_part_fn)(void *user, const double *send, double *recv, int64_t stride,
                                      int64_t offset, int64_t count);
typedef int (*cudamat_gather_window_fn)(void *user, const double *send, double *recv, int64_t stride,
                                        const int64_t *send_off, const int64_t *send_cnt,
                                        const int64_t *recv_off, const int64_t *recv_cnt);
typedef struct cudamat_comm {
    int rank;
    int world;
    void *user;
    cudamat_allgather_fn allgather;
    cudamat_allreduce_fn allreduce;
    cudamat_gather_part_fn gather_part;
    void *comm_stream;
    cudamat_allreduce_fn allreduce_side;
    void *reduce_stream;
    cudamat_gather_window_fn gather_window;
} cudamat_comm;

#define CUDAMAT_RCCL_ID_BYTES 384
int cudamat_rccl_available(void);
int cudamat_rccl_unique_id(void *id);
int cudamat_rccl_comm_create(cudamat_ctx *ctx, const void *id, int rank, int world, cudamat_comm *out);
int cudamat_rccl_comm_destroy(cudamat_comm *comm);
int cudamat_rccl_comm_abort(cudamat_comm *comm);

int cudamat_comm_dry_create(cudamat_ctx *ctx, int rank, int world, cudamat_comm *out);
int cudamat_comm_dry_destroy(cudamat_comm *comm);

int         cudamat_version(void);
const char *cudamat_last_error(void);
int         cudamat_device_count(int *count);

int cudamat_ctx_create(int device, void *stream, cudamat_ctx **out);
int cudamat_ctx_destroy(cudamat_ctx *ctx);
int cudamat_ctx_set_option(cudamat_ctx *ctx, const char *name, const char *value);
int cudamat_ctx_reset_options(cudamat_ctx *ctx);
const char *cudamat_options_help(void);
int cudamat_option_check(const char *name, const char *value);
int cudamat_ctx_sync(cudamat_ctx *ctx);
int cudamat_ctx_stream(cudamat_ctx *ctx, void **stream);

int cudamat_malloc(cudamat_ctx *ctx, size_t bytes, void **dev);
int cudamat_free(cudamat_ctx *ctx, void *dev);
int cudamat_h2d(cudamat_ctx *ctx, void *dev, const void *host, size_t bytes);
int cudamat_d2h(cudamat_ctx *ctx, void *host, const void *dev, size_t bytes);
int cudamat_d2d(cudamat_ctx *ctx, void *dst, const void *src, size_t bytes);
int cudamat_memset(cudamat_ctx *ctx, void *dev, int value, size_t bytes);

int cudamat_timer_create(cudamat_ctx *ctx, void **timer);
int cudamat_timer_start(cudamat_ctx *ctx, void *timer);
int cudamat_timer_stop(cudamat_ctx *ctx, void *timer);
int cudamat_timer_elapsed_ms(cudamat_ctx *ctx, void *timer, double *ms);
int cudamat_timer_destroy(cudamat_ctx *ctx, void *timer);

int cudamat_spmv(cudamat_ctx *ctx, int n, const int *rowptr, const int *colidx,
                 const double *val, int base, double alpha, const double *x,
                 const double *d, double beta, double *y);
int cudamat_dot(cudamat_ctx *ctx, int64_t n, const double *x, const double *y, double *out_dev);
int cudamat_nrm2(cudamat_ctx *ctx, int64_t n, const double *x, double *out_dev);
int cudamat_axpy(cudamat_ctx *ctx, int64_t n, double alpha, const double *x, double *y);
int cudamat_scal(cudamat_ctx *ctx, int64_t n, double alpha, double *x);

int cudamat_solver_create(cudamat_ctx *ctx, int n_local, int64_t n_cols, int64_t nnz,
                          const int *rowptr, const int *colidx, const double *val,
                          int base, cudamat_solver **out);
int cudamat_solver_create_host(cudamat_ctx *ctx, int n_local, int64_t n_cols, int64_t nnz,
                               const int *rowptr_host, const int *colidx_host, const double *val_host,
                               int base, cudamat_solver **out);
int cudamat_solver_destroy(cudamat_solver *s);
int cudamat_solver_set_shift(cudamat_solver *s, const double *d);
int cudamat_solver_ilu0(cudamat_solver *s);
int cudamat_solver_block_ilu0(cudamat_solver *s);
int cudamat_solver_ilu0_values(cudamat_solver *s, double *out_dev);
int cudamat_solver_ilu0_nnz(cudamat_solver *s, int64_t *count);
int cudamat_solver_trsv_form(cudamat_solver *s, int *form);
int cudamat_solver_precond_apply(cudamat_solver *s, const double *in, double *out);
int cudamat_solver_set_comm(cudamat_solver *s, const cudamat_comm *comm);
int cudamat_solver_spmv_mode(cudamat_solver *s, int *mode);
int cudamat_solver_value_dict(cudamat_solver *s, int *distinct);
int cudamat_solver_spmv_kernel(cudamat_solver *s, char *name, int cap);
int cudamat_solver_placement(cudamat_solver *s, int *placed, int *slabs, double *seconds, char *classes, int cap);
int cudamat_solver_spmv(cudamat_solver *s, const double *x_local, double *y_local);
int cudamat_solver_solve(cudamat_solver *s, const double *b, double *x, int precond,
                         int loop, int maxit, double tol, int flags, cudamat_stats *st);
int cudamat_solver_history(cudamat_solver *s, double *hist_host, int cap, int *count);

int cudamat_solver_spmm(cudamat_solver *s, int nrhs, const double *X, int ldx, double *Y, int ldy);
int cudamat_solver_solve_many(cudamat_solver *s, int nrhs, const double *B, int ldb, double *X, int ldx, int precond,
                              int loop, int maxit, double tol, int flags, cudamat_stats *st, int *form);
int cudamat_solver_precond_apply_many(cudamat_solver *s, int nrhs, const double *In, int ldin, double *Out, int ldout);
int cudamat_solver_trsm_kernel(cudamat_solver *s, int nrhs, char *name, int cap);
int cudamat_solver_spmm_shifts(cudamat_solver *s, int nrhs, const double *X, int ldx, const double *D, int ldd, double *Y,
                               int ldy);
int cudamat_solver_solve_shifts(cudamat_solver *s, int nrhs, const double *D, int ldd, const double *B, int ldb, double *X,
                                int ldx, int precond, int loop, int maxit, double tol, int flags, cudamat_stats *st, int *form);
int cudamat_solver_history_col(cudamat_solver *s, int col, double *hist_host, int cap, int *count);

int cudamat_solve(int n, int nnz, const double *A, const int *iA, const int *jA,
                  const double *d, const double *x0, const double *b, int precond,
                  int loop, int maxit, double tol, int debug, double *x,
                  cudamat_stats *st);

int cudamat_solve_many(int n, int nnz, const double *A, const int *iA, const int *jA, const double *d, int nrhs,
                       const double *B, int ldb, const double *x0, double *X, int ldx, int precond, int loop, int maxit,
                       double tol, cudamat_stats *st, int *form);

int cudamat_solve_shifts(int n, int nnz, const double *A0, const int *iA0, const int *jA0, int nrhs, const double *D, int ldd,
                         const double *B, int ldb, const double *x0, double *X, int ldx, int loop, int maxit, double tol,
                         cudamat_stats *st, int *form);

int cudamat_plan_cache_clear(void);

int cudamat_pool_trim(void);
int cudamat_mem_info(int device, size_t *driver_free, size_t *driver_total, size_t *pool_free);

int cudamat_solve_sharded(int ngpu, int n, int nnz, const double *A, const int *iA, const int *jA,
                          const double *d, const double *x0, const double *b, int precond,
                          int loop, int maxit, double tol, int debug, double *x,
                          cudamat_stats *st);

int64_t cudamat_poisson5_nnz(int nx, int ny);
int cudamat_gen_poisson5(cudamat_ctx *ctx, int nx, int ny, int64_t row0, int64_t row1,
                         int base, int *rowptr, int *colidx, double *val);
int cudamat_rand_row_nnz(int64_t n, int per_row);
int cudamat_gen_rand_rows(cudamat_ctx *ctx, int64_t n, int per_row, uint64_t seed,
                          int64_t row0, int64_t row1, int base, int *rowptr,
                          int *colidx, double *val);
int cudamat_gen_xstar(cudamat_ctx *ctx, int64_t i0, int64_t i1, uint64_t seed, double *x);

int cudamat_load_mtx(const char *filename, int csr_format, int *m, int *n, int *nnz,
                     double **val, int **row, int **col);
void cudamat_host_free(void *p);
void cudamat_to_dense_vector(int n, int nnz, const double *A, const int *IA, double *out);

#ifdef __cplusplus
}
#endif
#endif
```

Baseline: 182.6.

## Store blocked-SpMV row indices in one byte with per-segment high-bit boundaries

The blocked two-phase SpMV copy now keeps one byte of row index per entry instead of two. The high two bits of each row are recovered from per-segment boundary positions, packed into the segment length word, or into a side table for segments longer than 127 entries. This cuts the index bytes streamed from HBM per nonzero in phase 2. In exchange it adds a counting pass at build time, decode arithmetic in the inner loop, more template instantiations, and applies only when sub-blocks have at most 1024 rows and few long segments.

```diff
diff --git a/cuda_mat_amd/_lib.py b/cuda_mat_amd/_lib.py
--- a/cuda_mat_amd/_lib.py
+++ b/cuda_mat_amd/_lib.py
@@ -112,6 +112,7 @@
     "cudamat_solver_spmv_mode": (C.c_int, [_P, C.POINTER(C.c_int)]),
     "cudamat_solver_spmv_kernel": (C.c_int, [_P, C.c_char_p, C.c_int]),
     "cudamat_solver_value_dict": (C.c_int, [_P, C.POINTER(C.c_int)]),
+    "cudamat_solver_pb_geometry": (C.c_int, [_P] + [C.POINTER(C.c_int)] * 5),
     "cudamat_solver_placement": (C.c_int, [_P, C.POINTER(C.c_int), C.POINTER(C.c_int), C.POINTER(C.c_double), C.c_char_p, C.c_int]),
     "cudamat_solver_spmv": (C.c_int, [_P, _P, _P]),
     "cudamat_solver_solve": (C.c_int, [_P, _P, _P, C.c_int, C.c_int, C.c_int, C.c_double, C.c_int,
diff --git a/cuda_mat_amd/api.py b/cuda_mat_amd/api.py
--- a/cuda_mat_amd/api.py
+++ b/cuda_mat_amd/api.py
@@ -384,6 +384,13 @@
         check(_lib.lib().cudamat_solver_placement(self.h, C.byref(placed), C.byref(slabs), C.byref(sec), buf, 256))
         return {"placed": placed.value, "slabs": slabs.value, "seconds": sec.value, "blocks_by_class": buf.value.decode().strip()}
 
+    def pb_geometry(self):
+        v = [C.c_int() for _ in range(5)]
+        check(_lib.lib().cudamat_solver_pb_geometry(self.h, *[C.byref(x) for x in v]))
+        if v[4].value == 0:
+            return None
+        return dict(zip(("NCB", "NSUB", "SR", "LPS", "row_bytes"), (x.value for x in v)))
+
     def value_dict(self):
         m = C.c_int()
         check(_lib.lib().cudamat_solver_value_dict(self.h, C.byref(m)))
diff --git a/cuda_mat_amd/csrc/config.cpp b/cuda_mat_amd/csrc/config.cpp
--- a/cuda_mat_amd/csrc/config.cpp
+++ b/cuda_mat_amd/csrc/config.cpp
@@ -52,6 +52,7 @@
     OPT_FLAG("EARLY_ANALYSIS", early_analysis, "0: cudamat_solve analyses the ILU(0) levels after the upload of the values instead of beside it"),
     OPT_INT("PB_FILL_OCC", pb_fill_occ, 0, 64, "resident waves per CU of the two-pass fill's first pass (0: 8; probing)"),
     OPT_FLAG("PB_FILL2", pb_fill2, "0: fill the blocked copy with the single-pass scatter kernel (rounds 1-4) instead of the two-pass partition"),
+    OPT_FLAG("PB_ROWS8", pb_rows8, "0: the blocked copy keeps two bytes of row index per entry; 1 (default): one byte, the row's high bits in the segment's length word, where a sub-block has <= 1024 rows and at most 4 segments per sub-block exceed 127 entries (spmv_pb.hip, pb_rows.h)"),
     OPT_INT("PB_PLACE", pb_place, 0, 2, "blocked copy of a large matrix: 1 (default): a resident solver's product stream is placed in a memory class of its own, values and indices in another (timed probe of the device's memory classes, 10-35 ms per copy: spmv_pb.hip); 2: the drop-in calls place theirs as well; 0: arrays wherever the allocator puts them"),
     OPT_INT("PB_PLACE_MAX_MS", pb_place_max_ms, 0, 60000, "PB_PLACE: what the search for an arrangement may take before the arrays are allocated as ever (ms; the slabs it allocates included -- 0.3 ms per 16 GB on most boxes, 2 s on some)"),
     OPT_FLAG("PB_PROBE_FAIL", pb_probe_fail, "1 (tests): treat the run-time LDS-order probe as failed, i.e. select the architected-order phase 2"),
diff --git a/cuda_mat_amd/csrc/config.h b/cuda_mat_amd/csrc/config.h
--- a/cuda_mat_amd/csrc/config.h
+++ b/cuda_mat_amd/csrc/config.h
@@ -20,6 +20,7 @@
     int early_analysis = 1;
     int pb_fill_occ = 0;
     int pb_fill2 = 1;
+    int pb_rows8 = 1;
     int pb_place = 1;
     int pb_place_max_ms = 300;
     int pb_probe_fail = 0;
diff --git a/cuda_mat_amd/csrc/pb_rows.h b/cuda_mat_amd/csrc/pb_rows.h
--- /dev/null
+++ b/cuda_mat_amd/csrc/pb_rows.h
@@ -0,0 +1,57 @@
+#pragma once
+
+#if defined(__HIPCC__)
+#define CM_PB_HD __host__ __device__
+#else
+#define CM_PB_HD
+#endif
+
+namespace cm {
+
+constexpr int kPbRows8MaxSR = 1024;
+constexpr int kPbRows8Short = 127;
+constexpr int kPbRows8MaxLen = 65535;
+constexpr int kPbRows8LongPerSub = 4;
+
+struct PbSeg { int len, b1, b2, b3; };
+
+CM_PB_HD inline bool pb_seg_is_long(int word) { return word < 0; }
+CM_PB_HD inline int pb_seg_long_index(int word) { return word & 0x7fffffff; }
+
+CM_PB_HD inline unsigned long long pb_seg_count_add(int hi)
+{
+    return 1ULL | (hi < 1 ? 1ULL << 16 : 0ULL) | (hi < 2 ? 1ULL << 32 : 0ULL) | (hi < 3 ? 1ULL << 48 : 0ULL);
+}
+CM_PB_HD inline PbSeg pb_seg_counted(unsigned long long c)
+{
+    return PbSeg{(int)(c & 0xffffULL), (int)(c >> 16 & 0xffffULL), (int)(c >> 32 & 0xffffULL), (int)(c >> 48)};
+}
+
+CM_PB_HD inline int pb_seg_word_short(const PbSeg &s)
+{
+    return (int)((unsigned)s.len | (unsigned)s.b1 << 8 | (unsigned)s.b2 << 16 | (unsigned)s.b3 << 24);
+}
+CM_PB_HD inline int pb_seg_word_long(int index) { return (int)(0x80000000u | (unsigned)index); }
+
+CM_PB_HD inline PbSeg pb_seg_of(int word, const int *longtab)
+{
+    if (pb_seg_is_long(word)) {
+        const int *q = longtab + 4 * (long long)pb_seg_long_index(word);
+        return PbSeg{q[0], q[1], q[2], q[3]};
+    }
+    const unsigned w = (unsigned)word;
+    return PbSeg{(int)(w & 0xffu), (int)(w >> 8 & 0xffu), (int)(w >> 16 & 0xffu), (int)(w >> 24)};
+}
+
+CM_PB_HD inline int pb_seg_len(int word, bool narrow, const int *longtab)
+{
+    if (!narrow) return word;
+    return pb_seg_is_long(word) ? longtab[4 * (long long)pb_seg_long_index(word)] : (word & 0xff);
+}
+
+CM_PB_HD inline int pb_seg_row(int lo8, const PbSeg &s, int pos)
+{
+    return lo8 + 256 * ((pos >= s.b1 ? 1 : 0) + (pos >= s.b2 ? 1 : 0) + (pos >= s.b3 ? 1 : 0));
+}
+
+}
diff --git a/cuda_mat_amd/csrc/solver.hip b/cuda_mat_amd/csrc/solver.hip
--- a/cuda_mat_amd/csrc/solver.hip
+++ b/cuda_mat_amd/csrc/solver.hip
@@ -793,6 +793,21 @@
     return CUDAMAT_OK;
 }
 
+extern "C" int cudamat_solver_pb_geometry(cudamat_solver *s, int *ncb, int *nsub, int *sr, int *lps, int *row_bytes)
+{
+    CM_ARG(s, "null pointer");
+    CM_HIP(hipSetDevice(s->ctx->device));
+    CM_TRY(ensure_work(s));
+    CM_TRY(ensure_spmv_mode(s));
+    const PbPlan *q = s->spmv_mode == 1 && s->pb.P ? &s->pb : nullptr;
+    if (ncb) *ncb = q ? q->NCB : 0;
+    if (nsub) *nsub = q ? q->NSUB : 0;
+    if (sr) *sr = q ? q->SR : 0;
+    if (lps) *lps = q ? q->LPS : 0;
+    if (row_bytes) *row_bytes = q ? q->row_bytes : 0;
+    return CUDAMAT_OK;
+}
+
 extern "C" int cudamat_solver_spmv_kernel(cudamat_solver *s, char *name, int cap)
 {
     CM_ARG(s && name && cap > 0, "null pointer");
diff --git a/cuda_mat_amd/csrc/spmv_pb.h b/cuda_mat_amd/csrc/spmv_pb.h
--- a/cuda_mat_amd/csrc/spmv_pb.h
+++ b/cuda_mat_amd/csrc/spmv_pb.h
@@ -1,6 +1,7 @@
 #pragma once
 #include "kernels.h"
 #include "valdict.h"
+#include "pb_rows.h"
 
 namespace cm {
 
@@ -32,7 +33,10 @@
     const double *dict = nullptr;
     int ndict = 0;
     unsigned short *pc = nullptr;
-    unsigned short *pr = nullptr;
+    void *pr = nullptr;
+    int row_bytes = 2;
+    int *longseg = nullptr;
+    int nlong = 0;
     double *P = nullptr;
     int *cstart = nullptr;
     int *col0 = nullptr;
@@ -55,6 +59,9 @@
 struct PbBuild {
     PbPlan p;
     int *bins = nullptr;
+    int *segmax = nullptr;
+    bool counted = false;
+    int rows8 = 1;
     PbCut cut{};
     size_t cap = 0;
     double t0 = 0.0;
diff --git a/cuda_mat_amd/csrc/spmv_pb.hip b/cuda_mat_amd/csrc/spmv_pb.hip
--- a/cuda_mat_amd/csrc/spmv_pb.hip
+++ b/cuda_mat_amd/csrc/spmv_pb.hip
@@ -4,6 +4,7 @@
 #include <string>
 #include <vector>
 
+#include "pb_rows.h"
 #include "spmv_pb.h"
 
 namespace cm {
@@ -29,7 +30,7 @@
 
 void pb_free(PbPlan *p)
 {
-    void *ptrs[] = {p->pv, p->pvi, p->pc, p->pr, p->P, p->cstart, p->col0, p->sstart, p->slen, p->order};
+    void *ptrs[] = {p->pv, p->pvi, p->pc, p->pr, p->P, p->cstart, p->col0, p->sstart, p->slen, p->order, p->longseg};
     for (void *q : ptrs)
         if (q) CM_DROP(hipFree(q));
     *p = PbPlan();
@@ -77,10 +78,16 @@
     return __popcll(mine & ((1ULL << lane) - 1ULL));
 }
 
+__device__ __forceinline__ void pb_store_row(void *pr, size_t at, int r, int row_bytes)
+{
+    if (row_bytes == 1) ((unsigned char *)pr)[at] = (unsigned char)(r & 255);
+    else ((u16 *)pr)[at] = (u16)r;
+}
+
 template <bool FILL>
 __global__ __launch_bounds__(64 * kPbBuildWaves) void k_pb_rows(int n, const int *rp, const int *ci,
                                                                const double *val, PbCut cut, const int *col0, int NCB,
-                                                               int SR, int NSUB, int *bins, double *pv, u16 *pc, u16 *pr,
+                                                               int SR, int NSUB, int *bins, double *pv, u16 *pc, void *pr, int row_bytes,
                                                                const unsigned char *vidx, unsigned char *pvi, int sub0, int sub1)
 {
     extern __shared__ int lds_i[];
@@ -118,7 +125,7 @@
                     if (pvi) pvi[dest] = vidx[k];
                     else pv[dest] = val[k];
                     pc[dest] = (u16)(col - col0[cb]);
-                    pr[dest] = (u16)(row - (int)row0);
+                    pb_store_row(pr, (size_t)dest, row - (int)row0, row_bytes);
                 }
                 if (tail) cur[cb] = base + rank + 1;
             }
@@ -168,11 +175,60 @@
     for (int c = lane; c < NCB; c += 64) bins[(size_t)c * NSUB + sub] = cur[c];
 }
 
+__global__ __launch_bounds__(64 * kPbBuildWaves) void k_pb_bounds(int n, const int *rp, const int *ci, PbCut cut, int NCB, int SR, int NSUB,
+                                                                 int *slen, int *longtab, int *nlong, int long_cap)
+{
+    extern __shared__ unsigned long long lds_q[];
+    const int wave = threadIdx.x >> 6, lane = threadIdx.x & 63;
+    const int sub = blockIdx.x * kPbBuildWaves + wave;
+    if (sub >= NSUB) return;
+    unsigned long long *cur = lds_q + (size_t)wave * NCB;
+    for (int c = lane; c < NCB; c += 64) cur[c] = 0ULL;
+    __builtin_amdgcn_fence(__ATOMIC_RELEASE, "wavefront");
+    __builtin_amdgcn_wave_barrier();
+    const long long row0 = (long long)sub * SR;
+    const int row1 = (int)(row0 + SR < n ? row0 + SR : n);
+    const int e0 = row0 < n ? rp[row0] : rp[n], e1 = rp[row1];
+    int t[3];
+#pragma unroll
+    for (int j = 0; j < 3; j++) t[j] = row0 + 256 * (j + 1) < row1 ? rp[row0 + 256 * (j + 1)] : e1;
+    const double inv_cb = 1.0 / (double)cut.CB;
+    for (int k0 = e0; k0 < e1; k0 += 256) {
+        int col[4];
+#pragma unroll
+        for (int u = 0; u < 4; u++) col[u] = k0 + 64 * u + lane < e1 ? ci[k0 + 64 * u + lane] : -1;
+#pragma unroll
+        for (int u = 0; u < 4; u++)
+            if (col[u] >= 0) {
+                const int k = k0 + 64 * u + lane;
+                const int hi = (k >= t[0] ? 1 : 0) + (k >= t[1] ? 1 : 0) + (k >= t[2] ? 1 : 0);
+                atomicAdd(&cur[col_to_cb_fast(cut, inv_cb, col[u])], pb_seg_count_add(hi));
+            }
+    }
+    __builtin_amdgcn_fence(__ATOMIC_RELEASE, "wavefront");
+    __builtin_amdgcn_wave_barrier();
+    for (int c = lane; c < NCB; c += 64) {
+        const PbSeg sg = pb_seg_counted(cur[c]);
+        int word = pb_seg_word_short(sg);
+        if (sg.len > kPbRows8Short) {
+            const int slot = atomicAdd(nlong, 1);
+            if (slot < long_cap) {
+                longtab[4 * (size_t)slot] = sg.len;
+                longtab[4 * (size_t)slot + 1] = sg.b1;
+                longtab[4 * (size_t)slot + 2] = sg.b2;
+                longtab[4 * (size_t)slot + 3] = sg.b3;
+            }
+            word = pb_seg_word_long(slot);
+        }
+        slen[(size_t)sub * NCB + c] = word;
+    }
+}
+
 __global__ __launch_bounds__(64 * kPbBuildWaves) void k_pb_group(int n, const int *rp, const int *ci, const double *val,
                                                                 const unsigned char *vidx, PbCut cut, const int *col0, int NCB,
                                                                 int SR, const int *slen, int GB, int NG, int *gstart,
                                                                 double *sval, unsigned char *sval8, unsigned long long *smeta,
-                                                                int sub0, int sub1)
+                                                                int row_bytes, const int *longtab, int sub0, int sub1)
 {
     __shared__ unsigned long long tab_all[kPbBuildWaves][kPbGroups];
     __shared__ int lrp_all[kPbBuildWaves][kPbRpMax + 1];
@@ -188,7 +244,7 @@
     int cnt = 0;
     if (lane < NG) {
         const int *sl = slen + (size_t)sub * NCB;
-        for (int c = lane * GB; c < (lane + 1) * GB && c < NCB; c++) cnt += sl[c];
+        for (int c = lane * GB; c < (lane + 1) * GB && c < NCB; c++) cnt += pb_seg_len(sl[c], row_bytes == 1, longtab);
     }
     int inc = cnt;
 #pragma unroll
@@ -247,7 +303,7 @@
 __global__ __launch_bounds__(64 * kPbScatterWaves) void k_pb_scatter(int NCB, int NSUB, const int *slen, const int *bins, int GB, int NG,
                                                                     const int *gstart, const double *sval, const unsigned char *sval8,
                                                                     const unsigned long long *smeta, double *pv, unsigned char *pvi,
-                                                                    u16 *pc, u16 *pr, int sub0, int sub1)
+                                                                    u16 *pc, void *pr, int row_bytes, const int *longtab, int sub0, int sub1)
 {
     __shared__ unsigned raw_all[kPbScatterWaves][kPbBucketMax];
     __shared__ unsigned char cbl_all[kPbScatterWaves][kPbBucketMax];
@@ -264,7 +320,7 @@
     if (len <= 0) return;
     const int cbid = g * GB + lane;
     const bool owner = lane < GB && cbid < NCB;
-    const int cnt = owner ? slen[(size_t)sub * NCB + cbid] : 0;
+    const int cnt = owner ? pb_seg_len(slen[(size_t)sub * NCB + cbid], row_bytes == 1, longtab) : 0;
     int inc = cnt;
 #pragma unroll
     for (int o = 1; o < 64; o <<= 1) {
@@ -292,7 +348,7 @@
                 if (pvi) pvi[r] = sval8[start + k];
                 else pv[r] = sval[start + k];
                 pc[r] = (u16)((m >> 16) & 0xffff);
-                pr[r] = (u16)(m & 0xffff);
+                pb_store_row(pr, (size_t)r, (int)(m & 0xffff), row_bytes);
             }
         }
     }
@@ -322,7 +378,7 @@
                 if (pvi) pvi[dest[u]] = vi[u];
                 else pv[dest[u]] = v[u];
                 pc[dest[u]] = (u16)((m[u] >> 16) & 0xffff);
-                pr[dest[u]] = (u16)(m[u] & 0xffff);
+                pb_store_row(pr, (size_t)dest[u], (int)(m[u] & 0xffff), row_bytes);
             }
         }
     }
@@ -383,15 +439,18 @@
 }
 
 __global__ __launch_bounds__(kBlock) void k_pb_segscan(int NCB, int NSUB, const int *cstart, int *bins, int *sstart,
-                                                       int *slen)
+                                                       int *slen, int *segmax)
 {
     __shared__ int lds_waves[kBlock / 64];
     const int c = blockIdx.x;
     int *b = bins + (size_t)c * NSUB;
     int run = cstart[c];
+    int longest = 0, nlong = 0;
     for (int s0 = 0; s0 < NSUB; s0 += kBlock) {
         const int sidx = s0 + threadIdx.x;
         const int cnt = sidx < NSUB ? b[sidx] : 0;
+        longest = cnt > longest ? cnt : longest;
+        nlong += cnt > kPbRows8Short ? 1 : 0;
         int total;
         const int ex = block_exclusive_scan(cnt, lds_waves, &total);
         if (sidx < NSUB) {
@@ -402,6 +461,16 @@
         }
         run += total;
     }
+#pragma unroll
+    for (int o = 32; o > 0; o >>= 1) {
+        const int t = __shfl_xor(longest, o, 64);
+        longest = t > longest ? t : longest;
+        nlong += __shfl_xor(nlong, o, 64);
+    }
+    if ((threadIdx.x & 63) == 0) {
+        atomicMax(segmax, longest);
+        if (nlong) atomicAdd(segmax + 1, nlong);
+    }
 }
 
 static int round_blocks(int64_t n, int tile_max)
@@ -424,6 +493,8 @@
     pb_scratch_free(b);
     if (b->bins) CM_DROP(hipFree(b->bins));
     b->bins = nullptr;
+    if (b->segmax) CM_DROP(hipFree(b->segmax));
+    b->segmax = nullptr;
     pb_free(&b->p);
 }
 
@@ -494,9 +565,14 @@
     const size_t nbins = (size_t)p.NCB * p.NSUB;
     int *&bins = b->bins;
     bins = nullptr;
+    b->segmax = nullptr;
+    b->counted = false;
+    b->rows8 = cfg.pb_rows8;
     int rc = CUDAMAT_OK;
     do {
         if ((rc = dalloc(&bins, nbins))) break;
+        if ((rc = dalloc(&b->segmax, 3))) break;
+        if ((rc = dalloc(&p.longseg, 4 * (size_t)kPbRows8LongPerSub * (size_t)p.NSUB))) break;
         constexpr int align = kPbAlign;
         const size_t cap = (size_t)nnz + (size_t)(align - 1) * (size_t)p.NCB + 16;
         b->cap = cap;
@@ -541,6 +617,7 @@
         if ((rc = dalloc(&p.sstart, nbins))) break;
         if ((rc = dalloc(&p.slen, nbins))) break;
         if ((rc = set_max_lds((const void *)k_pb_count))) break;
+        if ((rc = set_max_lds((const void *)k_pb_bounds))) break;
         if ((rc = set_max_lds((const void *)k_pb_rows<true>))) break;
         b->GB = 1;
         while (b->GB * kPbGroups < p.NCB) b->GB *= 2;
@@ -579,13 +656,26 @@
         if (hipGetLastError() != hipSuccess) { rc = CUDAMAT_ERR_HIP; set_error("pb count launch failed"); break; }
         hipLaunchKernelGGL(k_pb_colsum, dim3(p.NCB), dim3(kBlock), 0, st, p.NSUB, bins, p.cstart);
         hipLaunchKernelGGL(k_pb_colscan, dim3(1), dim3(kBlock), 0, st, p.NCB, p.cstart, p.cstart, align);
-        hipLaunchKernelGGL(k_pb_segscan, dim3(p.NCB), dim3(kBlock), 0, st, p.NCB, p.NSUB, p.cstart, bins, p.sstart, p.slen);
-        int counted = -1;
+        if (hipMemsetAsync(b->segmax, 0, 3 * sizeof(int), st) != hipSuccess) { rc = CUDAMAT_ERR_HIP; set_error("pb scan failed"); break; }
+        hipLaunchKernelGGL(k_pb_segscan, dim3(p.NCB), dim3(kBlock), 0, st, p.NCB, p.NSUB, p.cstart, bins, p.sstart, p.slen, b->segmax);
+        int counted = -1, seg[2] = {-1, -1};
         if (hipGetLastError() != hipSuccess ||
             hipMemcpyAsync(&counted, p.cstart + p.NCB, sizeof(int), hipMemcpyDeviceToHost, st) != hipSuccess ||
+            hipMemcpyAsync(seg, b->segmax, 2 * sizeof(int), hipMemcpyDeviceToHost, st) != hipSuccess ||
             hipStreamSynchronize(st) != hipSuccess) { rc = CUDAMAT_ERR_HIP; set_error("pb scan failed"); break; }
         if ((int64_t)counted < nnz || (int64_t)counted > nnz + (int64_t)(align - 1) * p.NCB) {
             rc = CUDAMAT_ERR_ARG; set_error("pb_build: counted %d entries, expected %lld", counted, (long long)nnz); break;
+        }
+        const int long_cap = kPbRows8LongPerSub * p.NSUB;
+        const size_t lds8 = sizeof(unsigned long long) * (size_t)kPbBuildWaves * p.NCB;
+        p.row_bytes = b->rows8 && p.SR <= kPbRows8MaxSR && seg[0] >= 0 && seg[0] <= kPbRows8MaxLen && seg[1] >= 0 && seg[1] <= long_cap &&
+                              lds8 <= 150 * 1024 ? 1 : 2;
+        p.nlong = p.row_bytes == 1 ? seg[1] : 0;
+        b->counted = true;
+        if (p.row_bytes == 1) {
+            hipLaunchKernelGGL(k_pb_bounds, dim3(grid), dim3(64 * kPbBuildWaves), lds8, st, n, rp, ci, cut, p.NCB, p.SR, p.NSUB, p.slen, p.longseg,
+                               b->segmax + 2, long_cap);
+            if (hipGetLastError() != hipSuccess) { rc = CUDAMAT_ERR_HIP; set_error("pb row-index pass launch failed"); break; }
         }
         b->verbose = cfg.verbose != 0;
         b->report_classes = cfg.verbose >= 2;
@@ -734,7 +824,7 @@
     return false;
 }
 
-static int place_copy(hipStream_t st, bool verbose, double max_seconds, size_t b_vals, size_t b_idx, size_t b_prod, void **vals, void **pc, void **pr, void **prod, bool *placed,
+static int place_copy(hipStream_t st, bool verbose, double max_seconds, size_t b_vals, size_t b_idx, size_t b_rows, size_t b_prod, void **vals, void **pc, void **pr, void **prod, bool *placed,
                       PbPlan *report)
 {
     *placed = false;
@@ -752,9 +842,9 @@
     }
     const size_t gran = (size_t)2 << 20;
     auto up = [&](size_t x) { return (x + gran - 1) / gran * gran; };
-    const size_t a_vals = up(b_vals), a_idx = up(b_idx), a_prod = up(b_prod);
+    const size_t a_vals = up(b_vals), a_idx = up(b_idx), a_rows = up(b_rows), a_prod = up(b_prod);
     const size_t n_prod = (a_prod + kPlaceBlock - 1) / kPlaceBlock;
-    const size_t n_vals = (a_vals + 2 * a_idx + kPlaceBlock - 1) / kPlaceBlock;
+    const size_t n_vals = (a_vals + a_idx + a_rows + kPlaceBlock - 1) / kPlaceBlock;
     const size_t slab_bytes = std::max(kPlaceSlab, (n_prod + n_vals + 1) * kPlaceBlock);
     std::vector<PlaceSlab> slabs;
     PlaceRun r_prod{}, r_vals{};
@@ -800,7 +890,7 @@
         char *p_vals = slabs[r_vals.slab].b0 + r_vals.first * kPlaceBlock, *p_prod = slabs[r_prod.slab].b0 + r_prod.first * kPlaceBlock;
         char *p_idx = p_vals + a_vals;
         const size_t s_idx = r_vals.slab;
-        const Keep keeps[4] = {{r_vals.slab, p_vals, a_vals, vals}, {s_idx, p_idx, a_idx, pc}, {s_idx, p_idx + a_idx, a_idx, pr}, {r_prod.slab, p_prod, a_prod, prod}};
+        const Keep keeps[4] = {{r_vals.slab, p_vals, a_vals, vals}, {s_idx, p_idx, a_idx, pc}, {s_idx, p_idx + a_idx, a_rows, pr}, {r_prod.slab, p_prod, a_prod, prod}};
         for (size_t si = 0; si < slabs.size(); si++) {
             PlaceSlab &sl = slabs[si];
             std::vector<std::pair<char *, bool>> marks, cuts;
@@ -859,16 +949,17 @@
     PbPlan &p = b->p;
     const size_t cap = b->cap;
     const bool dict = vd && vd->n > 0;
+    const size_t row_bytes = b->counted ? (size_t)p.row_bytes : sizeof(u16);
     int rc = CUDAMAT_OK;
     do {
         if (!p.P && b->place > 0 && sizeof(double) * cap >= kPlaceMinBytes) {
             void *v = nullptr, *c = nullptr, *r = nullptr, *pp = nullptr;
             bool placed = false;
-            if ((rc = place_copy(st, b->verbose, b->place_max_seconds, dict ? cap : sizeof(double) * cap, sizeof(u16) * cap, sizeof(double) * cap, &v, &c, &r, &pp, &placed, &p))) break;
+            if ((rc = place_copy(st, b->verbose, b->place_max_seconds, dict ? cap : sizeof(double) * cap, sizeof(u16) * cap, row_bytes * cap, sizeof(double) * cap, &v, &c, &r, &pp, &placed, &p))) break;
             if (placed) {
                 if (dict) p.pvi = (unsigned char *)v; else p.pv = (double *)v;
                 p.pc = (u16 *)c;
-                p.pr = (u16 *)r;
+                p.pr = r;
                 p.P = (double *)pp;
             }
         }
@@ -883,7 +974,7 @@
         }
         if (p.P && p.pc && p.pr && p.pc_zeroed) break;
         if (!p.pc && (rc = dalloc(&p.pc, cap))) break;
-        if (!p.pr && (rc = dalloc(&p.pr, cap))) break;
+        if (!p.pr && (rc = dalloc((unsigned char **)&p.pr, row_bytes * cap))) break;
         if (!p.P && (rc = dalloc(&p.P, cap))) break;
         if (kPbAlign > 1 && hipMemsetAsync(p.pc, 0, sizeof(u16) * cap, st) != hipSuccess) { rc = CUDAMAT_ERR_HIP; break; }
         p.pc_zeroed = true;
@@ -908,15 +999,15 @@
             if (pad > 64 * 1024) pad = 64 * 1024;
         }
         hipLaunchKernelGGL(k_pb_group, dim3(grid), dim3(64 * kPbBuildWaves), pad, st, p.n, rp, ci, val, vidx, b->cut, p.col0, p.NCB, p.SR,
-                           p.slen, b->GB, b->NG, b->gstart, p.P, p.pvi ? (unsigned char *)p.P : (unsigned char *)nullptr, b->smeta, sub0, sub1);
+                           p.slen, b->GB, b->NG, b->gstart, p.P, p.pvi ? (unsigned char *)p.P : (unsigned char *)nullptr, b->smeta, p.row_bytes, p.longseg, sub0, sub1);
         const long long buckets = (long long)(sub1 - sub0) * b->NG;
         hipLaunchKernelGGL(k_pb_scatter, dim3((unsigned)((buckets + kPbScatterWaves - 1) / kPbScatterWaves)), dim3(64 * kPbScatterWaves), 0, st,
                            p.NCB, p.NSUB, p.slen, b->bins, b->GB, b->NG, b->gstart, p.P, p.pvi ? (const unsigned char *)p.P : (const unsigned char *)nullptr,
-                           b->smeta, p.pv, p.pvi, p.pc, p.pr, sub0, sub1);
+                           b->smeta, p.pv, p.pvi, p.pc, p.pr, p.row_bytes, p.longseg, sub0, sub1);
     } else {
         const size_t lds = sizeof(int) * (size_t)kPbBuildWaves * p.NCB;
         hipLaunchKernelGGL(k_pb_rows<true>, dim3(grid), dim3(64 * kPbBuildWaves), lds, st, p.n, rp, ci, val, b->cut, p.col0,
-                           p.NCB, p.SR, p.NSUB, b->bins, p.pv, p.pc, p.pr, vidx, p.pvi, sub0, sub1);
+                           p.NCB, p.SR, p.NSUB, b->bins, p.pv, p.pc, p.pr, p.row_bytes, vidx, p.pvi, sub0, sub1);
     }
     if (hipGetLastError() != hipSuccess) { set_error("pb fill launch failed"); pb_build_abort(b); return CUDAMAT_ERR_HIP; }
     return CUDAMAT_OK;
@@ -928,16 +1019,19 @@
     std::vector<int> hl(nbins);
     if (hipMemcpy(hl.data(), p.slen, sizeof(int) * nbins, hipMemcpyDeviceToHost) != hipSuccess) return;
     long long hist[7] = {0, 0, 0, 0, 0, 0, 0}, in_long = 0;
-    for (int v : hl) {
+    std::vector<int> lt(4 * (size_t)(p.nlong > 0 ? p.nlong : 1));
+    if (p.nlong > 0 && hipMemcpy(lt.data(), p.longseg, sizeof(int) * 4 * (size_t)p.nlong, hipMemcpyDeviceToHost) != hipSuccess) return;
+    for (int w : hl) {
+        const int v = pb_seg_len(w, p.row_bytes == 1, lt.data());
         hist[v == 0 ? 0 : v <= 8 ? 1 : v <= 24 ? 2 : v <= 48 ? 3 : v <= 64 ? 4 : v <= 128 ? 5 : 6]++;
         if (v > 64) in_long += v;
     }
     fprintf(stderr, "[cudamat] pb arrays: pv %p pvi %p pc %p pr %p P %p sstart %p slen %p cstart %p\n", (void *)p.pv, (void *)p.pvi, (void *)p.pc,
             (void *)p.pr, (void *)p.P, (void *)p.sstart, (void *)p.slen, (void *)p.cstart);
-    fprintf(stderr, "[cudamat] pb plan: %d x %lld, nnz %lld, NCB %d (CB %d), NSUB %d (NW %d, SR %d), LPS %d, depth %d; segments: "
+    fprintf(stderr, "[cudamat] pb plan: %d x %lld, nnz %lld, NCB %d (CB %d), NSUB %d (NW %d, SR %d), LPS %d, depth %d, %d-byte row index (%d segments above 127 entries); segments: "
                     "empty %lld, 1-8 %lld, 9-24 %lld, 25-48 %lld, 49-64 %lld, 65-128 %lld, >128 %lld; %.1f %% of the entries in "
                     "segments longer than a wave\n",
-            p.n, (long long)p.n_cols, (long long)p.nnz, p.NCB, p.CB, p.NSUB, p.NW, p.SR, p.LPS, p.depth, hist[0], hist[1], hist[2], hist[3],
+            p.n, (long long)p.n_cols, (long long)p.nnz, p.NCB, p.CB, p.NSUB, p.NW, p.SR, p.LPS, p.depth, p.row_bytes, p.nlong, hist[0], hist[1], hist[2], hist[3],
             hist[4], hist[5], hist[6], 100.0 * (double)in_long / (double)(p.nnz > 0 ? p.nnz : 1));
 }
 
@@ -968,7 +1062,7 @@
     }
     struct Arr { const char *name; const char *ptr; size_t bytes; };
     const Arr arrs[4] = {{"values", p.pv ? (const char *)p.pv : (const char *)p.pvi, p.pv ? sizeof(double) * cap : cap},
-                         {"col idx", (const char *)p.pc, sizeof(u16) * cap}, {"row idx", (const char *)p.pr, sizeof(u16) * cap}, {"products", (const char *)p.P, sizeof(double) * cap}};
+                         {"col idx", (const char *)p.pc, sizeof(u16) * cap}, {"row idx", (const char *)p.pr, (size_t)p.row_bytes * cap}, {"products", (const char *)p.P, sizeof(double) * cap}};
     for (const Arr &a : arrs) {
         std::string line;
         for (size_t off = 0; off + kPlaceSample <= a.bytes; off += kPlaceSample) {
@@ -994,6 +1088,8 @@
     pb_scratch_free(b);
     CM_DROP(hipFree(b->bins));
     b->bins = nullptr;
+    CM_DROP(hipFree(b->segmax));
+    b->segmax = nullptr;
     b->p.build_seconds = now_s() - b->t0;
     *out = b->p;
     b->p = PbPlan();
@@ -1130,7 +1226,8 @@
     int n, NCB, SR;
     const int *sstart, *slen;
     const double *P;
-    const u16 *pr;
+    const void *pr;
+    const int *longseg;
     const double *d, *xd;
     double alpha, beta;
     double *y;
@@ -1222,7 +1319,23 @@
     return CUDAMAT_OK;
 }
 
-template <int NW, int LPS, int DEPTH>
+template <bool R8>
+__device__ __forceinline__ int pb_row_load(const void *pr, int at)
+{
+    return R8 ? (int)((const unsigned char *)pr)[at] : (int)((const u16 *)pr)[at];
+}
+template <bool R8>
+__device__ __forceinline__ PbSeg pb_seg_decode(int word, const int *longtab)
+{
+    return R8 ? pb_seg_of(word, longtab) : PbSeg{word, 0, 0, 0};
+}
+template <bool R8>
+__device__ __forceinline__ int pb_row_of(int loaded, const PbSeg &sg, int pos)
+{
+    return R8 ? pb_seg_row(loaded, sg, pos) : loaded;
+}
+
+template <int NW, int LPS, int DEPTH, bool R8>
 __global__ __launch_bounds__(64 * NW) void k_pb_phase2(Pb2Args a)
 {
     extern __shared__ __attribute__((aligned(16))) double yt[];
@@ -1238,32 +1351,36 @@
     for (int cb0 = 0; cb0 < a.NCB; cb0 += 64) {
         const int c = cb0 + lane;
         const int mys = c < a.NCB ? ss[c] : 0;
-        const int myl = c < a.NCB ? sl[c] : 0;
+        const int myw = c < a.NCB ? sl[c] : 0;
+        const int myl = R8 ? (pb_seg_is_long(myw) ? kPbRows8Short + 1 : (myw & 0xff)) : myw;
         const int lim = a.NCB - cb0 < 64 ? a.NCB - cb0 : 64;
         const bool grouped = LPS < 64 && !__any(myl > LPS);
         if (!grouped) {
             for (int j = 0; j < lim; j += DEPTH) {
-                int s[DEPTH], l[DEPTH];
+                int s[DEPTH], w[DEPTH], l[DEPTH];
                 double pv4[DEPTH];
                 int r4[DEPTH];
 #pragma unroll
                 for (int u = 0; u < DEPTH; u++) {
                     s[u] = __builtin_amdgcn_readlane(mys, (j + u) & 63);
-                    l[u] = __builtin_amdgcn_readlane(myl, (j + u) & 63);
+                    w[u] = __builtin_amdgcn_readlane(myw, (j + u) & 63);
+                    l[u] = R8 ? pb_seg_len(w[u], true, a.longseg) : w[u];
                 }
 #pragma unroll
                 for (int u = 0; u < DEPTH; u++) {
                     const bool on = lane < l[u];
                     pv4[u] = on ? a.P[s[u] + lane] : 0.0;
-                    r4[u] = on ? (int)a.pr[s[u] + lane] : 0;
+                    r4[u] = on ? pb_row_load<R8>(a.pr, s[u] + lane) : 0;
                 }
 #pragma unroll
                 for (int u = 0; u < DEPTH; u++) {
-                    pb_seg_add(my, r4[u], pv4[u], lane < l[u], lane, 0, a.strict != 0);
+                    const PbSeg sg = pb_seg_decode<R8>(w[u], a.longseg);
+                    pb_seg_add(my, pb_row_of<R8>(r4[u], sg, lane), pv4[u], lane < l[u], lane, 0, a.strict != 0);
                     for (int off0 = 64; off0 < l[u]; off0 += 64) {
                         const int off = off0 + lane;
                         const bool on = off < l[u];
-                        pb_seg_add(my, on ? (int)a.pr[s[u] + off] : 0, on ? a.P[s[u] + off] : 0.0, on, lane, 0, a.strict != 0);
+                        pb_seg_add(my, on ? pb_row_of<R8>(pb_row_load<R8>(a.pr, s[u] + off), sg, off) : 0, on ? a.P[s[u] + off] : 0.0, on, lane, 0,
+                                   a.strict != 0);
                     }
                 }
             }
@@ -1271,21 +1388,24 @@
             constexpr int G = 64 / LPS;
             const int g = lane / LPS, li = lane % LPS;
             for (int j = 0; j < lim; j += DEPTH * G) {
-                int s[DEPTH], l[DEPTH];
+                int s[DEPTH], w[DEPTH], l[DEPTH];
                 double pv4[DEPTH];
                 int r4[DEPTH];
 #pragma unroll
                 for (int u = 0; u < DEPTH; u++) {
                     const int cbi = j + u * G + g;
                     s[u] = __shfl(mys, cbi & 63, 64);
-                    l[u] = cbi < 64 ? __shfl(myl, cbi & 63, 64) : 0;
+                    w[u] = cbi < 64 ? __shfl(myw, cbi & 63, 64) : 0;
+                    l[u] = R8 ? (w[u] & 0xff) : w[u];
                 }
 #pragma unroll
                 for (int u = 0; u < DEPTH; u++) {
                     const bool on = li < l[u];
                     pv4[u] = on ? a.P[s[u] + li] : 0.0;
-                    r4[u] = on ? (int)a.pr[s[u] + li] : 0;
+                    r4[u] = on ? pb_row_load<R8>(a.pr, s[u] + li) : 0;
                 }
+#pragma unroll
+                for (int u = 0; u < DEPTH; u++) r4[u] = pb_row_of<R8>(r4[u], pb_seg_decode<R8>(w[u], nullptr), li);
 #pragma unroll
                 for (int u = 0; u < DEPTH; u++) {
                     if (!a.strict) {
@@ -1389,17 +1509,22 @@
     Pb2Args b;
     b.n = p.n; b.NCB = p.NCB; b.SR = p.SR;
     b.sstart = p.sstart; b.slen = p.slen;
-    b.P = p.P; b.pr = p.pr;
+    b.P = p.P; b.pr = p.pr; b.longseg = p.longseg;
     b.d = a.d; b.xd = a.xd;
     b.alpha = a.alpha; b.beta = a.beta;
     b.y = a.y; b.dot = a.dot; b.w = a.w; b.parts = a.parts;
     b.st = a.loop.st;
     b.strict = a.pb_strict;
     const size_t lds = sizeof(double) * ((size_t)p.NW * p.SR + 2 * (size_t)p.NW);
+#define CM_P2R(NWV, LPSV, DV, R8V)                                                                        \
+    do {                                                                                                  \
+        CM_TRY(set_max_lds((const void *)k_pb_phase2<NWV, LPSV, DV, R8V>));                              \
+        hipLaunchKernelGGL((k_pb_phase2<NWV, LPSV, DV, R8V>), dim3(p.NRB), dim3(64 * NWV), lds, st, b);  \
+    } while (0)
 #define CM_P2D(NWV, LPSV, DV)                                                                             \
     do {                                                                                                  \
-        CM_TRY(set_max_lds((const void *)k_pb_phase2<NWV, LPSV, DV>));                                   \
-        hipLaunchKernelGGL((k_pb_phase2<NWV, LPSV, DV>), dim3(p.NRB), dim3(64 * NWV), lds, st, b);       \
+        if (p.row_bytes == 1) CM_P2R(NWV, LPSV, DV, true);                                                \
+        else CM_P2R(NWV, LPSV, DV, false);                                                                \
     } while (0)
 #define CM_P2(NWV, LPSV)                                                                                  \
     do {                                                                                                  \
@@ -1421,6 +1546,7 @@
 #undef CM_P2_LPS
 #undef CM_P2
 #undef CM_P2D
+#undef CM_P2R
     CM_HIP(hipGetLastError());
     return CUDAMAT_OK;
 }
diff --git a/cuda_mat_amd/host/selftest.cpp b/cuda_mat_amd/host/selftest.cpp
--- a/cuda_mat_amd/host/selftest.cpp
+++ b/cuda_mat_amd/host/selftest.cpp
@@ -1,11 +1,13 @@
 #include <cstdio>
 #include <cstdlib>
 #include <cstring>
+#include <algorithm>
 #include <string>
 #include <vector>
 
 #include "Matrix.h"
 #include "cudamat.h"
+#include "../csrc/pb_rows.h"
 
 static int failures = 0;
 #define EXPECT(cond)                                                       \
@@ -24,6 +26,50 @@
 static int load(const std::string &path, bool csr, int *m, int *n, int *nnz, double **v, int **r, int **c)
 {
     return cudamat_load_mtx(path.c_str(), csr ? 1 : 0, m, n, nnz, v, r, c);
+}
+
+static void check_segment(const std::vector<int> &rows, int slot)
+{
+    using namespace cm;
+    unsigned long long cnt = 0;
+    for (int r : rows) cnt += pb_seg_count_add(r >> 8);
+    const PbSeg sg = pb_seg_counted(cnt);
+    EXPECT(sg.len == (int)rows.size());
+    std::vector<int> table(4 * (size_t)(slot + 1), -1);
+    int word;
+    if (sg.len > kPbRows8Short) {
+        word = pb_seg_word_long(slot);
+        table[4 * (size_t)slot] = sg.len; table[4 * (size_t)slot + 1] = sg.b1; table[4 * (size_t)slot + 2] = sg.b2; table[4 * (size_t)slot + 3] = sg.b3;
+        EXPECT(pb_seg_is_long(word) && pb_seg_long_index(word) == slot);
+    } else {
+        word = pb_seg_word_short(sg);
+        EXPECT(!pb_seg_is_long(word));
+    }
+    EXPECT(pb_seg_len(word, true, table.data()) == sg.len && pb_seg_len(sg.len, false, nullptr) == sg.len);
+    const PbSeg back = pb_seg_of(word, table.data());
+    EXPECT(back.len == sg.len && back.b1 == sg.b1 && back.b2 == sg.b2 && back.b3 == sg.b3);
+    for (size_t i = 0; i < rows.size(); i++) EXPECT(pb_seg_row(rows[i] & 255, back, (int)i) == rows[i]);
+}
+
+static void check_pb_rows()
+{
+    unsigned long long z = 12345;
+    auto next = [&z]() { z = z * 6364136223846793005ULL + 1442695040888963407ULL; return (unsigned)(z >> 33); };
+    const int lens[] = {0, 1, 2, 63, 64, 65, 127, 128, 254, 255, 256, 300, 1024, 5000, 65535};
+    for (int len : lens) {
+        for (int shape = 0; shape < 6; shape++) {
+            std::vector<int> rows((size_t)len);
+            for (int i = 0; i < len; i++)
+                rows[(size_t)i] = shape == 0 ? (int)(next() % 1024)
+                                  : shape == 1 ? (int)(next() % 256)
+                                  : shape == 2 ? 768 + (int)(next() % 256)
+                                  : shape == 3 ? (int)((long long)i * 1024 / (len > 0 ? len : 1))
+                                  : shape == 4 ? (i < len / 2 ? 255 : 256)
+                                  : (i % 2 ? 1023 : 0);
+            std::sort(rows.begin(), rows.end());
+            check_segment(rows, shape);
+        }
+    }
 }
 
 int main(int argc, char **argv)
@@ -90,6 +136,7 @@
     bool threw = false;
     try { A.get(2, 0); } catch (const std::out_of_range &) { threw = true; }
     EXPECT(threw);
+    check_pb_rows();
     if (failures == 0) std::printf("SELFTEST_OK\n");
     return failures ? 1 : 0;
 }
diff --git a/include/cudamat.h b/include/cudamat.h
--- a/include/cudamat.h
+++ b/include/cudamat.h
@@ -148,6 +148,7 @@
 int cudamat_solver_value_dict(cudamat_solver *s, int *distinct);
 int cudamat_solver_spmv_kernel(cudamat_solver *s, char *name, int cap);
 int cudamat_solver_placement(cudamat_solver *s, int *placed, int *slabs, double *seconds, char *classes, int cap);
+int cudamat_solver_pb_geometry(cudamat_solver *s, int *ncb, int *nsub, int *sr, int *lps, int *row_bytes);
 int cudamat_solver_spmv(cudamat_solver *s, const double *x_local, double *y_local);
 int cudamat_solver_solve(cudamat_solver *s, const double *b, double *x, int precond,
                          int loop, int maxit, double tol, int flags, cudamat_stats *st);
```

Result: slower. 170.7 (-6.5%).
